# TUMFTM/DPFT

Hardware: AMD Instinct MI355X
Metric: training samples/sec (K-Radar C+R, bs4/GPU) (higher is better)
Workload: dtype f32

## Files before the change

dpft_amd/csrc/common.h:

```cpp
#pragma once
#include <hip/hip_runtime.h>
#include <stdint.h>
#include <stdio.h>
#include <string.h>

#include "../../include/dpft_hip.h"

typedef float f32x4 __attribute__((ext_vector_type(4)));
typedef float f32x16 __attribute__((ext_vector_type(16)));

namespace dpft {

void set_error(const char* fmt, ...);
struct BnReduceFuse {
    const float* y;
    const float* bnp;
    const unsigned char* mask8;
    int self_mask;
    float* sums;
    bool applied;
};
int conv_dgrad_residual(const dpft_conv_desc* d, const float* dy, const float* w_t, float* dx, const float* res_src,
                        const float* res_mask, void* workspace, dpft_stream_t stream, BnReduceFuse* fuse = nullptr,
                        const unsigned char* res_mask8 = nullptr);
// ... 19 lines not shown
__device__ __forceinline__ void bn_from_sums(const BnSumsRef& r, int c, float& mean, float& scale, float& beta, float& invstd) {
    const double m = bn_sums_get(r.sums, r.K, c, 0) * r.invn;
    const double var = fmax(bn_sums_get(r.sums, r.K, c, 1) * r.invn - m * m, 0.0);
    mean = (float)m;
    invstd = 1.0f / sqrtf((float)var + r.eps);
    scale = r.gamma[c] * invstd;
    beta = r.beta[c];
}
__device__ __forceinline__ void fill_pro_table(float* tab, const float* bnp, const BnSumsRef& r, int K, int tid, int nt) {
    if (r.sums) {
        for (int c = tid; c < K; c += nt) {
            float mean, scale, beta, invstd;
            bn_from_sums(r, c, mean, scale, beta, invstd);
            tab[c] = mean; tab[K + c] = scale; tab[2 * K + c] = beta;
        }
    } else {
        for (int i = tid; i < 3 * K; i += nt) tab[i] = bnp[i];
    }
}
int conv_fwd_sums(const dpft_conv_desc* d, const float* x, const float* w, const float* bias, const float* pro_bn,
                  int32_t pro_relu, float* y, float* stats, void* workspace, dpft_stream_t stream,
                  unsigned long long* sums = nullptr, bool* sums_used = nullptr,
                  const BnSumsRef* pro_sums = nullptr, bool* pro_sums_used = nullptr);
int conv_dgrad_fused(const dpft_conv_desc* d, const float* dy, const float* w_t, float* dx, int32_t accumulate,
                     void* workspace, dpft_stream_t stream, BnReduceFuse* fuse);
int bn_bwd_reduce_prezeroed(const float* y, const float* dout, const float* out, const float* mask_bnp, const float* bnp,
                            float* sums, int64_t M, int32_t K, bool act16, dpft_stream_t stream,
                            const unsigned char* mask8 = nullptr);
int bn_bwd_apply_zeroing(const float* y, const float* dout, const float* out, const float* mask_bnp, const float* bnp,
                         const float* gamma, const float* sums, float* dy, float* dgamma, float* dbeta, int64_t M,
                         int32_t K, float* zero_buf, int32_t zero_n, bool act16, dpft_stream_t stream,
                         const unsigned char* mask8 = nullptr, bool frozen = false);
int bn_act_any(const float* y, const float* bnp, const float* res, const float* res_bnp, int32_t relu, float* out,
               float* out32, int64_t M, int32_t K, bool act16, dpft_stream_t stream, unsigned char* mask8 = nullptr);
int bn_act_sums(const float* y, const float* bnp, const BnSumsRef& ys, const float* res, const float* res_bnp, const BnSumsRef& rs,
                int32_t relu, float* out, int64_t M, int32_t K, dpft_stream_t stream, unsigned char* mask8, bool* used);
struct BnSumsBatch {
    static constexpr int MAX = 48;
    const unsigned long long* sums[MAX];
    const float *gamma[MAX], *beta[MAX];
    float *rm[MAX], *rv[MAX], *out[MAX];
    double invn[MAX];
    long long M[MAX];
    int K[MAX];
    int n;
    float eps, momentum;
};
int bn_finalize_sums_batch(const BnSumsBatch& batch, dpft_stream_t stream);
int bn_relu_maxpool_any(const float* y, const float* bnp, float* out, int32_t B, int32_t H, int32_t W, int32_t K,
                        int32_t PH, int32_t PW, bool out16, dpft_stream_t stream);
int bn_relu_maxpool_bwd_any(const float* y, const float* bnp, const float* dout, float* dact, int32_t B, int32_t H,
                            int32_t W, int32_t K, int32_t PH, int32_t PW, bool dout16, dpft_stream_t stream);
int add_inplace_any(float* a, const float* b, int64_t n, bool a16, dpft_stream_t stream);
int cvt_f32_to_bf16(const float* src, float* dst_bf16, int64_t n, dpft_stream_t stream);
struct BnEvalBatch {
    const float *gamma[16], *beta[16], *rm[16], *rv[16];
    float* out[16];
    int K[16];
    int n;
    float eps;
};
int bn_eval_params_batch(const BnEvalBatch& batch, dpft_stream_t stream);
struct TransposeBatch {
    static constexpr int MAX = 80;
    const float* w[MAX];
    float* wt[MAX];
    int K[MAX], taps[MAX], C[MAX];
    int blk_start[MAX + 1];
    int n;
    int mode = 0;
    int tile = 0;
    static int tile_of(int k, int c) { return (k % 64 == 0 && c % 64 == 0) ? 64 : 32; }
    bool fits(int k, int c) const { return n == 0 || tile == tile_of(k, c); }
    void add(const float* src, float* dst, int k, int t, int c) {
        if (n == 0) tile = tile_of(k, c);
        w[n] = src; wt[n] = dst; K[n] = k; taps[n] = t; C[n] = c;
        if (n == 0) blk_start[0] = 0;
        blk_start[n + 1] = blk_start[n] + ((c + tile - 1) / tile) * ((k + tile - 1) / tile) * t;
        ++n;
    }
};
int weight_transpose_batch(const TransposeBatch& tb, dpft_stream_t stream);
int conv_mode_key();
bool profiling_active();
int zero_fill(void* ptr, size_t bytes, dpft_stream_t stream);
int bias_grad_ws(const float* dy, float* db, int64_t M, int32_t K, void* workspace, dpft_stream_t stream);

struct LdsGrant {
    size_t granted[16] = {};
};
inline bool lds_grant(LdsGrant& g, const void* fn, size_t lds) {
    int dev = 0;
    (void)hipGetDevice(&dev);
    size_t& have = g.granted[dev & 15];
    if (lds <= have) return true;
    if (hipFuncSetAttribute(fn, hipFuncAttributeMaxDynamicSharedMemorySize, (int)lds) != hipSuccess) return false;
    have = lds;
    return true;
}

inline int check_launch(const char* what) {
    hipError_t e = hipGetLastError();
    if (e != hipSuccess) {
        set_error("%s: launch failed: %s", what, hipGetErrorString(e));
        return DPFT_ERR_LAUNCH;
    }
    return DPFT_OK;
}

inline int cdiv(int64_t a, int64_t b) { return (int)((a + b - 1) / b); }

constexpr int kNumCU = 256;
constexpr int kNumXCD = 8;

__device__ __forceinline__ int xcd_remap(int bid, int nwg) {
    const int q = nwg / kNumXCD, r = nwg % kNumXCD;
    const int xcd = bid % kNumXCD, idx = bid / kNumXCD;
    const int base = (xcd < r) ? xcd * (q + 1) : r * (q + 1) + (xcd - r) * q;
    return base + idx;
}

}

#ifndef DPFT_PRIO_BN
#define DPFT_PRIO_BN 3
#endif
#ifndef DPFT_PRIO_IGEMM
#define DPFT_PRIO_IGEMM 1
#endif
#define DPFT_SETPRIO_BN() do { if (DPFT_PRIO_BN) __builtin_amdgcn_s_setprio(DPFT_PRIO_BN); } while (0)
#define DPFT_SETPRIO_IGEMM() do { if (DPFT_PRIO_IGEMM) __builtin_amdgcn_s_setprio(DPFT_PRIO_IGEMM); } while (0)

#define DPFT_REQUIRE(cond, ...)                 \
    do {                                        \
        if (!(cond)) {                          \
            dpft::set_error(__VA_ARGS__);       \
            return DPFT_ERR_ARG;                \
        }                                       \
    } while (0)
```

dpft_amd/csrc/conv.hip:

```cpp
#include "conv_core.h"

namespace dpft {


template <int BM, int BN, int WGM, int WGN, bool DGRAD, bool PRO, bool LIN = true, bool BF16 = false, int KS = 1>
__global__ __launch_bounds__(64 * WGM * WGN * KS) void igemm_vec_kernel(IgemmArgs a) {
    static_assert(KS == 1 || KS == 2, "K-split form: two wave sets");
    constexpr int NT = 64 * WGM * WGN * KS, ROWS = NT / 16;
    constexpr int RB = BM / WGM / 32, CB = BN / WGN / 32;
    constexpr int AP = BM / ROWS, BP = BN / ROWS;
    static_assert(WGM * WGN == 4 && RB >= 1 && CB >= 1, "bad tile");
    extern __shared__ __attribute__((aligned(16))) float smem[];
    float* As = smem;
    float* Bs = smem + BM * LDK;
    __bf16* Ah = reinterpret_cast<__bf16*>(smem);
    __bf16* Bh = Ah + BM * LDKH;

    const int tid = threadIdx.x, lane = tid & 63, wave = (tid >> 6) & 3;
    const int kh = KS == 1 ? 0 : tid >> 8;
    const int wm = wave / WGN, wn = wave % WGN;
    int mt, nt, split;
    decode_tile(a, mt, nt, split);
    const int m0 = mt * BM, n0 = nt * BN;

// ... 355 lines not shown
            bh = ok ? oh + a.pad : -(1 << 28);
            bw = ow + a.pad;
        }
        abase = a.x + (size_t)b * a.H * a.W * a.C;
    }
    const int brow = tid % BN, bkq = tid / BN;
    const bool bok = (n0 + brow) < a.N;
    const float* bbase = a.w + (size_t)(bok ? n0 + brow : 0) * a.Ktot;

    float ra[16], rbv[KPB];
    auto load_tile = [&](int kt) {
        int k = kt * BK + akh * 16;
        int tap = k / a.C;
        int c = k - tap * a.C;
        int r = tap / a.kw, s = tap - r * a.kw;
#pragma unroll
        for (int e = 0; e < 16; ++e) {
            int hi, wi;
            bool v = (k + e) < a.Ktot;
            if (!DGRAD) {
                hi = bh + r;
                wi = bw + s;
                v = v && (unsigned)hi < (unsigned)a.H && (unsigned)wi < (unsigned)a.W;
            } else {
                const int th = bh - r, tw = bw - s;
                v = v && th >= 0 && tw >= 0;
                hi = th / a.stride;
                wi = tw / a.stride;
                v = v && (hi * a.stride == th) && (wi * a.stride == tw) && hi < a.H && wi < a.W;
            }
            ra[e] = v ? abase[((size_t)hi * a.W + wi) * a.C + c] : 0.f;
            if (++c == a.C) {
                c = 0;
                if (++s == a.kw) {
                    s = 0;
                    ++r;
                }
            }
        }
        const int kb = kt * BK + bkq * KPB;
#pragma unroll
        for (int e = 0; e < KPB; ++e) rbv[e] = (bok && (kb + e) < a.Ktot) ? bbase[kb + e] : 0.f;
    };
    auto store_tile = [&]() {
#pragma unroll
        for (int e = 0; e < 16; ++e) As[arow * LDG + akh * 16 + e] = ra[e];
#pragma unroll
        for (int e = 0; e < KPB; ++e) Bs[brow * LDG + bkq * KPB + e] = rbv[e];
    };

    f32x16 acc[RB][CB];
#pragma unroll
    for (int j = 0; j < CB; ++j)
#pragma unroll
        for (int r = 0; r < 16; ++r) acc[0][j][r] = 0.f;

    const int kt_begin = split * a.ksteps_per_split;
    const int kt_end = min(a.ksteps, kt_begin + a.ksteps_per_split);
    const float* a_frag = As + (wm * 32 + (lane & 31)) * LDG + (lane >> 5);
    const float* b_frag = Bs + (lane & 31) * LDG + (lane >> 5);
    if (kt_begin < kt_end) {
        load_tile(kt_begin);
        store_tile();
    }
    __syncthreads();
    for (int kt = kt_begin; kt < kt_end; ++kt) {
        const bool more = kt + 1 < kt_end;
        if (more) load_tile(kt + 1);
#pragma unroll
        for (int kk = 0; kk < BK / 2; ++kk) {
            const float av = a_frag[kk * 2];
#pragma unroll
            for (int j = 0; j < CB; ++j)
                acc[0][j] = __builtin_amdgcn_mfma_f32_32x32x2f32(av, b_frag[j * 32 * LDG + kk * 2],
                                                                 acc[0][j], 0, 0, 0);
        }
        __syncthreads();
        if (more) store_tile();
        __syncthreads();
    }
    igemm_epilogue<BM, BN, WGM, WGN, RB, CB>(a, acc, m0, n0, mt, split, smem);
}

__global__ void splitk_reduce_kernel(const float* __restrict__ partial, const float* __restrict__ bias,
                                     float* __restrict__ y, int64_t MN, int N, int splits, int accumulate) {
    int64_t i = ((int64_t)blockIdx.x * blockDim.x + threadIdx.x) * 4;
    if (i >= MN) return;
    if (i + 3 < MN && (N % 4) == 0) {
        f32x4 s = *reinterpret_cast<const f32x4*>(partial + i);
        for (int k = 1; k < splits; ++k) {
            f32x4 t = *reinterpret_cast<const f32x4*>(partial + (size_t)k * MN + i);
            s += t;
        }
        if (bias) {
            const int c = (int)(i % N);
#pragma unroll
            for (int e = 0; e < 4; ++e) s[e] += bias[c + e];
        }
        if (accumulate) s += *reinterpret_cast<const f32x4*>(y + i);
        *reinterpret_cast<f32x4*>(y + i) = s;
    } else {
        for (int e = 0; e < 4 && i + e < MN; ++e) {
            float s = 0.f;
            for (int k = 0; k < splits; ++k) s += partial[(size_t)k * MN + i + e];
            if (bias) s += bias[(i + e) % N];
            if (accumulate) s += y[i + e];
            y[i + e] = s;
        }
    }
}

__global__ __launch_bounds__(256) void splitk_reduce_stats_kernel(const float* __restrict__ partial, float* __restrict__ y,
                                                                  float* __restrict__ stats, int64_t M, int N, int splits,
                                                                  int tile_rows) {
    __shared__ f32x4 red[16][16];
    __shared__ f32x4 smean[16];
    const int cl = threadIdx.x & 15, rg = threadIdx.x >> 4;
    const int tile = blockIdx.x, c = blockIdx.y * 64 + cl * 4;
    const int64_t r0 = (int64_t)tile * tile_rows, MN = M * N;
    const int cnt = (int)min((int64_t)tile_rows, M - r0);
    f32x4 v[8];
    f32x4 sum = {0.f, 0.f, 0.f, 0.f};
#pragma unroll
    for (int i = 0; i < 8; ++i) {
        const int r = rg + i * 16;
        v[i] = f32x4{0.f, 0.f, 0.f, 0.f};
        if (r < cnt) {
            const int64_t o = (r0 + r) * N + c;
            f32x4 a = *reinterpret_cast<const f32x4*>(partial + o);
            for (int k = 1; k < splits; ++k) a += *reinterpret_cast<const f32x4*>(partial + (size_t)k * MN + o);
            *reinterpret_cast<f32x4*>(y + o) = a;
            v[i] = a;
            sum += a;
        }
    }
    red[rg][cl] = sum;
    __syncthreads();
    if (rg == 0) {
        f32x4 t = red[0][cl];
        for (int i = 1; i < 16; ++i) t += red[i][cl];
        smean[cl] = t * (1.0f / (float)cnt);
    }
    __syncthreads();
    const f32x4 mean = smean[cl];
    f32x4 m2 = {0.f, 0.f, 0.f, 0.f};
#pragma unroll
    for (int i = 0; i < 8; ++i)
        if (rg + i * 16 < cnt) {
            const f32x4 dlt = v[i] - mean;
            m2 += dlt * dlt;
        }
    __syncthreads();
    red[rg][cl] = m2;
    __syncthreads();
    if (rg == 0) {
        f32x4 t = red[0][cl];
        for (int i = 1; i < 16; ++i) t += red[i][cl];
        *reinterpret_cast<f32x4*>(stats + ((size_t)tile * 2 + 0) * N + c) = mean;
        *reinterpret_cast<f32x4*>(stats + ((size_t)tile * 2 + 1) * N + c) = t;
    }
}

template <int PARTS>
__global__ __launch_bounds__(256) void splitk_reduce_wide_kernel(const float* __restrict__ partial, float* __restrict__ y,
                                                                 int64_t MN, int splits) {
    constexpr int CH = 256 / PARTS;
    __shared__ f32x4 red[256];
    const int ch = threadIdx.x % CH, part = threadIdx.x / CH;
    const int64_t i = ((int64_t)blockIdx.x * CH + ch) * 4;
    f32x4 s = {0.f, 0.f, 0.f, 0.f};
    if (i < MN)
        for (int k = part; k < splits; k += PARTS) s += *reinterpret_cast<const f32x4*>(partial + (size_t)k * MN + i);
    red[threadIdx.x] = s;
    __syncthreads();
    if (part == 0 && i < MN) {
#pragma unroll
        for (int q = 1; q < PARTS; ++q) s += red[q * CH + ch];
        *reinterpret_cast<f32x4*>(y + i) = s;
    }
}

__global__ void splitk_reduce_residual_kernel(const float* __restrict__ partial, const float* __restrict__ src,
                                              const float* __restrict__ mask, float* __restrict__ y, int64_t MN,
                                              int splits) {
    const int64_t i = (int64_t)blockIdx.x * blockDim.x + threadIdx.x;
    if (i >= MN) return;
    float s = 0.f;
    for (int k = 0; k < splits; ++k) s += partial[(size_t)k * MN + i];
    y[i] = s + (mask[i] > 0.f ? src[i] : 0.f);
}


template <int BMn, int BNc, int WGM, int WGN, bool PRO, bool BF16 = false>
__global__ __launch_bounds__(256) void wgrad_vec_kernel(WgradArgs a) {
    static_assert(!BF16 || (BMn == BNc && (BMn == 128 || BMn == 64)), "bf16 weight gradient: 128 x 128 and 64 x 64 tiles");
    constexpr int RB = BMn / WGM / 32, CB = BNc / WGN / 32;
    constexpr int YCH = BMn / 4, XCH = BNc / 4;
    constexpr int YRP = 256 / YCH, XRP = 256 / XCH;
    constexpr int YP = BKP / YRP, XP = BKP / XRP;
    static_assert(WGM * WGN == 4 && YP >= 1 && XP >= 1, "bad wgrad tile");
    constexpr int SMEM_FLOATS = BKP * (BMn + BNc);
    __shared__ __attribute__((aligned(16))) float smem[SMEM_FLOATS];
    float* Ys = smem;
    float* Xs = smem + BKP * BMn;
    const int tid = threadIdx.x, lane = tid & 63, wave = tid >> 6;
    const int wm = wave / WGN, wn = wave % WGN;

    const int nwg = a.ktiles * a.ctiles * a.taps * a.splits;
    int bid = xcd_remap(blockIdx.x, nwg);
    const int split = bid / (a.ktiles * a.ctiles * a.taps);
    bid -= split * (a.ktiles * a.ctiles * a.taps);
    const int tap = bid / (a.ktiles * a.ctiles);
    bid -= tap * (a.ktiles * a.ctiles);
    const int kt_ = bid / a.ctiles, ct_ = bid - kt_ * a.ctiles;
    const int n0 = kt_ * BMn, c0 = ct_ * BNc;
    const int r = tap / a.kw, s = tap - r * a.kw;

    const int ych = tid % YCH, yrow = tid / YCH;
    const int xch = tid % XCH, xrow = tid / XCH;
    const bool y_ok = (n0 + ych * 4) < a.K;
    const bool x_ok = (c0 + xch * 4) < a.C;
    f32x4 mu = {0.f, 0.f, 0.f, 0.f}, sc = {1.f, 1.f, 1.f, 1.f}, sh = {0.f, 0.f, 0.f, 0.f};
    if (PRO && x_ok) {
        mu = *reinterpret_cast<const f32x4*>(a.pro + c0 + xch * 4);
        sc = *reinterpret_cast<const f32x4*>(a.pro + a.C + c0 + xch * 4);
        sh = *reinterpret_cast<const f32x4*>(a.pro + 2 * a.C + c0 + xch * 4);
        if (BF16) sh -= mu * sc;
    }
    const int ohw = a.OH * a.OW;

    f32x4 ry[YP], rx[XP];
    unsigned x_valid = 0;
    constexpr unsigned OOB = 0x80000000u;
    const bool x16 = a.x16 != 0, dy16 = a.dy16 != 0;
    const __amdgpu_buffer_rsrc_t rsrc_y =
        __builtin_amdgcn_make_buffer_rsrc(const_cast<float*>(a.dy), 0, a.M * a.K * (dy16 ? 2 : 4), 0x00020000);
    const __amdgpu_buffer_rsrc_t rsrc_x =
        __builtin_amdgcn_make_buffer_rsrc(const_cast<float*>(a.x), 0, a.B * a.H * a.W * a.C * (x16 ? 2 : 4), 0x00020000);
    auto ypix = [&](int i) { return BF16 ? 2 * YRP * (i >> 1) + 2 * yrow + (i & 1) : yrow + i * YRP; };
    auto xpix = [&](int i) { return BF16 ? 2 * XRP * (i >> 1) + 2 * xrow + (i & 1) : xrow + i * XRP; };
    unsigned y_voff[YP];
#pragma unroll
    for (int i = 0; i < YP; ++i) y_voff[i] = y_ok ? (unsigned)(ypix(i) * a.K + n0 + ych * 4) * 4u : OOB;
    int xb[XP], xoh[XP], xow[XP];
    {
        const int p_first = (split * a.psteps_per_split) * BKP;
#pragma unroll
        for (int i = 0; i < XP; ++i) {
// ... 988 lines not shown
    (void)big16_tile(d, a, false, false, t);
    if (tile_rows) *tile_rows = t.bm;
    return cdiv(a.M, t.bm);
}

extern "C" int dpft_conv2d_nhwc_fwd_f32(const dpft_conv_desc* d, const float* x, const float* w,
                                        const float* bias, const float* pro_bn, int32_t pro_relu,
                                        float* y, float* stats, void* workspace, dpft_stream_t stream) {
    return dpft::conv_fwd_sums(d, x, w, bias, pro_bn, pro_relu, y, stats, workspace, stream);
}

int dpft::conv_fwd_sums(const dpft_conv_desc* d, const float* x, const float* w, const float* bias, const float* pro_bn,
                        int32_t pro_relu, float* y, float* stats, void* workspace, dpft_stream_t stream,
                        unsigned long long* sums, bool* sums_used, const BnSumsRef* pro_sums, bool* pro_sums_used) {
    if (sums_used) *sums_used = false;
    if (pro_sums_used) *pro_sums_used = false;
    if (pro_sums && !pro_sums->sums) pro_sums = nullptr;
    DPFT_REQUIRE(!pro_sums || (pro_bn && pro_sums_used), "conv fwd: a prologue from column sums needs the BN block's address and the answer slot");
    DPFT_REQUIRE(!sums || (stats && sums_used), "conv fwd: column sums need the statistics table and the answer slot");
    int rc = check_desc(d);
    if (rc) return rc;
    DPFT_REQUIRE(x && w && y, "conv fwd: null tensor");
    {
        static const char* skip = getenv("DPFT_SKIP");
        if (skip && ((strstr(skip, "fwd3x3") && d->kh == 3) || (strstr(skip, "fwd1x1") && d->kh == 1)) && (int64_t)d->B * d->OH * d->OW >= 4096) return DPFT_OK;
    }
    hipStream_t st = (hipStream_t)stream;
    ProfScope prof(0, d, st);
    if (conv16_matches(d) && !pro_bn && !stats) return conv16_forward(d, x, w, bias, y, st);
    static const bool thin_fwd = getenv("DPFT_THIN_FWD") == nullptr || atoi(getenv("DPFT_THIN_FWD")) != 0;
    if (thin_fwd && conv1x1_to16_matches(d) && !pro_bn && !stats) return conv1x1_to16_forward(d, x, w, bias, y, st);
    if (takes_stream1x1(d)) {
        const bool fits = !bias && (!pro_bn || pro_relu);
        DPFT_REQUIRE(fits || !stats, "conv fwd: statistics of a streaming 1x1 conv (%d -> %d) take no bias and only the BatchNorm + ReLU prologue", d->C, d->K);
        if (fits) {
            g_prof_family = kFamF32;
            unsigned long long* bns = sums && (int64_t)d->B * d->OH * d->OW < (1 << 22) ? sums : nullptr;
            if (bns) *sums_used = true;
            if (pro_sums) *pro_sums_used = true;
            return launch_stream1x1(d, x, w, pro_bn, y, stats, nullptr, nullptr, 0, st, bns, pro_sums);
        }
    }
    IgemmArgs a; fill_igemm(a, d, false);
    a.x = x; a.w = w; a.y = y; a.bias = bias; a.stats = stats;
    a.pro = pro_bn; a.pro_relu = pro_relu;
    a.x16 = a.y16 = d->act16 != 0;
    a.w16 = d->act16 == 2;
    if (d->a_planes && d->w_planes && !pro_bn && !d->act16) { a.x3 = d->a_planes; a.w3 = d->w_planes; }
    DPFT_REQUIRE(!(a.w16 && (bias || pro_bn)), "conv fwd: act16 = 2 (bf16 weights) takes no bias and no operand prologue");
    const bool pro = pro_bn != nullptr;
    TileChoice t = choose_tile(a.M, a.N, a.C, a.ksteps, (d->act16 || (pro && !pro_relu)) ? 1 : taps_of(d));
    const bool big16 = !pro && !bias && big16_tile(d, a, false, workspace != nullptr, t);
    if (d->act16 && !big16) t.splits = 1;
    if (big16 && t.splits > 1 && !sk_fixup_ok(a, t.splits, 1)) t.splits = 1;
    DPFT_REQUIRE(!(pro && !t.vec), "conv fwd: fused prologue needs C %% 64 == 0 (C=%d)", d->C);
    if (pro_sums) {
        static const int pipe_env = getenv("DPFT_PIPE") ? atoi(getenv("DPFT_PIPE")) : 3;
        if (!(t.vec && g_conv_bf16 != 1 && !d->act16 && pro_relu && (t.x3 || (pipe_env & 1)) && (int64_t)12 * d->C <= 16384)) return DPFT_OK;
        a.pro_s = *pro_sums;
        *pro_sums_used = true;
    }
    bool fixup = false;
    if (t.splits > 1) {
        DPFT_REQUIRE(workspace, "conv fwd: split-K selected but no workspace given");
        a.partial = ws_slabs(workspace);
        fixup = sk_fixup_ok(a, t.splits, 1);
        if (fixup) a.sk_ticket = reinterpret_cast<int*>(workspace);
        else a.stats = nullptr;
    }
    if (sums && !bias && t.vec && (a.N & 3) == 0 && (t.splits == 1 || fixup) && a.M < (1 << 22)) {
        a.bns = sums;
        a.stats = nullptr;
        *sums_used = true;
    }
    rc = launch_igemm<false>(a, t, pro, st);
    if (rc) return rc;
    if (t.splits > 1 && !fixup) {
        const int64_t MN = (int64_t)a.M * a.N;
        if (stats && !bias && (a.N % 64) == 0 && t.bm <= 128) {
            hipLaunchKernelGGL(splitk_reduce_stats_kernel, dim3(cdiv(a.M, t.bm), a.N / 64), dim3(256), 0, st, a.partial, y,
                               stats, (int64_t)a.M, a.N, t.splits, t.bm);
            return check_launch("conv fwd split-K reduce + stats");
        }
        hipLaunchKernelGGL(splitk_reduce_kernel, dim3(cdiv(MN, 1024)), dim3(256), 0, st, a.partial, bias, y, MN, a.N, t.splits, 0);
        rc = check_launch("conv fwd split-K reduce");
        if (rc) return rc;
        if (stats) {
            rc = dpft_bn_stats_f32(y, stats, a.M, a.N, t.bm, stream);
        }
    }
    return rc;
}

extern "C" int dpft_conv2d_nhwc_fwd_bnact_f32(const dpft_conv_desc* d, const float* x, const float* w, const float* out_bn,
                                              int32_t relu, const float* residual, float* y, void* workspace,
                                              dpft_stream_t stream) {
    int rc = check_desc(d);
    if (rc) return rc;
    DPFT_REQUIRE(x && w && y && out_bn, "conv fwd_bnact: null tensor");
    DPFT_REQUIRE(d->K % 4 == 0, "conv fwd_bnact: K %% 4 == 0 needed (K=%d)", d->K);
    hipStream_t st = (hipStream_t)stream;
    if (takes_stream1x1(d)) {
        ProfScope prof(0, d, st);
        g_prof_family = kFamF32;
        return launch_stream1x1(d, x, w, nullptr, y, nullptr, out_bn, residual, relu, st);
    }
    IgemmArgs a; fill_igemm(a, d, false);
    TileChoice t = choose_tile(a.M, a.N, a.C, a.ksteps, d->act16 ? 1 : taps_of(d));
    if (d->act16) t.splits = 1;
    const int64_t M = (int64_t)d->B * d->OH * d->OW;
    static const bool fix_all = getenv("DPFT_BNACT_FIXUP") == nullptr || atoi(getenv("DPFT_BNACT_FIXUP")) != 0;
    if ((t.x3 || (fix_all && t.vec && !conv16_matches(d))) && t.splits > 1 && workspace && sk_fixup_ok(a, t.splits, 1)) {
        ProfScope prof(0, d, st);
        a.x = x; a.w = w; a.y = y;
        a.partial = ws_slabs(workspace);
        a.sk_ticket = reinterpret_cast<int*>(workspace);
        a.obn = out_bn; a.oadd = residual; a.orelu = relu;
        return launch_igemm<false>(a, t, false, st);
    }
    if (!t.vec || t.splits > 1 || conv16_matches(d)) {
        rc = dpft_conv2d_nhwc_fwd_f32(d, x, w, nullptr, nullptr, 0, y, nullptr, workspace, stream);
        if (rc) return rc;
        return bn_act_any(y, out_bn, residual, nullptr, relu, y, nullptr, M, d->K, d->act16 != 0, stream);
    }
    ProfScope prof(0, d, st);
    a.x = x; a.w = w; a.y = y; a.bias = nullptr; a.stats = nullptr; a.pro = nullptr; a.pro_relu = 0;
    a.x16 = a.y16 = d->act16 != 0;
    if (d->a_planes && d->w_planes && !d->act16) { a.x3 = d->a_planes; a.w3 = d->w_planes; }
    a.obn = out_bn; a.oadd = residual; a.orelu = relu;
    static const int epf_on = getenv("DPFT_EPF") == nullptr ? 7 : atoi(getenv("DPFT_EPF"));
    if ((epf_on & 4) && residual && !d->act16 && !a.x3 && !t.x3 && (int64_t)a.M * a.N < (1ll << 29) && d->stride == 1 && g_conv_bf16 != 1) a.epf = 3;
    return launch_igemm<false>(a, t, false, st);
}

extern "C" int dpft_fpn_lateral_f32(const dpft_conv_desc* d, const float* x, const float* w, const float* bias, const float* top,
                                    int32_t TH, int32_t TW, float* lat, void* workspace, dpft_stream_t stream) {
    int rc = check_desc(d);
    if (rc) return rc;
    DPFT_REQUIRE(x && w && lat && d->kh == 1 && d->kw == 1 && d->stride == 1 && d->pad == 0, "fpn_lateral: a 1x1 conv (stride 1) with its tensors");
    DPFT_REQUIRE(!top || (TH >= 1 && TW >= 1 && TH <= d->H && TW <= d->W && d->K % 4 == 0), "fpn_lateral: bad top level (%d x %d)", TH, TW);
    static const bool fuse = getenv("DPFT_FPN_FUSE") == nullptr || atoi(getenv("DPFT_FPN_FUSE")) != 0;
    if (top && fuse && conv1x1_to16_top_matches(d)) {
        ProfScope prof(0, d, (hipStream_t)stream);
        g_prof_family = kFamVector;
        return conv1x1_to16_top_forward(d, x, w, bias, top, TH, TW, lat, (hipStream_t)stream);
    }
    rc = dpft_conv2d_nhwc_fwd_f32(d, x, w, bias, nullptr, 0, lat, nullptr, workspace, stream);
    if (rc || !top) return rc;
    return dpft_fpn_topdown_add_f32(lat, top, d->B, d->H, d->W, TH, TW, d->K, stream);
}

extern "C" int dpft_fpn_output_f32(const dpft_conv_desc* d, const float* lat, const float* w, const float* bias, const float* pos_x,
                                   const float* pos_y, float* out, void* workspace, dpft_stream_t stream) {
    int rc = check_desc(d);
    if (rc) return rc;
    DPFT_REQUIRE(lat && w && out && (pos_x == nullptr) == (pos_y == nullptr), "fpn_output: null tensor / one embedding table without the other");
    DPFT_REQUIRE(d->H == d->OH && d->W == d->OW, "fpn_output: a same-size conv");
    static const bool fuse = getenv("DPFT_FPN_FUSE") == nullptr || atoi(getenv("DPFT_FPN_FUSE")) != 0;
    if (pos_x && fuse && conv16_matches(d) && !d->act16) {
        ProfScope prof(0, d, (hipStream_t)stream);
        g_prof_family = kFamVector;
        return conv16_forward(d, lat, w, bias, out, (hipStream_t)stream, pos_x, pos_y);
    }
    rc = dpft_conv2d_nhwc_fwd_f32(d, lat, w, bias, nullptr, 0, out, nullptr, workspace, stream);
    if (rc || !pos_x) return rc;
    return dpft_add_pos_f32(out, pos_x, pos_y, d->B, d->H, d->W, d->K, stream);
}
// ... 19 lines not shown
        if (skip && ((strstr(skip, "dgrad3x3") && d->kh == 3) || (strstr(skip, "dgrad1x1") && d->kh == 1)) && (int64_t)d->B * d->H * d->W >= 4096) {
            if (fuse && fuse->sums) fuse->applied = true;
            return DPFT_OK;
        }
    }
    hipStream_t st = (hipStream_t)stream;
    ProfScope prof(1, d, st);
    if (conv16_matches(d)) return conv16_dgrad(d, dy, w_t, dx, accumulate, st);
    if (d->C <= 4 && d->K % 4 == 0 && (size_t)d->C * d->kh * d->kw * d->K * 4 <= 40960 && ((d->C * d->kh * d->kw * d->K) % 4) == 0) {
        const size_t lds = (size_t)d->C * d->kh * d->kw * d->K * 4;
        const dim3 grid(cdiv((int64_t)d->B * d->H * d->W, 256));
#define THIN_DGRAD(CI)                                                                                                  \
    hipLaunchKernelGGL(thin_dgrad_kernel<CI>, grid, dim3(256), lds, st, dy, w_t, dx, d->B, d->H, d->W, d->OH, d->OW, \
                       d->K, d->kh, d->kw, d->stride, d->pad, accumulate)
        switch (d->C) {
            case 1: THIN_DGRAD(1); break;
            case 2: THIN_DGRAD(2); break;
            case 3: THIN_DGRAD(3); break;
            default: THIN_DGRAD(4); break;
        }
#undef THIN_DGRAD
        return check_launch("conv dgrad (thin input)");
    }
    IgemmArgs a; fill_igemm(a, d, true);
    a.x = dy; a.w = w_t; a.y = dx; a.accumulate = accumulate;
    a.x16 = a.y16 = d->act16 != 0;
    a.w16 = d->act16 == 2;
    if (d->a_planes && d->w_planes && !d->act16) { a.x3 = d->a_planes; a.w3 = d->w_planes; }
    const bool fuse_ok = fuse && fuse->sums && (a.N & 3) == 0;
    const int64_t class_wgs = (int64_t)cdiv((int64_t)a.B * cdiv(a.OH, d->stride) * cdiv(a.OW, d->stride), 64) * cdiv(a.N, 64);
    if (d->stride > 1 && (a.C % BKV) == 0 && (class_wgs >= kNumCU / 2 || !workspace || d->act16)) {
        const int sp = d->stride, cpt = a.C / BKV;
        bool empty_class = false;
        for (int ph = 0; ph < sp; ++ph)
            for (int pw = 0; pw < sp; ++pw) {
                const int r0 = (ph + d->pad) % sp, s0 = (pw + d->pad) % sp;
                if (r0 >= d->kh || s0 >= d->kw) empty_class = true;
            }
        if (empty_class && !accumulate)
            DPFT_REQUIRE(zero_fill(dx, (d->act16 ? 2 : sizeof(float)) * (size_t)a.B * a.OH * a.OW * a.N, st) == DPFT_OK,
                         "conv dgrad: zero fill failed");
        for (int ph = 0; ph < sp; ++ph)
            for (int pw = 0; pw < sp; ++pw) {
                const int r0 = (ph + d->pad) % sp, s0 = (pw + d->pad) % sp;
                if (r0 >= d->kh || s0 >= d->kw || ph >= a.OH || pw >= a.OW) continue;
                IgemmArgs q = a;
                q.sub_step = sp; q.sub_ph = ph; q.sub_pw = pw;
                q.sub_oh = (a.OH - ph + sp - 1) / sp; q.sub_ow = (a.OW - pw + sp - 1) / sp;
                q.sub_r0 = r0; q.sub_s0 = s0;
                q.sub_nr = (d->kh - r0 + sp - 1) / sp; q.sub_ns = (d->kw - s0 + sp - 1) / sp;
                q.M = a.B * q.sub_oh * q.sub_ow;
                q.ksteps = q.sub_nr * q.sub_ns * cpt;
                TileChoice tq = choose_tile(q.M, q.N, q.C, q.ksteps);
                tq.splits = 1;
                if (fuse_ok && !empty_class) set_bnr(q, fuse);
                rc = launch_igemm<true>(q, tq, false, st);
                if (rc) return rc;
            }
        if (fuse_ok && !empty_class) fuse->applied = true;
        return DPFT_OK;
    }
    TileChoice t = choose_tile(a.M, a.N, a.C, a.ksteps, (d->act16 || d->stride > 1) ? 1 : taps_of(d));
    const bool big16 = big16_tile(d, a, true, workspace != nullptr, t);
    if (d->act16 && !big16) t.splits = 1;
    if (big16 && t.splits > 1 && !sk_fixup_ok(a, t.splits, 2)) t.splits = 1;
    bool fixup = false;
    if (t.splits > 1) {
        DPFT_REQUIRE(workspace, "conv dgrad: split-K selected but no workspace given");
        a.partial = ws_slabs(workspace);
        fixup = sk_fixup_ok(a, t.splits, 2);
        if (fixup) a.sk_ticket = reinterpret_cast<int*>(workspace);
    }
    if ((t.splits == 1 || fixup) && fuse_ok) {
        set_bnr(a, fuse);
        fuse->applied = true;
    }
    static const int epf_on = getenv("DPFT_EPF") == nullptr ? 3 : atoi(getenv("DPFT_EPF"));
    if ((epf_on & 2) && t.splits == 1 && a.bnr_sums && !accumulate && d->stride == 1 && t.vec && (int64_t)a.M * a.N < (1ll << 29))
        a.epf = 2;
    rc = launch_igemm<true>(a, t, false, st);
    if (rc) return rc;
    if (t.splits > 1 && !fixup) {
        const int64_t MN = (int64_t)a.M * a.N;
        hipLaunchKernelGGL(splitk_reduce_kernel, dim3(cdiv(MN, 1024)), dim3(256), 0, st, a.partial, (const float*)nullptr, dx, MN, a.N, t.splits, accumulate);
        rc = check_launch("conv dgrad split-K reduce");
    }
    return rc;
}

int dpft::conv_dgrad_residual(const dpft_conv_desc* d, const float* dy, const float* w_t, float* dx, const float* res_src,
                              const float* res_mask, void* workspace, dpft_stream_t stream, BnReduceFuse* fuse,
                              const unsigned char* res_mask8) {
    if (fuse) fuse->applied = false;
    int rc = check_desc(d);
    if (rc) return rc;
    DPFT_REQUIRE(dy && w_t && dx && res_src && res_mask, "conv dgrad residual: null tensor");
    {
        static const char* skip = getenv("DPFT_SKIP");
        if (skip && ((strstr(skip, "dgrad3x3") && d->kh == 3) || (strstr(skip, "dgrad1x1") && d->kh == 1)) && (int64_t)d->B * d->H * d->W >= 4096) {
            if (fuse && fuse->sums) fuse->applied = true;
            return DPFT_OK;
        }
    }

    DPFT_REQUIRE(d->stride == 1 && !conv16_matches(d), "conv dgrad residual: stride-1 bottleneck convs only");
    hipStream_t st = (hipStream_t)stream;
    ProfScope prof(1, d, st);
    IgemmArgs a; fill_igemm(a, d, true);
    a.x = dy; a.w = w_t; a.y = dx; a.res_src = res_src; a.res_mask = res_mask;
    a.x16 = a.y16 = d->act16 != 0;
    a.w16 = d->act16 == 2;
    if (d->a_planes && d->w_planes && !d->act16) { a.x3 = d->a_planes; a.w3 = d->w_planes; }
    if (res_mask8 && (a.N & 3) == 0) a.res_mask8 = res_mask8;
    TileChoice t = choose_tile(a.M, a.N, a.C, a.ksteps, d->act16 ? 1 : taps_of(d));
    const bool big16 = big16_tile(d, a, true, workspace != nullptr, t);
    if (d->act16 && !big16) t.splits = 1;
    if (big16 && t.splits > 1 && !sk_fixup_ok(a, t.splits, 4)) t.splits = 1;
    bool fixup = false;
    if (t.splits > 1) {
        DPFT_REQUIRE(workspace, "conv dgrad: split-K selected but no workspace given");
        a.partial = ws_slabs(workspace);
        fixup = sk_fixup_ok(a, t.splits, 4);
        if (fixup) a.sk_ticket = reinterpret_cast<int*>(workspace);
    }
    if ((t.splits == 1 || fixup) && fuse && fuse->sums && (a.N & 3) == 0) {
        set_bnr(a, fuse);
        fuse->applied = true;
    }
    static const int epf_on = getenv("DPFT_EPF") == nullptr ? 3 : atoi(getenv("DPFT_EPF"));
    if ((epf_on & 1) && t.splits == 1 && a.bnr_sums && a.bnr_mask8 && a.res_mask8 && t.vec && (int64_t)a.M * a.N < (1ll << 29) &&
        (int64_t)cdiv(a.M, 128) * cdiv(a.N, 64) >= kNumCU && getenv("DPFT_FORCE_TILE") == nullptr && !big16) {
        a.epf = 1;
        t.bm = 128; t.bn = 64;
    }
    rc = launch_igemm<true>(a, t, false, st);
    if (rc) return rc;
    if (t.splits > 1 && !fixup) {
        const int64_t MN = (int64_t)a.M * a.N;
        hipLaunchKernelGGL(splitk_reduce_residual_kernel, dim3(cdiv(MN, 256)), dim3(256), 0, st, a.partial, res_src,
                           res_mask, dx, MN, t.splits);
        rc = check_launch("conv dgrad split-K residual reduce");
    }
    return rc;
}

extern "C" int dpft_conv2d_nhwc_dgrad_bn_reduce_f32(const dpft_conv_desc* d, const float* dy, const float* w_t, float* dx,
                                                    int32_t accumulate, const float* res_src, const float* res_out,
                                                    const uint8_t* res_mask8, const float* bn_y, const float* bn_block,
                                                    const uint8_t* bn_mask8, int32_t bn_self_mask, float* sums,
                                                    int32_t* applied, void* workspace, dpft_stream_t stream) {
    DPFT_REQUIRE(bn_y && bn_block && sums && applied, "conv dgrad_bn_reduce: null BatchNorm argument");
    DPFT_REQUIRE((bn_mask8 != nullptr) != (bn_self_mask != 0), "conv dgrad_bn_reduce: exactly one of bn_mask8 / bn_self_mask");
    dpft::BnReduceFuse f{bn_y, bn_block, bn_mask8, bn_self_mask, sums, false};
    int rc;
    if (res_src) {
        DPFT_REQUIRE(!accumulate && res_out, "conv dgrad_bn_reduce: the residual form needs res_out and does not accumulate");
        rc = dpft::conv_dgrad_residual(d, dy, w_t, dx, res_src, res_out, workspace, stream, &f, res_mask8);
    } else {
        rc = dpft::conv_dgrad_fused(d, dy, w_t, dx, accumulate, workspace, stream, &f);
    }
    *applied = f.applied ? 1 : 0;
    return rc;
}

extern "C" int dpft_conv2d_nhwc_wgrad_f32(const dpft_conv_desc* d, const float* x, const float* dy,
                                          const float* pro_bn, int32_t pro_relu, float* dw,
                                          void* workspace, dpft_stream_t stream) {
    {
        static const char* skip = getenv("DPFT_SKIP");
        if (skip && strstr(skip, "wgrad")) return DPFT_OK;
    }
    int rc = check_desc(d);
    if (rc) return rc;
    DPFT_REQUIRE(x && dy && dw, "conv wgrad: null tensor");
    DPFT_REQUIRE(!pro_bn || ((d->C % 32 == 0) && (d->K % 4 == 0)),
                 "conv wgrad: fused prologue needs C %% 32 == 0 and K %% 4 == 0 (C=%d, K=%d)", d->C, d->K);
    hipStream_t st = (hipStream_t)stream;
    ProfScope prof(2, d, st);
    if (!pro_bn) {
        bool handled = false;
        rc = thin_wgrad(d, x, dy, dw, workspace, st, handled);
        if (rc || handled) return rc;
    }
    WgradArgs a; memset(&a, 0, sizeof(a));
    a.x = x; a.dy = dy; a.dw = dw; a.pro = pro_bn; a.pro_relu = pro_relu;
    a.x16 = a.dy16 = d->act16 != 0;
    a.B = d->B; a.H = d->H; a.W = d->W; a.C = d->C; a.OH = d->OH; a.OW = d->OW; a.K = d->K;
    a.kh = d->kh; a.kw = d->kw; a.stride = d->stride; a.pad = d->pad;
    a.M = d->B * d->OH * d->OW;
    a.taps = d->kh * d->kw;
    a.J = a.taps * a.C;
    const bool pro = pro_bn != nullptr;
    const bool vec = (d->C % 32 == 0) && (d->K % 4 == 0);
    a.psteps = cdiv(a.M, vec ? BKP : BK);
    DPFT_REQUIRE(!vec || ((int64_t)a.M * a.K < (1ll << 29) && (int64_t)a.B * a.H * a.W * a.C < (1ll << 29)),
                 "conv wgrad: operand larger than 2 GiB");
    int bmn, bnc;
    int64_t tiles;
    if (vec) {
        if (d->K <= 32) { bmn = 32; bnc = 128; }
        else if (d->K >= 128 && d->C >= 128 && (int64_t)cdiv(d->K, 128) * cdiv(d->C, 128) * a.taps >= 8) { bmn = 128; bnc = 128; }
        else { bmn = 64; bnc = 64; }
        a.ktiles = cdiv(d->K, bmn);
        a.ctiles = cdiv(d->C, bnc);
        tiles = (int64_t)a.ktiles * a.ctiles * a.taps;
    } else {
        bmn = 64; bnc = 64;
        a.ktiles = cdiv(d->K, 64);
        a.ctiles = cdiv(a.J, 64);
        tiles = (int64_t)a.ktiles * a.ctiles;
    }
    const int round_wgs = (vec && bmn == 128) ? kNumCU : kNumCU * 2;
    int splits = (int)std::max<int64_t>(1, round_wgs / tiles);
    {
        const int s2 = (int)std::max<int64_t>(1, 2 * round_wgs / tiles);
        const double f1 = (double)tiles * splits / round_wgs, f2 = (double)tiles * s2 / (2.0 * round_wgs);
        if (f1 < 0.8 && f2 > f1 + 0.1) splits = s2;
    }
    const int64_t wbytes = (int64_t)d->K * a.J * 4;
    const int max_splits = (int)std::max<int64_t>(1, std::min<int64_t>(512, (64ll << 20) / wbytes));
    if (splits > max_splits) splits = max_splits;
    if (splits > 1 && a.psteps / splits < 4) {
        if (vec && bmn == 128) {
            bmn = 64; bnc = 64;
            a.ktiles = cdiv(d->K, bmn); a.ctiles = cdiv(d->C, bnc);
            tiles = (int64_t)a.ktiles * a.ctiles * a.taps;
        }
        splits = (int)std::max<int64_t>(1, std::min<int64_t>(std::min<int64_t>(kNumCU / tiles, a.psteps), max_splits));
    }
    if (splits < 1) splits = 1;
    if (const char* f = getenv("DPFT_FORCE_WGRAD")) {
        int tb, sp;
        if (vec && sscanf(f, "%d,%d", &tb, &sp) == 2 && (tb == 128 || tb == 64)) {
            bmn = tb; bnc = tb;
            a.ktiles = cdiv(d->K, bmn); a.ctiles = cdiv(d->C, bnc);
            tiles = (int64_t)a.ktiles * a.ctiles * a.taps;
            splits = std::max(1, std::min(sp, max_splits));
        }
    }
    if (splits > 1 && !workspace) splits = 1;
    a.splits = splits;
    a.psteps_per_split = cdiv(a.psteps, splits);
    a.partial = splits > 1 ? ws_slabs(workspace) : nullptr;
    const int nwg = (int)(tiles * splits);
    dim3 grid(nwg), block(256);
    static const int wpipe_env = getenv("DPFT_PIPE") ? atoi(getenv("DPFT_PIPE")) : 3;
    static const int w16_env = getenv("DPFT_WGRAD16_PIPE") ? atoi(getenv("DPFT_WGRAD16_PIPE")) : 1;
    if (vec && d->act16 && !pro && w16_env && (bmn == 128 || bmn == 64) && (d->C % 8) == 0 && (d->K % 8) == 0) {
        const int pk = bmn == 128 ? 64 : 128;
        a.psteps = cdiv(a.M, pk);
        a.psteps_per_split = cdiv(a.psteps, splits);
        const size_t lds = (size_t)2 * pk * (bmn + bnc) * 2 + (size_t)a.psteps_per_split * pk * 4;
        g_prof_family = kFamBf16;
        if (bmn == 128) launch_lds(wgrad_pipe16_kernel<128, 128, 2, 2, 64>, grid, block, lds, st, a);
        else launch_lds(wgrad_pipe16_kernel<64, 64, 2, 2, 128>, grid, block, lds, st, a);
    } else if (vec && (wpipe_env & 2) && g_conv_bf16 != 1 && !d->act16 && (!pro || pro_relu) && (bmn == 128 || bmn == 64)) {
        const int pk = bmn == 128 ? 32 : 64;
        a.psteps = cdiv(a.M, pk);
        a.psteps_per_split = cdiv(a.psteps, splits);
        const size_t tbl = (size_t)a.psteps_per_split * pk * 4;
        g_prof_family = kFamF32;
        static const bool wx3 = getenv("DPFT_WGRAD_X3") == nullptr || atoi(getenv("DPFT_WGRAD_X3")) != 0;
        static const bool wx3_1x1 = getenv("DPFT_WGRAD_X3_1X1") == nullptr || atoi(getenv("DPFT_WGRAD_X3_1X1")) != 0;
        if (bmn == 128 && wx3 && split_on() && (a.taps > 1 || wx3_1x1) && 2.0 * a.M * (double)d->K * a.J >= 2e9) {
            g_prof_family = kFamX3;
            rc = launch_wgrad_x3(a, pro, grid, st);
            if (rc) return rc;
        } else if (bmn == 128) {
            const size_t lds = (size_t)2 * 32 * (128 + 128) * 4 + tbl;
            if (pro) launch_lds(wgrad_pipe_kernel<128, 128, 2, 2, 32, true>, grid, block, lds, st, a);
            else launch_lds(wgrad_pipe_kernel<128, 128, 2, 2, 32, false>, grid, block, lds, st, a);
        } else {
            const size_t lds = (size_t)2 * 64 * (64 + 64) * 4 + tbl;
            if (pro) launch_lds(wgrad_pipe_kernel<64, 64, 2, 2, 64, true>, grid, block, lds, st, a);
            else launch_lds(wgrad_pipe_kernel<64, 64, 2, 2, 64, false>, grid, block, lds, st, a);
        }
    } else if (vec) {
        g_prof_family = g_conv_bf16 == 1 && (bmn == 128 || bmn == 64) ? kFamBf16 : kFamF32;
#define LAUNCH_WG(BM_, BN_, WGM_, WGN_)                                                           \
    do {                                                                                          \
        if (pro) hipLaunchKernelGGL((wgrad_vec_kernel<BM_, BN_, WGM_, WGN_, true>), grid, block, 0, st, a);  \
        else hipLaunchKernelGGL((wgrad_vec_kernel<BM_, BN_, WGM_, WGN_, false>), grid, block, 0, st, a);     \
    } while (0)
        if (bmn == 128 && g_conv_bf16 == 1) {
            if (pro) hipLaunchKernelGGL((wgrad_vec_kernel<128, 128, 2, 2, true, true>), grid, block, 0, st, a);
            else hipLaunchKernelGGL((wgrad_vec_kernel<128, 128, 2, 2, false, true>), grid, block, 0, st, a);
        } else if (bmn == 64 && g_conv_bf16 == 1) {
            if (pro) hipLaunchKernelGGL((wgrad_vec_kernel<64, 64, 2, 2, true, true>), grid, block, 0, st, a);
            else hipLaunchKernelGGL((wgrad_vec_kernel<64, 64, 2, 2, false, true>), grid, block, 0, st, a);
        } else if (bmn == 128) LAUNCH_WG(128, 128, 2, 2);
        else if (bmn == 64) LAUNCH_WG(64, 64, 2, 2);
        else LAUNCH_WG(32, 128, 1, 4);
#undef LAUNCH_WG
    } else {
        hipLaunchKernelGGL(wgrad_gen_kernel, grid, block, 0, st, a);
    }
    rc = check_launch("conv wgrad");
    if (rc) return rc;
    {
        static const char* skip = getenv("DPFT_SKIP");
        if (skip && strstr(skip, "wreduce")) return rc;
    }
    if (splits > 1) {
        const int64_t n = (int64_t)d->K * a.J;
        if ((n & 3) == 0 && splits >= 16) {
            if (n / 4 <= (int64_t)kNumCU * 64) hipLaunchKernelGGL(splitk_reduce_wide_kernel<16>, dim3(cdiv(n / 4, 16)), dim3(256), 0, st, a.partial, dw, n, splits);
            else hipLaunchKernelGGL(splitk_reduce_wide_kernel<4>, dim3(cdiv(n / 4, 64)), dim3(256), 0, st, a.partial, dw, n, splits);
        } else {
            hipLaunchKernelGGL(splitk_reduce_kernel, dim3(cdiv(n, 1024)), dim3(256), 0, st, a.partial, (const float*)nullptr, dw, n, 4, splits, 0);
        }
        rc = check_launch("conv wgrad split-K reduce");
    }
    return rc;
}

extern "C" int dpft_weight_transpose_f32(const float* w, float* w_t, int32_t K, int32_t taps,
                                         int32_t C, dpft_stream_t stream) {
    DPFT_REQUIRE(w && w_t && K > 0 && taps > 0 && C > 0, "weight_transpose: bad arguments");
    dim3 grid(cdiv(C, 32), cdiv(K, 32), taps);
    hipLaunchKernelGGL(weight_transpose_kernel, grid, dim3(256), 0, (hipStream_t)stream, w, w_t, K, taps, C);
    return check_launch("weight_transpose");
}

extern "C" int dpft_weight_transpose_batch_f32(int32_t n, const float* const* w, float* const* w_t, const int32_t* K,
                                               const int32_t* taps, const int32_t* C, dpft_stream_t stream) {
    DPFT_REQUIRE(n >= 1 && n <= dpft::TransposeBatch::MAX && w && w_t && K && taps && C, "weight_transpose_batch: 1..80 tensors");
    dpft::TransposeBatch tb;
    tb.n = 0;
    tb.mode = 0;
    for (int i = 0; i < n; ++i) {
        DPFT_REQUIRE(w[i] && w_t[i] && K[i] > 0 && taps[i] > 0 && C[i] > 0, "weight_transpose_batch: bad entry %d", i);
        if (!tb.fits(K[i], C[i])) {
            int rc = dpft::weight_transpose_batch(tb, stream);
            if (rc) return rc;
            tb.n = 0;
        }
        tb.add(w[i], w_t[i], K[i], taps[i], C[i]);
    }
    return dpft::weight_transpose_batch(tb, stream);
}

int dpft::weight_transpose_batch(const TransposeBatch& tb, dpft_stream_t stream) {
    DPFT_REQUIRE(tb.n >= 1 && tb.n <= TransposeBatch::MAX, "weight_transpose_batch: 1..%d tensors", TransposeBatch::MAX);
    if (tb.tile == 64) hipLaunchKernelGGL(weight_transpose_batch64_kernel, dim3(tb.blk_start[tb.n]), dim3(256), 0, (hipStream_t)stream, tb);
    else hipLaunchKernelGGL(weight_transpose_batch_kernel, dim3(tb.blk_start[tb.n]), dim3(256), 0, (hipStream_t)stream, tb);
    return check_launch("weight_transpose_batch");
}

namespace dpft {
__global__ __launch_bounds__(256) void zero_fill_kernel(unsigned* __restrict__ p, size_t n4, size_t n) {
    const size_t stride = (size_t)gridDim.x * 256;
    for (size_t i = (size_t)blockIdx.x * 256 + threadIdx.x; i < n4; i += stride) reinterpret_cast<uint4*>(p)[i] = uint4{0u, 0u, 0u, 0u};
    if (blockIdx.x == 0)
        for (size_t i = n4 * 4 + threadIdx.x; i < n; i += 256) p[i] = 0u;
}
}

int dpft::zero_fill(void* ptr, size_t bytes, dpft_stream_t stream) {
    DPFT_REQUIRE(ptr && (bytes & 3) == 0 && ((uintptr_t)ptr & 15) == 0, "zero_fill: 16-byte aligned pointer, size a multiple of 4");
    const size_t n = bytes / 4, n4 = n / 4;
    const int blocks = (int)std::max<size_t>(1, std::min<size_t>(kNumCU * 8, (n4 + 255) / 256));
    hipLaunchKernelGGL(zero_fill_kernel, dim3(blocks), dim3(256), 0, (hipStream_t)stream, (unsigned*)ptr, n4, n);
    return check_launch("zero_fill");
}

extern "C" int dpft_bias_grad_f32(const float* dy, float* db, int64_t M, int32_t K,
                                  dpft_stream_t stream) {
    DPFT_REQUIRE(dy && db && M > 0 && K > 0 && K <= 256, "bias_grad: bad arguments (K=%d)", K);
    (void)hipMemsetAsync(db, 0, sizeof(float) * K, (hipStream_t)stream);
    const int rpi = 256 / K;
    int blocks = (int)std::min<int64_t>(1024, (M + rpi - 1) / rpi);
    hipLaunchKernelGGL(bias_grad_kernel, dim3(blocks), dim3(256), 0, (hipStream_t)stream, dy, db, M, K);
    return check_launch("bias_grad");
}

int dpft::bias_grad_ws(const float* dy, float* db, int64_t M, int32_t K, void* workspace, dpft_stream_t stream) {
    static const bool slab_on = getenv("DPFT_BIAS_SLAB") == nullptr || atoi(getenv("DPFT_BIAS_SLAB")) != 0;
    if (!workspace || !slab_on || K > 256 || K <= 0) return dpft_bias_grad_f32(dy, db, M, K, stream);
    const int rpi = 256 / K;
    const int blocks = (int)std::min<int64_t>(kBiasBlocks, (M + rpi - 1) / rpi);
    hipLaunchKernelGGL(bias_grad_slab_kernel, dim3(blocks), dim3(256), 0, (hipStream_t)stream, dy, db, M, (int)K, ws_slabs(workspace),
                       reinterpret_cast<int*>(workspace));
    return check_launch("bias_grad (slab)");
}

extern "C" int dpft_conv2d_nhwc_wgrad_bias_f32(const dpft_conv_desc* d, const float* x, const float* dy, float* dw, float* db,
                                               void* workspace, dpft_stream_t stream) {
    int rc = check_desc(d);
    if (rc) return rc;
    DPFT_REQUIRE(x && dy && dw && db, "conv wgrad_bias: null tensor");
    static const bool fuse = getenv("DPFT_BIAS_FUSE") == nullptr || atoi(getenv("DPFT_BIAS_FUSE")) != 0;
    const bool fusable = dpft::conv16_matches(d) ||
                         (d->kh == 1 && d->kw == 1 && d->stride == 1 && d->pad == 0 && d->K == 16 && (d->C == 3 || d->C == 6));
    if (fuse && fusable && workspace && !d->act16) {
        dpft::ProfScope prof(2, d, (hipStream_t)stream);
        bool handled = false, bias_done = false;
// ... 73 lines not shown
```

dpft_amd/csrc/conv_core.h:

```cpp
#pragma once
#include "common.h"

#include <math.h>
#include <stdlib.h>

#include <algorithm>
#include <type_traits>
#include <utility>
#include <vector>

namespace dpft {

constexpr int BK = 32;
constexpr int BKV = 64;
constexpr int LDK = BKV + 4;
constexpr int LDKH = BKV + 8;
typedef __bf16 bf16x4 __attribute__((ext_vector_type(4)));
typedef __bf16 bf16x8 __attribute__((ext_vector_type(8)));
constexpr int LDG = BK + 1;
constexpr int BKP = 64;

typedef unsigned u32x2 __attribute__((ext_vector_type(2)));
typedef unsigned u32x4 __attribute__((ext_vector_type(4)));
__device__ __forceinline__ f32x4 widen_bf16x4(u32x2 v) {
// ... 351 lines not shown
                    }
                    if (accum || resid || oadd) v += old[it];
                    if (obn && a.orelu) {
#pragma unroll
                        for (int e = 0; e < 4; ++e) v[e] = fmaxf(v[e], 0.f);
                    }
                    const size_t ooff = out_pixel(a, m0 + row) * a.N + n0 + c4 * 4;
                    store4_act(out, ooff, v, decltype(H16)::value);
                    if (bnr) {
                        const f32x4 yv = bnr_yv[it];
                        f32x4 d = v;
                        if (decltype(H16)::value) d = __builtin_convertvector(__builtin_convertvector(v, bf16x4s), f32x4);
                        if (PFM == 1 || a.bnr_mask8) {
                            const unsigned mk = bnr_mk[it];
#pragma unroll
                            for (int e = 0; e < 4; ++e) d[e] = ((mk >> e) & 1u) ? d[e] : 0.f;
                        } else if (a.bnr_self_mask) {
#pragma unroll
                            for (int e = 0; e < 4; ++e) d[e] = fmaf(yv[e] - bmu[e], bsc[e], bbe[e]) > 0.f ? d[e] : 0.f;
                        }
#pragma unroll
                        for (int e = 0; e < 4; ++e) {
                            bs0[e] += d[e];
                            bs1[e] += d[e] * ((yv[e] - bmu[e]) * bis[e]);
                        }
                    }
                }
            }
        };
        if (y16) store_all(std::true_type{});
        else store_all(std::false_type{});
        if (bnr) {
            __syncthreads();
            float* red = smem;
            *reinterpret_cast<f32x4*>(red + tid * 8) = bs0;
            *reinterpret_cast<f32x4*>(red + tid * 8 + 4) = bs1;
            __syncthreads();
            if (tid < BN && n0 + tid < a.N) {
                const int ch = tid >> 2, e = tid & 3;
                float t0 = 0.f, t1 = 0.f;
                for (int g = 0; g < NT / C4; ++g) {
                    t0 += red[(g * C4 + ch) * 8 + e];
                    t1 += red[(g * C4 + ch) * 8 + 4 + e];
                }
                atomicAdd(a.bnr_sums + n0 + tid, t0);
                atomicAdd(a.bnr_sums + a.N + n0 + tid, t1);
            }
        }
    } else {
        for (int idx = tid; idx < BM * BN; idx += NT) {
            const int row = idx / BN, c = idx - row * BN;
            if (m0 + row < a.M && n0 + c < a.N) {
                float v = Cs[row * LDC + c];
                if (add_bias) v += a.bias[n0 + c];
                const size_t off = out_pixel(a, m0 + row) * a.N + n0 + c;
                float* o = out + off;
                if (a.res_src != nullptr && !part) v += a.res_mask[off] > 0.f ? a.res_src[off] : 0.f;
                else if (accum) v += *o;
                *o = v;
            }
        }
    }
}

__device__ __forceinline__ void decode_tile(const IgemmArgs& a, int& mt, int& nt, int& split) {
    const int nwg = a.mtiles * a.ntiles * a.splits;
    int bid = xcd_remap(blockIdx.x, nwg);
    const int per = a.mtiles * a.ntiles;
    split = bid / per;
    bid -= split * per;
    mt = bid / a.ntiles;
    nt = bid - mt * a.ntiles;
}

template <typename Fn, int... I>
__device__ __forceinline__ void static_for_impl(Fn&& f, std::integer_sequence<int, I...>) {
    (f(std::integral_constant<int, I>{}), ...);
}
template <int N, typename Fn>
__device__ __forceinline__ void static_for(Fn&& f) {
    static_for_impl(f, std::make_integer_sequence<int, N>{});
}

struct WgradArgs {
    const float* x;
    const float* dy;
    float* dw;
    float* partial;
    const float* pro;
    int B, H, W, C;
    int OH, OW, K;
    int kh, kw, stride, pad;
    int M;
    int ktiles, ctiles, taps, splits, psteps, psteps_per_split;
    int pro_relu;
    int J;
    int x16, dy16;
};

int launch_igemm_x3(IgemmArgs& a, int bm, int bn, bool dgrad, bool pro, hipStream_t st);
int split_planes(const float* src, void* dst, int64_t n, hipStream_t st);
bool stream1x1_match(const dpft_conv_desc* d, int* tile_rows);
int launch_stream1x1(const dpft_conv_desc* d, const float* x, const float* w, const float* pro_bn, float* y, float* stats,
                     const float* out_bn, const float* residual, int relu, hipStream_t st, unsigned long long* bns = nullptr,
                     const BnSumsRef* pro_sums = nullptr);
int launch_igemm_b16w(IgemmArgs& a, int bm, int bn, bool dgrad, hipStream_t st);
int launch_wgrad_x3(const WgradArgs& a, bool pro, dim3 grid, hipStream_t st);

}
```

dpft_amd/csrc/conv_pipe.h:

```cpp
#pragma once

namespace dpft {


template <int BM, int BN, int WGM, int WGN, int PBK, bool DGRAD, bool PRO, bool B16 = false, int EPF = 0>
__global__ __launch_bounds__(256) void igemm_pipe_kernel(IgemmArgs a) {
    static_assert(EPF == 0 || (EPF == 3 ? (!DGRAD && !PRO) : (DGRAD && !PRO)), "epilogue prefetch: data gradients (1, 2) / inference forward (3)");
    static_assert(!(PRO && B16), "operand prologue: fp32 operands only");
    constexpr int EB = B16 ? 2 : 4;
    constexpr int EPC = 16 / EB;
    constexpr int RB = BM / WGM / 32, CB = BN / WGN / 32;
    constexpr int CH = PBK / EPC;
    constexpr int RW = 64 / CH;
    constexpr int RPP = 4 * RW;
    constexpr int AP = BM / RPP, BP = BN / RPP;
    constexpr int ROWB = PBK * EB;
    constexpr int A_BYTES = BM * ROWB, B_BYTES = BN * ROWB, STAGE = A_BYTES + B_BYTES;
    constexpr int NG = PBK / (2 * EPC);
    static_assert(CH == 8 || CH == 16, "rows of 128 or 256 bytes");
    static_assert(WGM * WGN == 4 && RB >= 1 && CB >= 1 && AP >= 1 && BP >= 1, "bad tile");
    static_assert(2 * STAGE <= 65536, "LDS offsets must fit the ds_read immediate");
    extern __shared__ __attribute__((aligned(16))) float smem[];
    typedef __attribute__((address_space(3))) char lds_char;
    lds_char* const lds0 = (lds_char*)smem;
// ... 202 lines not shown
    auto step = [&](auto STG, auto MORE) __attribute__((always_inline)) {
        constexpr int stg = decltype(STG)::value;
        constexpr bool more = decltype(MORE)::value;
        using OTHER = std::integral_constant<int, (stg ^ 1)>;
        if constexpr (more) prep();
        f32x4 af[2][RB], bf[2][CB];
        auto frags = [&](auto SET, auto KG) {
            constexpr int set = decltype(SET)::value, kg = decltype(KG)::value;
#pragma unroll
            for (int i = 0; i < RB; ++i) af[set][i] = *(lds_f32x4*)(size_t)(a_ad[kg] + (unsigned)(stg * STAGE + i * 32 * ROWB));
#pragma unroll
            for (int j = 0; j < CB; ++j) bf[set][j] = *(lds_f32x4*)(size_t)(b_ad[kg] + (unsigned)(stg * STAGE + j * 32 * ROWB));
        };
        frags(std::integral_constant<int, 0>{}, std::integral_constant<int, 0>{});
        __builtin_amdgcn_sched_barrier(0);
        static_for<SLOTS>([&](auto S) {
            constexpr int sl = decltype(S)::value;
            constexpr int g = sl / MPG, w = sl % MPG, e = w / (RB * CB), ij = w % (RB * CB), i = ij / CB, j = ij % CB;
            if constexpr (w == 0 && g + 1 < NG)
                frags(std::integral_constant<int, ((g + 1) & 1)>{}, std::integral_constant<int, (g + 1 < NG ? g + 1 : 0)>{});
            if constexpr (B16)
                acc[i][j] = __builtin_amdgcn_mfma_f32_32x32x16_bf16(__builtin_bit_cast(bf16x8, af[g & 1][i]),
                                                                    __builtin_bit_cast(bf16x8, bf[g & 1][j]), acc[i][j], 0, 0, 0);
            else
                acc[i][j] = __builtin_amdgcn_mfma_f32_32x32x2f32(af[g & 1][i][e], bf[g & 1][j][e], acc[i][j], 0, 0, 0);
            __builtin_amdgcn_sched_barrier(0);
            if constexpr (more && sl < NOPS) {
                vmem_op(OTHER{}, std::integral_constant<int, (sl < NOPS ? sl : 0)>{});
                __builtin_amdgcn_sched_barrier(0);
            }
            if constexpr (more && PRO) {
                constexpr int gq = g - (NG - LASTG);
                constexpr int sp = MPG / QPG;
                if constexpr (gq >= 0 && (w % sp) == sp - 1 && (w / sp) < QPG) {
                    consume(OTHER{}, std::integral_constant<int, (gq >= 0 ? gq * QPG + w / sp : 0)>{});
                    __builtin_amdgcn_sched_barrier(0);
                }
            }
        });
        if constexpr (more) advance();
    };
    auto fence = [&]() {
        asm volatile("s_waitcnt vmcnt(0) lgkmcnt(0)" ::: "memory");
        __builtin_amdgcn_s_barrier();
        __builtin_amdgcn_sched_barrier(0);
    };
    using S0 = std::integral_constant<int, 0>;
    using S1 = std::integral_constant<int, 1>;
    using T = std::true_type;
    using F = std::false_type;

    if (nsteps > 0) {
        prep();
        static_for<NOPS>([&](auto K) { vmem_op(S0{}, K); });
        if constexpr (PRO) static_for<AP>([&](auto I) { consume(S0{}, I); });
        advance();
    }
    if constexpr (EPF != 0) {
        static_for<EP_ITER * 4>([&](auto O) {
            constexpr int o = decltype(O)::value;
            pf_op(std::integral_constant<int, o / 4>{}, std::integral_constant<int, o % 4>{});
        });
    }
    fence();
    int s_ = 0;
    for (; s_ + 2 < nsteps; s_ += 2) {
        step(S0{}, T{});
        fence();
        step(S1{}, T{});
        fence();
    }
    if (nsteps - s_ == 2) {
        step(S0{}, T{});
        fence();
        step(S1{}, F{});
    } else if (nsteps - s_ == 1) {
        step(S0{}, F{});
    }
    if constexpr (EPF != 0) igemm_epilogue<BM, BN, WGM, WGN, RB, CB, 256, PFT>(a, acc, m0, n0, mt, split, smem, &pf);
    else igemm_epilogue<BM, BN, WGM, WGN, RB, CB, 256>(a, acc, m0, n0, mt, split, smem);
}

template <int BMn, int BNc, int WGM, int WGN, int PK, bool PRO>
__global__ __launch_bounds__(256) void wgrad_pipe_kernel(WgradArgs a) {
    constexpr int RB = BMn / WGM / 32, CB = BNc / WGN / 32;
    constexpr int YL = BMn / 4, XL = BNc / 4;
    constexpr int YRW = 64 / YL, XRW = 64 / XL;
    constexpr int YRPP = 4 * YRW, XRPP = 4 * XRW;
    constexpr int YP = PK / YRPP, XP = PK / XRPP;
    constexpr int Y_BYTES = PK * BMn * 4, X_BYTES = PK * BNc * 4, STAGE = Y_BYTES + X_BYTES;
    static_assert(WGM * WGN == 4 && RB >= 1 && CB >= 1 && YP >= 1 && XP >= 1 && YL <= 64 && XL <= 64, "bad wgrad tile");
    static_assert(2 * STAGE <= 65536, "LDS offsets must fit the ds_read immediate");
    extern __shared__ __attribute__((aligned(16))) float smem[];
    typedef __attribute__((address_space(3))) char lds_char;
    lds_char* const lds0 = (lds_char*)smem;
    const int tid = threadIdx.x, lane = tid & 63, wave = __builtin_amdgcn_readfirstlane(tid >> 6);
    const int wm = wave / WGN, wn = wave % WGN;

    const int nwg = a.ktiles * a.ctiles * a.taps * a.splits;
    int bid = xcd_remap(blockIdx.x, nwg);
    const int split = bid / (a.ktiles * a.ctiles * a.taps);
    bid -= split * (a.ktiles * a.ctiles * a.taps);
    const int tap = bid / (a.ktiles * a.ctiles);
    bid -= tap * (a.ktiles * a.ctiles);
    const int kt_ = bid / a.ctiles, ct_ = bid - kt_ * a.ctiles;
    const int n0 = kt_ * BMn, c0 = ct_ * BNc;
    const int r = tap / a.kw, s = tap - r * a.kw;

    const int yr = YRW * wave + lane / YL, ych = lane % YL;
    const int xr = XRW * wave + lane / XL, xch = lane % XL;
    const bool y_ok = (n0 + ych * 4) < a.K;
    const bool x_ok = (c0 + xch * 4) < a.C;
    f32x4 mu = {0.f, 0.f, 0.f, 0.f}, sc = {1.f, 1.f, 1.f, 1.f}, sh = {0.f, 0.f, 0.f, 0.f};
    if (PRO && x_ok) {
        mu = *reinterpret_cast<const f32x4*>(a.pro + c0 + xch * 4);
        sc = *reinterpret_cast<const f32x4*>(a.pro + a.C + c0 + xch * 4);
        sh = *reinterpret_cast<const f32x4*>(a.pro + 2 * a.C + c0 + xch * 4);
    }
    const int ohw = a.OH * a.OW;
    constexpr unsigned OOB = 0x80000000u;
    const __amdgpu_buffer_rsrc_t rsrc_y =
        __builtin_amdgcn_make_buffer_rsrc(const_cast<float*>(a.dy), 0, a.M * a.K * 4, 0x00020000);
    const __amdgpu_buffer_rsrc_t rsrc_x =
        __builtin_amdgcn_make_buffer_rsrc(const_cast<float*>(a.x), 0, a.B * a.H * a.W * a.C * 4, 0x00020000);
    unsigned y_voff[YP];
#pragma unroll
    for (int i = 0; i < YP; ++i) y_voff[i] = y_ok ? (unsigned)((YRPP * i + yr) * a.K + n0 + ych * 4) * 4u : OOB;
    const int ps_begin = split * a.psteps_per_split;
    const int ps_end = min(a.psteps, ps_begin + a.psteps_per_split);
    const int nsteps = max(ps_end - ps_begin, 0);
    unsigned* const tbl = reinterpret_cast<unsigned*>(reinterpret_cast<char*>(smem) + 2 * STAGE);
    {
        const int npix = nsteps * PK;
        for (int idx = tid; idx < npix; idx += 256) {
            const int p = ps_begin * PK + idx;
            const int b = p / ohw;
            const int rem = p - b * ohw;
            const int oh = rem / a.OW, ow = rem - oh * a.OW;
            const int hi = oh * a.stride - a.pad + r, wi = ow * a.stride - a.pad + s;
            const bool v = p < a.M && (unsigned)hi < (unsigned)a.H && (unsigned)wi < (unsigned)a.W;
            tbl[idx] = v ? ((((unsigned)b * a.H + hi) * a.W + wi) * a.C) * 4u : OOB;
        }
    }
    __syncthreads();
    typedef __attribute__((address_space(3))) const unsigned lds_u32;
    unsigned tbl_ad = (unsigned)(size_t)lds0 + 2 * STAGE + xr * 4;
    const unsigned x_lane = x_ok ? (unsigned)(c0 + xch * 4) * 4u : OOB;
    int next_ps = ps_begin;
    int so_y = 0;
    unsigned xoffs[XP];
    unsigned long long x_inv[PRO ? XP : 1] = {};
    auto prep = [&]() {
        so_y = __builtin_amdgcn_readfirstlane(next_ps * PK * a.K * 4);
#pragma unroll
        for (int i = 0; i < XP; ++i) {
            const unsigned t = *(lds_u32*)(size_t)(tbl_ad + (unsigned)(XRPP * i * 4));
            xoffs[i] = t + x_lane;
            if constexpr (PRO) x_inv[i] = __builtin_amdgcn_ballot_w64((int)xoffs[i] < 0);
        }
        tbl_ad += PK * 4;
        ++next_ps;
    };
    f32x4 rx[PRO ? XP : 1];
    unsigned rxo[PRO ? XP : 1] = {};
    unsigned long long rx_inv[PRO ? XP : 1] = {};
    constexpr int NOPS = YP + XP;
    auto vmem_op = [&](auto STG, auto K) {
        constexpr int stg = decltype(STG)::value, k = decltype(K)::value;
        if constexpr (k < YP) {
            __builtin_amdgcn_raw_ptr_buffer_load_lds(rsrc_y, lds0 + stg * STAGE + (YRPP * k + YRW * wave) * BMn * 4, 16,
                                                     (int)y_voff[k], so_y, 0, 0);
        } else {
            constexpr int i = k - YP;
            if constexpr (PRO) {
                rx[i] = __builtin_bit_cast(f32x4, __builtin_amdgcn_raw_buffer_load_b128(rsrc_x, (int)xoffs[i], 0, 0));
                rxo[i] = xoffs[i];
                rx_inv[i] = x_inv[i];
            } else {
                __builtin_amdgcn_raw_ptr_buffer_load_lds(rsrc_x, lds0 + stg * STAGE + Y_BYTES + (XRPP * i + XRW * wave) * BNc * 4, 16,
                                                         (int)xoffs[i], 0, 0, 0);
            }
        }
    };
// ... 373 lines not shown
```

dpft_amd/csrc/conv_x3.hip:

```cpp
#include "conv_core.h"

namespace dpft {

typedef __bf16 bf16x2_t __attribute__((ext_vector_type(2)));
typedef float f32x2_t __attribute__((ext_vector_type(2)));

__device__ __forceinline__ unsigned cvt_pk_bf16(float x, float y) {
    return __builtin_bit_cast(unsigned, __builtin_convertvector(f32x2_t{x, y}, bf16x2_t));
}
__device__ __forceinline__ void split3(const f32x4 v, u32x2& p1, u32x2& p2, u32x2& p3) {
#pragma unroll
    for (int h = 0; h < 2; ++h) {
        const float x = v[2 * h], y = v[2 * h + 1];
        const unsigned q1 = cvt_pk_bf16(x, y);
        const float rx = x - __uint_as_float(q1 << 16), ry = y - __uint_as_float(q1 & 0xffff0000u);
        const unsigned q2 = cvt_pk_bf16(rx, ry);
        const float sx = rx - __uint_as_float(q2 << 16), sy = ry - __uint_as_float(q2 & 0xffff0000u);
        p1[h] = q1;
        p2[h] = q2;
        p3[h] = cvt_pk_bf16(sx, sy);
    }
}

template <int BM, int BN, bool DGRAD, int PRO_, int EPF = 0>
// ... 597 lines not shown
    };
    using S0 = std::integral_constant<int, 0>;
    using S1 = std::integral_constant<int, 1>;
    using T = std::true_type;
    using F = std::false_type;
    if (nsteps > 0) {
        prep();
        static_for<NU>([&](auto U) { load_unit(S0{}, U); });
        advance();
        static_for<NU>([&](auto U) { store_unit(S0{}, U); });
        if (nsteps > 1) {
            prep();
            static_for<NU>([&](auto U) { load_unit(S1{}, U); });
            advance();
        }
        if (nsteps > 2) {
            prep();
            static_for<NU>([&](auto U) { load_unit(S0{}, U); });
            advance();
        }
    }
    if constexpr (EPF != 0) {
        static_for<EP_ITER * 4>([&](auto O) {
            constexpr int o = decltype(O)::value;
            pf_op(std::integral_constant<int, o / 4>{}, std::integral_constant<int, o % 4>{});
        });
    }
    fence();
    int rem = nsteps;
    for (; rem >= 5; rem -= 2) {
        step(S0{}, T{}, T{});
        fence();
        step(S1{}, T{}, T{});
        fence();
    }
    if (rem == 4) {
        step(S0{}, T{}, T{});
        fence();
        step(S1{}, T{}, F{});
        fence();
        step(S0{}, T{}, F{});
        fence();
        step(S1{}, F{}, F{});
    } else if (rem == 3) {
        step(S0{}, T{}, F{});
        fence();
        step(S1{}, T{}, F{});
        fence();
        step(S0{}, F{}, F{});
    } else if (rem == 2) {
        step(S0{}, T{}, F{});
        fence();
        step(S1{}, F{}, F{});
    } else if (rem == 1) {
        step(S0{}, F{}, F{});
    }
#pragma unroll
    for (int i = 0; i < RB; ++i)
#pragma unroll
        for (int j = 0; j < CB; ++j) acc[i][j] += acl[i][j];
    if constexpr (EPF != 0) igemm_epilogue<BM, BN, WGM, WGN, RB, CB, 256, PFT>(a, acc, m0, n0, mt, split, smem, &pf);
    else igemm_epilogue<BM, BN, WGM, WGN, RB, CB, 256>(a, acc, m0, n0, mt, split, smem);
}

__global__ __launch_bounds__(256) void split_planes_kernel(const float* __restrict__ src, __bf16* __restrict__ dst, int64_t n) {
    for (int64_t i = ((int64_t)blockIdx.x * 256 + threadIdx.x) * 4; i < n; i += (int64_t)gridDim.x * 1024) {
        const f32x4 v = *reinterpret_cast<const f32x4*>(src + i);
        u32x2 p1, p2, p3;
        split3(v, p1, p2, p3);
        *reinterpret_cast<u32x2*>(dst + i) = p1;
        *reinterpret_cast<u32x2*>(dst + n + i) = p2;
        *reinterpret_cast<u32x2*>(dst + 2 * n + i) = p3;
    }
}
int split_planes(const float* src, void* dst, int64_t n, hipStream_t st) {
    DPFT_REQUIRE(src && dst && n > 0 && n % 4 == 0, "split_planes: bad arguments (n %% 4 == 0)");
    const int nb = (int)std::min<int64_t>((n / 4 + 255) / 256, kNumCU * 16);
    hipLaunchKernelGGL(split_planes_kernel, dim3(nb), dim3(256), 0, st, src, (__bf16*)dst, n);
    return check_launch("split_planes");
}


template <int PRO_>
__global__ __launch_bounds__(256) void wgrad_x3_kernel(WgradArgs a) {
    constexpr bool PRO = PRO_ != 0, MASK = PRO_ == 2;
    constexpr int BMn = 128, BNc = 128, WGM = 2, WGN = 2, PK = 32;
    constexpr int RB = 2, CB = 2;
    constexpr int YL = BMn / 4, XL = BNc / 4;
    constexpr int YRW = 64 / YL, XRW = 64 / XL;
    constexpr int YRPP = 4 * YRW, XRPP = 4 * XRW;
    constexpr int YP = PK / YRPP, XP = PK / XRPP, NQ = YP + XP;
    constexpr int Y_ROWB = BMn * 2, X_ROWB = BNc * 2;
    constexpr int Y_PLANE = PK * Y_ROWB, X_PLANE = PK * X_ROWB;
    constexpr int Y_BYTES = 3 * Y_PLANE, X_BYTES = 3 * X_PLANE, STAGE = Y_BYTES + X_BYTES;
    constexpr int NG = PK / 16;
    extern __shared__ __attribute__((aligned(16))) float smem[];
    char* const lds = reinterpret_cast<char*>(smem);
    typedef __attribute__((address_space(3))) char lds_char;
    const unsigned lds_base = (unsigned)(size_t)(lds_char*)smem;
    const int tid = threadIdx.x, lane = tid & 63, wave = __builtin_amdgcn_readfirstlane(tid >> 6);
    const int wm = wave / WGN, wn = wave % WGN;

    const int nwg = a.ktiles * a.ctiles * a.taps * a.splits;
    int bid = xcd_remap(blockIdx.x, nwg);
    const int split = bid / (a.ktiles * a.ctiles * a.taps);
    bid -= split * (a.ktiles * a.ctiles * a.taps);
    const int tap = bid / (a.ktiles * a.ctiles);
    bid -= tap * (a.ktiles * a.ctiles);
    const int kt_ = bid / a.ctiles, ct_ = bid - kt_ * a.ctiles;
    const int n0 = kt_ * BMn, c0 = ct_ * BNc;
    const int r = tap / a.kw, s = tap - r * a.kw;

    const int yr = YRW * wave + lane / YL, ych = lane % YL;
    const int xr = XRW * wave + lane / XL, xch = lane % XL;
    const bool y_ok = (n0 + ych * 4) < a.K;
    const bool x_ok = (c0 + xch * 4) < a.C;
    f32x4 p_mu = {0.f, 0.f, 0.f, 0.f}, p_sc = {1.f, 1.f, 1.f, 1.f}, p_sh = {0.f, 0.f, 0.f, 0.f};
    if (PRO && x_ok) {
        p_mu = *reinterpret_cast<const f32x4*>(a.pro + c0 + xch * 4);
        p_sc = *reinterpret_cast<const f32x4*>(a.pro + a.C + c0 + xch * 4);
        p_sh = *reinterpret_cast<const f32x4*>(a.pro + 2 * a.C + c0 + xch * 4);
    }
    const int ohw = a.OH * a.OW;
    constexpr unsigned OOB = 0x80000000u;
    const __amdgpu_buffer_rsrc_t rsrc_y = __builtin_amdgcn_make_buffer_rsrc(const_cast<float*>(a.dy), 0, a.M * a.K * 4, 0x00020000);
    const __amdgpu_buffer_rsrc_t rsrc_x = __builtin_amdgcn_make_buffer_rsrc(const_cast<float*>(a.x), 0, a.B * a.H * a.W * a.C * 4, 0x00020000);
    unsigned y_voff[YP];
#pragma unroll
    for (int i = 0; i < YP; ++i) y_voff[i] = y_ok ? (unsigned)((YRPP * i + yr) * a.K + n0 + ych * 4) * 4u : OOB;
    const int ps_begin = split * a.psteps_per_split;
    const int ps_end = min(a.psteps, ps_begin + a.psteps_per_split);
    const int nsteps = max(ps_end - ps_begin, 0);
    unsigned* const tbl = reinterpret_cast<unsigned*>(lds + 2 * STAGE);
    {
        const int npix = nsteps * PK;
        for (int idx = tid; idx < npix; idx += 256) {
            const int p = ps_begin * PK + idx;
            const int b = p / ohw;
            const int rem = p - b * ohw;
            const int oh = rem / a.OW, ow = rem - oh * a.OW;
            const int hi = oh * a.stride - a.pad + r, wi = ow * a.stride - a.pad + s;
            const bool v = p < a.M && (unsigned)hi < (unsigned)a.H && (unsigned)wi < (unsigned)a.W;
            tbl[idx] = v ? ((((unsigned)b * a.H + hi) * a.W + wi) * a.C) * 4u : OOB;
        }
    }
    __syncthreads();
    typedef __attribute__((address_space(3))) const unsigned lds_u32;
    unsigned tbl_ad = lds_base + 2 * STAGE + xr * 4;
    const unsigned x_lane = x_ok ? (unsigned)(c0 + xch * 4) * 4u : OOB;
    int next_ps = ps_begin;
    int so_y = 0;
    unsigned xoffs[XP];
    auto prep = [&]() {
        so_y = __builtin_amdgcn_readfirstlane(next_ps * PK * a.K * 4);
#pragma unroll
        for (int i = 0; i < XP; ++i) xoffs[i] = *(lds_u32*)(size_t)(tbl_ad + (unsigned)(XRPP * i * 4)) + x_lane;
        tbl_ad += PK * 4;
        ++next_ps;
    };
    f32x4 rq[2][NQ];
    unsigned rx_bad[2] = {0, 0};
    auto load_quad = [&](auto SET, auto K) {
        constexpr int set = decltype(SET)::value, k = decltype(K)::value;
        if constexpr (k < YP) {
            rq[set][k] = __builtin_bit_cast(f32x4, __builtin_amdgcn_raw_buffer_load_b128(rsrc_y, (int)y_voff[k], so_y, 0));
        } else {
            constexpr int i = k - YP;
            rq[set][k] = __builtin_bit_cast(f32x4, __builtin_amdgcn_raw_buffer_load_b128(rsrc_x, (int)xoffs[i], 0, 0));
            if constexpr (MASK) rx_bad[set] = (rx_bad[set] & ~(1u << i)) | ((xoffs[i] >> 31) << i);
        }
    };
    const int yw_off = yr * Y_ROWB + ((((ych >> 1) ^ ((yr & 3) << 2)) << 4) | ((ych & 1) << 3));
    const int xw_off = xr * X_ROWB + ((((xch >> 1) ^ ((xr & 3) << 2)) << 4) | ((xch & 1) << 3));
    f32x4 cv;
    u32x2 c1, c2, c3;
    float rr0 = 0.f, rr1 = 0.f;
    auto piece = [&](auto STG, auto K, auto ID) __attribute__((always_inline)) {
        constexpr int stg = decltype(STG)::value, k = decltype(K)::value, id = decltype(ID)::value;
        constexpr bool bn = PRO && k >= YP;
        if constexpr (id == 0 || id == 1) {
            if constexpr (id == 0) cv = rq[stg][k];
#pragma unroll
            for (int e = 2 * id; e < 2 * id + 2; ++e) cv[e] = fmaxf(fmaf(cv[e] - p_mu[e], p_sc[e], p_sh[e]), 0.f);
        } else if constexpr (id == 2) {
            const unsigned keep = ~(unsigned)__builtin_amdgcn_sbfe(rx_bad[stg], k - YP, 1);
#pragma unroll
            for (int e = 0; e < 4; ++e) cv[e] = __uint_as_float(__float_as_uint(cv[e]) & keep);
// ... 300 lines not shown
```

dpft_amd/csrc/resnet_plan.hip:

```cpp
#include <algorithm>
#include <vector>

#include "common.h"

namespace dpft {

struct ConvRef {
    dpft_conv_desc d{};
    int w;
    size_t wt = 0;
    size_t w16 = 0;
};

struct BlockPlan {
    ConvRef c1, c2, c3, cd;
    bool has_ds;
    int bn1, bn2, bn3, bnd;
    int layer;
    size_t x, y1, y2, y3, yd, out, mask;
    size_t a1 = 0, a2 = 0;
    size_t p1, p2, p3, pd;
    size_t s1, s2, s3, sd;
    int t1, t2, t3, td, r1, r2, r3, rd;
};

struct ResnetPlan {
    dpft_resnet_desc desc;
    std::vector<BlockPlan> blocks;
    ConvRef adj, c0;
    int bn0;
    size_t xa, y0, p0, s0, pool;
    int t0, r0;
    int PH, PW;
    int n_conv, n_bn;
    size_t out_off[4];
    size_t out32_off[4];
    int out_shape[4][4];
    size_t fwd_floats;
    size_t bwd_floats;
    size_t ws_bytes;
    size_t arena_bytes;
    size_t g_off[2];
    size_t gmax;
    size_t o_dy, o_da, o_dd, o_wt, o_sums;
    std::vector<size_t> bnacc;
    size_t o_bnacc = 0, bnacc_floats = 0;
    struct PendingBn { int bn, K; long long M; size_t bnp; };
    std::vector<char> bn_pending;
    std::vector<PendingBn> pend_list;
    size_t o_dy2;
    int g_cur;
    bool g_valid;
    bool frozen = false;
    int mode_key = 0;
    hipStream_t side = nullptr;
    bool side_owned = true, side_set = false;
    bool ev_valid[3] = {false, false, false};
    bool use_graph = false;
    struct GraphEntry {
        int kind;
        const void *x, *arena, *dout, *st;
        uint64_t tables_hash;
        int warm;
        hipGraphExec_t exec;
        bool failed;
    };
    std::vector<GraphEntry> graphs;
    hipEvent_t ev_ready = nullptr, ev_done[3] = {nullptr, nullptr, nullptr}, ev_join = nullptr, ev_wt = nullptr;
    int dyi = 0;
    ~ResnetPlan() {
        if (side_set && side_owned) (void)hipStreamDestroy(side);
        for (auto& g : graphs)
            if (g.exec) (void)hipGraphExecDestroy(g.exec);
        if (ev_ready) (void)hipEventDestroy(ev_ready);
        if (ev_join) (void)hipEventDestroy(ev_join);
        if (ev_wt) (void)hipEventDestroy(ev_wt);
        for (auto& e : ev_done)
            if (e) (void)hipEventDestroy(e);
    }
};

static size_t align64(size_t f) { return (f + 63) & ~(size_t)63; }

static dpft_conv_desc mk(int B, int H, int W, int C, int K, int k, int s, int p) {
    dpft_conv_desc d{};
    d.B = B; d.H = H; d.W = W; d.C = C; d.K = K; d.kh = k; d.kw = k; d.stride = s; d.pad = p;
    d.OH = (H + 2 * p - k) / s + 1;
    d.OW = (W + 2 * p - k) / s + 1;
    return d;
}

static size_t nelem_out(const dpft_conv_desc& d) { return (size_t)d.B * d.OH * d.OW * d.K; }
static size_t nelem_in(const dpft_conv_desc& d) { return (size_t)d.B * d.H * d.W * d.C; }
static size_t nelem_w(const dpft_conv_desc& d) { return (size_t)d.K * d.kh * d.kw * d.C; }

}

using namespace dpft;

extern "C" int64_t dpft_resnet_plan_create(const dpft_resnet_desc* desc) {
    if (!desc || desc->B <= 0 || desc->H <= 0 || desc->W <= 0 || desc->n_layers < 1 || desc->n_layers > 4 ||
        desc->act16 < 0 || desc->act16 > 2) {
        set_error("resnet_plan_create: bad descriptor");
        return 0;
    }
    ResnetPlan* p = new ResnetPlan();
    p->desc = *desc;
    p->mode_key = conv_mode_key();
    size_t off = 0;
    auto take = [&](size_t floats) { size_t o = off; off += align64(floats); return o; };
    int nconv = 0, nbn = 0;
    const int B = desc->B;
    size_t wsb = 0;
    auto track_ws = [&](const dpft_conv_desc& d) {
        int64_t w = dpft_conv2d_workspace_bytes(&d);
        if (w > 0 && (size_t)w > wsb) wsb = (size_t)w;
    };
    size_t gmax = 0;
    auto track_g = [&](size_t n) { if (n > gmax) gmax = n; };
    auto stats_of = [&](const dpft_conv_desc& d, int& tiles, int& rows) {
        int32_t r = 0;
        tiles = dpft_conv2d_stats_tiles(&d, &r);
        rows = r;
        return (size_t)tiles * 2 * d.K;
    };
    int H = desc->H, W = desc->W;
    if (desc->in_channels != 3) {
        p->adj.d = mk(B, H, W, desc->in_channels, 3, 1, 1, 0);
        p->adj.w = nconv++;
        p->xa = take(nelem_out(p->adj.d));
        track_ws(p->adj.d);
    } else {
        p->adj.w = -1;
        p->xa = (size_t)-1;
    }
    p->c0.d = mk(B, H, W, 3, 64, 7, 2, 3);
    p->c0.w = nconv++;
    p->bn0 = nbn++;
    track_ws(p->c0.d);
    p->y0 = take(nelem_out(p->c0.d));
    p->p0 = take(4 * 64);
    p->s0 = take(stats_of(p->c0.d, p->t0, p->r0));
    track_g(nelem_out(p->c0.d));
    p->PH = (p->c0.d.OH + 2 - 3) / 2 + 1;
    p->PW = (p->c0.d.OW + 2 - 3) / 2 + 1;
    p->pool = take((size_t)B * p->PH * p->PW * 64);
    track_g((size_t)B * p->PH * p->PW * 64);
    int curH = p->PH, curW = p->PW, inC = 64;
    size_t cur = p->pool;
    const int planes_of[4] = {64, 128, 256, 512};
    for (int li = 0; li < desc->n_layers; ++li) {
        const int planes = planes_of[li];
        for (int b = 0; b < desc->depths[li]; ++b) {
            BlockPlan bp;
            const int stride = (li > 0 && b == 0) ? 2 : 1;
            bp.layer = li;
            bp.has_ds = (b == 0);
            bp.x = cur;
            bp.c1.d = mk(B, curH, curW, inC, planes, 1, 1, 0);   bp.c1.w = nconv++;  bp.bn1 = nbn++;
            bp.c2.d = mk(B, curH, curW, planes, planes, 3, stride, 1);  bp.c2.w = nconv++;  bp.bn2 = nbn++;
            const int oh = bp.c2.d.OH, ow = bp.c2.d.OW;
            bp.c3.d = mk(B, oh, ow, planes, planes * 4, 1, 1, 0);  bp.c3.w = nconv++;  bp.bn3 = nbn++;
            if (bp.has_ds) {
                bp.cd.d = mk(B, curH, curW, inC, planes * 4, 1, stride, 0);  bp.cd.w = nconv++;  bp.bnd = nbn++;
            } else {
                bp.cd.w = -1; bp.bnd = -1;
            }
            bp.c1.d.act16 = bp.c2.d.act16 = bp.c3.d.act16 = desc->act16;
            if (bp.has_ds) bp.cd.d.act16 = desc->act16;
            if (desc->act16 == 2) {
                bp.a1 = take(nelem_out(bp.c1.d) / 2);
                bp.a2 = take(nelem_out(bp.c2.d) / 2);
                bp.c1.w16 = take((nelem_w(bp.c1.d) + 1) / 2);
                bp.c2.w16 = take((nelem_w(bp.c2.d) + 1) / 2);
                bp.c3.w16 = take((nelem_w(bp.c3.d) + 1) / 2);
                if (bp.has_ds) bp.cd.w16 = take((nelem_w(bp.cd.d) + 1) / 2);
            }
            bp.y1 = take(nelem_out(bp.c1.d));  bp.p1 = take(4 * planes);  bp.s1 = take(stats_of(bp.c1.d, bp.t1, bp.r1));
            bp.y2 = take(nelem_out(bp.c2.d));  bp.p2 = take(4 * planes);  bp.s2 = take(stats_of(bp.c2.d, bp.t2, bp.r2));
            bp.y3 = take(nelem_out(bp.c3.d));  bp.p3 = take(4 * planes * 4);  bp.s3 = take(stats_of(bp.c3.d, bp.t3, bp.r3));
            if (bp.has_ds) {
                bp.yd = take(nelem_out(bp.cd.d));  bp.pd = take(4 * planes * 4);  bp.sd = take(stats_of(bp.cd.d, bp.td, bp.rd));
                track_ws(bp.cd.d);
            } else {
                bp.yd = bp.pd = bp.sd = (size_t)-1; bp.td = bp.rd = 0;
            }
            bp.out = take(nelem_out(bp.c3.d));
            bp.mask = take((nelem_out(bp.c3.d) / 4 + 3) / 4);
            track_ws(bp.c1.d); track_ws(bp.c2.d); track_ws(bp.c3.d);
            track_g(nelem_in(bp.c1.d)); track_g(nelem_out(bp.c1.d)); track_g(nelem_out(bp.c2.d)); track_g(nelem_out(bp.c3.d));
            p->blocks.push_back(bp);
            cur = bp.out;
            curH = oh; curW = ow; inC = planes * 4;
        }
        p->out_off[li] = cur;
        p->out32_off[li] = desc->act16 ? take(nelem_out(p->blocks.back().c3.d)) : cur;
        p->out_shape[li][0] = B; p->out_shape[li][1] = curH; p->out_shape[li][2] = curW; p->out_shape[li][3] = inC;
    }
    p->n_conv = nconv;
    p->n_bn = nbn;
    {
        p->bnacc.assign(nbn, 0);
        size_t acc = 0;
        auto add = [&](int bn, int K) { p->bnacc[bn] = acc; acc += align64((size_t)8 * K); };
        add(p->bn0, 64);
        for (const BlockPlan& b : p->blocks) {
            add(b.bn1, b.c1.d.K); add(b.bn2, b.c2.d.K); add(b.bn3, b.c3.d.K);
            if (b.has_ds) add(b.bnd, b.cd.d.K);
        }
        p->bnacc_floats = acc;
        p->bn_pending.assign(nbn, 0);
        p->o_bnacc = take(acc);
    }
    p->fwd_floats = off;
    p->gmax = gmax;
    p->g_off[0] = take(gmax);
    p->g_off[1] = take(gmax);
    size_t wmax = nelem_w(p->c0.d);
    for (int li = 0; li < p->desc.n_layers; ++li) {
        size_t acc = 0;
        for (auto& b : p->blocks) {
            if (b.layer != li) continue;
            b.c1.wt = acc; acc += align64(nelem_w(b.c1.d));
            b.c2.wt = acc; acc += align64(nelem_w(b.c2.d));
            b.c3.wt = acc; acc += align64(nelem_w(b.c3.d));
            if (b.has_ds) { b.cd.wt = acc; acc += align64(nelem_w(b.cd.d)); }
        }
        wmax = std::max(wmax, acc);
    }
    p->bwd_floats = off;
    p->o_dy = take(gmax);
    p->o_dy2 = take(gmax);
    p->o_da = take(gmax);
    p->o_dd = take(gmax);
    p->o_wt = take(wmax);
    p->o_sums = take(2 * 2 * 2048);
    p->ws_bytes = wsb;
    p->arena_bytes = off * sizeof(float) + 2 * wsb + 384;
    p->g_valid = false;
    p->g_cur = 0;
    return (int64_t)(intptr_t)p;
}

extern "C" void dpft_resnet_plan_destroy(int64_t h) { delete (ResnetPlan*)(intptr_t)h; }

extern "C" int64_t dpft_resnet_plan_query(int64_t h, int32_t what, int32_t idx) {
    ResnetPlan* p = (ResnetPlan*)(intptr_t)h;
    if (!p) return -1;
    switch (what) {
        case 0: return (int64_t)p->arena_bytes;
        case 1: return p->n_conv;
        case 2: return p->n_bn;
        case 3: return (int64_t)p->out32_off[idx];
        case 4: return p->out_shape[idx / 4][idx % 4];
        case 5: return (int64_t)p->fwd_floats;
        default: return -1;
    }
}

extern "C" int dpft_resnet_plan_set_side_stream(int64_t h, dpft_stream_t side) {
    ResnetPlan* p = (ResnetPlan*)(intptr_t)h;
    DPFT_REQUIRE(p, "resnet_plan_set_side_stream: null plan");
    if (p->side_set && p->side_owned && p->side != (hipStream_t)side) (void)hipStreamDestroy(p->side);
    p->side = (hipStream_t)side;
    p->side_owned = false;
    p->side_set = true;
    return DPFT_OK;
}

namespace dpft {

struct Tables {
    const dpft_resnet_tables* t;
    const float* w(int i) const { return (const float*)t->conv_w[i]; }
    float* dw(int i) const { return (float*)t->conv_dw[i]; }
    const float* gamma(int i) const { return (const float*)t->bn_gamma[i]; }
    const float* beta(int i) const { return (const float*)t->bn_beta[i]; }
    float* rm(int i) const { return (float*)t->bn_rm[i]; }
    float* rv(int i) const { return (float*)t->bn_rv[i]; }
    float* dgamma(int i) const { return (float*)t->bn_dgamma[i]; }
    float* dbeta(int i) const { return (float*)t->bn_dbeta[i]; }
};

#define RC(call)              \
    do {                      \
        int rc_ = (call);     \
        if (rc_) return rc_;  \
    } while (0)


static float* stage_out32(const ResnetPlan* p, const BlockPlan& b, float* A) {
    if (!p->desc.act16 || b.out != p->out_off[b.layer]) return nullptr;
    return A + p->out32_off[b.layer];
}

static int bn_params(const ResnetPlan* p, const Tables& T, int bn, const float* stats, int tiles, int rows, int64_t M,
                     int K, float* bnp, bool train, dpft_stream_t st) {
    if (train)
        return dpft_bn_finalize_f32(stats, tiles, rows, M, K, T.gamma(bn), T.beta(bn), p->desc.eps, p->desc.momentum,
                                    T.rm(bn), T.rv(bn), bnp, st);
    return DPFT_OK;
}

static bool bn_sums_on(const ResnetPlan* p) {
    static const int on = getenv("DPFT_BN_SUMS") ? atoi(getenv("DPFT_BN_SUMS")) : 1;
    return on != 0 && p->desc.act16 == 0 && !p->frozen;
}
static BnSumsRef bn_sums_ref(const ResnetPlan* p, const Tables& T, float* A, int bn, int K, int64_t M) {
    return BnSumsRef{(const unsigned long long*)(A + p->o_bnacc + p->bnacc[bn]), T.gamma(bn), T.beta(bn), 1.0 / (double)M, p->desc.eps, K};
}
static int bn_finalize_pending(ResnetPlan* p, const Tables& T, float* A, size_t from, dpft_stream_t st) {
    BnSumsBatch batch;
    memset(&batch, 0, sizeof(batch));
    batch.eps = p->desc.eps; batch.momentum = p->desc.momentum;
    for (size_t i = from; i < p->pend_list.size(); ++i) {
        const ResnetPlan::PendingBn& e = p->pend_list[i];
        if (!p->bn_pending[e.bn]) continue;
        const int j = batch.n++;
        batch.sums[j] = (const unsigned long long*)(A + p->o_bnacc + p->bnacc[e.bn]);
        batch.gamma[j] = T.gamma(e.bn); batch.beta[j] = T.beta(e.bn); batch.rm[j] = T.rm(e.bn); batch.rv[j] = T.rv(e.bn);
        batch.out[j] = A + e.bnp; batch.invn[j] = 1.0 / (double)e.M; batch.M[j] = e.M; batch.K[j] = e.K;
        p->bn_pending[e.bn] = 0;
        if (batch.n == BnSumsBatch::MAX) {
            RC(bn_finalize_sums_batch(batch, st));
            batch.n = 0;
        }
    }
    if (batch.n > 0) RC(bn_finalize_sums_batch(batch, st));
    return DPFT_OK;
}
static int bn_finalize_one(ResnetPlan* p, const Tables& T, float* A, int bn, dpft_stream_t st) {
    for (size_t i = 0; i < p->pend_list.size(); ++i)
        if (p->pend_list[i].bn == bn) {
            BnSumsBatch batch;
            memset(&batch, 0, sizeof(batch));
            const ResnetPlan::PendingBn& e = p->pend_list[i];
            batch.eps = p->desc.eps; batch.momentum = p->desc.momentum; batch.n = 1;
            batch.sums[0] = (const unsigned long long*)(A + p->o_bnacc + p->bnacc[bn]);
// ... 136 lines not shown
                }
                tb.add(T.w(c->w), A + c->w16, c->d.K, c->d.kh * c->d.kw, c->d.C);
                if (tb.n == TransposeBatch::MAX) {
                    RC(weight_transpose_batch(tb, st));
                    tb.n = 0;
                }
            }
        }
        if (tb.n > 0) RC(weight_transpose_batch(tb, st));
    }
    for (const BlockPlan& b : p->blocks) {
        const int64_t M1 = (int64_t)b.c1.d.B * b.c1.d.OH * b.c1.d.OW, M2 = (int64_t)b.c2.d.B * b.c2.d.OH * b.c2.d.OW;
        if (w16) {
            RC(conv_bn_train(p, T, b.c1, b.bn1, A + b.x, nullptr, A, A + b.y1, A + b.s1, b.t1, b.r1, M1, A + b.p1, ws, st, A + b.c1.w16));
            RC(train_act_pass(p, T, A, A + b.y1, b.bn1, b.c1.d.K, M1, A + b.p1, nullptr, -1, nullptr, A + b.a1, nullptr, true, st, nullptr));
            RC(conv_bn_train(p, T, b.c2, b.bn2, A + b.a1, nullptr, A, A + b.y2, A + b.s2, b.t2, b.r2, M2, A + b.p2, ws, st, A + b.c2.w16));
            RC(train_act_pass(p, T, A, A + b.y2, b.bn2, b.c2.d.K, M2, A + b.p2, nullptr, -1, nullptr, A + b.a2, nullptr, true, st, nullptr));
            RC(conv_bn_train(p, T, b.c3, b.bn3, A + b.a2, nullptr, A, A + b.y3, A + b.s3, b.t3, b.r3, M2, A + b.p3, ws, st, A + b.c3.w16));
        } else {
        RC(conv_bn_train(p, T, b.c1, b.bn1, A + b.x, nullptr, A, A + b.y1, A + b.s1, b.t1, b.r1, M1, A + b.p1, ws, st));
        RC(conv_bn_train(p, T, b.c2, b.bn2, A + b.y1, A + b.p1, A, A + b.y2, A + b.s2, b.t2, b.r2, M2, A + b.p2, ws, st, nullptr, b.bn1, b.c1.d.K, M1));
        RC(conv_bn_train(p, T, b.c3, b.bn3, A + b.y2, A + b.p2, A, A + b.y3, A + b.s3, b.t3, b.r3, M2, A + b.p3, ws, st, nullptr, b.bn2, b.c2.d.K, M2));
        }
        if (b.has_ds)
            RC(conv_bn_train(p, T, b.cd, b.bnd, A + b.x, nullptr, A, A + b.yd, A + b.sd, b.td, b.rd, M2, A + b.pd, ws, st,
                             w16 ? A + b.cd.w16 : nullptr));
        RC(train_act_pass(p, T, A, A + b.y3, b.bn3, b.c3.d.K, M2, A + b.p3, b.has_ds ? A + b.yd : A + b.x, b.has_ds ? b.bnd : -1,
                          b.has_ds ? A + b.pd : nullptr, A + b.out, stage_out32(p, b, A), a16, st, tr ? (unsigned char*)(A + b.mask) : nullptr));
    }
    RC(bn_finalize_pending(p, T, A, 0, st));
    p->g_valid = false;
    return DPFT_OK;
}

namespace dpft {

struct BnSums {
    float* buf[2];
    int cur;
    bool frozen;
};
static int bn_backward(const float* y, const float* dout, const float* out, const float* mask_bnp, const float* bnp,
                       const float* gamma, BnSums& bs, float* dy, float* dgamma, float* dbeta, int64_t M, int K,
                       dpft_stream_t st, bool act16 = false, const unsigned char* mask8 = nullptr, bool reduced = false) {
    float* sums = bs.buf[bs.cur];
    float* other = bs.buf[bs.cur ^ 1];
    bs.cur ^= 1;
    if (!reduced) RC(bn_bwd_reduce_prezeroed(y, dout, out, mask_bnp, bnp, sums, M, K, act16, st, mask8));
    return bn_bwd_apply_zeroing(y, dout, out, mask_bnp, bnp, gamma, sums, dy, dgamma, dbeta, M, K, other, 2 * 2048, act16, st,
                                mask8, bs.frozen);
}

static hipStream_t shared_side_stream() {
    static hipStream_t s = nullptr;
    static int mode = -1;
    if (mode < 0) {
        const char* e = getenv("DPFT_SHARED_WGRAD_STREAM");
        mode = (e && e[0] == '1') ? 1 : 0;
    }
    if (mode == 1 && !s && hipStreamCreateWithFlags(&s, hipStreamNonBlocking) != hipSuccess) s = nullptr;
    return mode == 1 ? s : nullptr;
}

struct SideCtx {
    ResnetPlan* p;
    hipStream_t main;
    void* ws2;
    int init() {
        if (!p->side_set) {
            if (hipStream_t sh = shared_side_stream()) {
                p->side = sh;
                p->side_owned = false;
            } else {
                DPFT_REQUIRE(hipStreamCreateWithFlags(&p->side, hipStreamNonBlocking) == hipSuccess, "resnet_backward: side stream");
            }
            p->side_set = true;
        }
        if (!p->ev_ready) {
            DPFT_REQUIRE(hipEventCreateWithFlags(&p->ev_ready, hipEventDisableTiming) == hipSuccess, "resnet_backward: event");
            DPFT_REQUIRE(hipEventCreateWithFlags(&p->ev_join, hipEventDisableTiming) == hipSuccess, "resnet_backward: event");
            DPFT_REQUIRE(hipEventCreateWithFlags(&p->ev_wt, hipEventDisableTiming) == hipSuccess, "resnet_backward: event");
            for (auto& e : p->ev_done)
                DPFT_REQUIRE(hipEventCreateWithFlags(&e, hipEventDisableTiming) == hipSuccess, "resnet_backward: event");
        }
        return DPFT_OK;
    }
    int acquire(int slot) {
        if (!p->ev_valid[slot]) return DPFT_OK;
        DPFT_REQUIRE(hipStreamWaitEvent(main, p->ev_done[slot], 0) == hipSuccess, "resnet_backward: wait event");
        return DPFT_OK;
    }
    int wgrad(int slot, const dpft_conv_desc* d, const float* x, const float* dy, const float* pro, int relu, float* dw) {
        if (profiling_active())
            return dpft_conv2d_nhwc_wgrad_f32(d, x, dy, pro, relu, dw, ws2, (dpft_stream_t)main);
        DPFT_REQUIRE(hipEventRecord(p->ev_ready, main) == hipSuccess, "resnet_backward: record event");
        DPFT_REQUIRE(hipStreamWaitEvent(p->side, p->ev_ready, 0) == hipSuccess, "resnet_backward: wait event");
        RC(dpft_conv2d_nhwc_wgrad_f32(d, x, dy, pro, relu, dw, ws2, (dpft_stream_t)p->side));
        DPFT_REQUIRE(hipEventRecord(p->ev_done[slot], p->side) == hipSuccess, "resnet_backward: record event");
        p->ev_valid[slot] = true;
        return DPFT_OK;
    }
    int transposes(const Tables& T, float* wt_base, int stage) {
        hipStream_t ts = profiling_active() ? main : p->side;
        if (ts != main) {
            DPFT_REQUIRE(hipEventRecord(p->ev_ready, main) == hipSuccess, "resnet_backward: record event");
            DPFT_REQUIRE(hipStreamWaitEvent(ts, p->ev_ready, 0) == hipSuccess, "resnet_backward: wait event");
        }
        TransposeBatch tb;
        tb.n = 0;
        tb.mode = p->desc.act16 == 2 ? 1 : 0;
        for (auto& b : p->blocks) {
            if (b.layer != stage) continue;
            const ConvRef* cs[4] = {&b.c3, &b.c2, &b.c1, b.has_ds ? &b.cd : nullptr};
            for (const ConvRef* c : cs) {
                if (!c) continue;
                if (!tb.fits(c->d.K, c->d.C)) {
                    RC(weight_transpose_batch(tb, (dpft_stream_t)ts));
                    tb.n = 0;
                }
                tb.add(T.w(c->w), wt_base + c->wt, c->d.K, c->d.kh * c->d.kw, c->d.C);
                if (tb.n == TransposeBatch::MAX) {
                    RC(weight_transpose_batch(tb, (dpft_stream_t)ts));
                    tb.n = 0;
                }
            }
        }
        if (tb.n > 0) RC(weight_transpose_batch(tb, (dpft_stream_t)ts));
        if (ts != main) {
            DPFT_REQUIRE(hipEventRecord(p->ev_wt, ts) == hipSuccess, "resnet_backward: record event");
            DPFT_REQUIRE(hipStreamWaitEvent(main, p->ev_wt, 0) == hipSuccess, "resnet_backward: wait event");
        }
        return DPFT_OK;
    }
    int join() {
        DPFT_REQUIRE(hipEventRecord(p->ev_join, p->side) == hipSuccess, "resnet_backward: record event");
        DPFT_REQUIRE(hipStreamWaitEvent(main, p->ev_join, 0) == hipSuccess, "resnet_backward: wait event");
        return DPFT_OK;
    }
};

static int block_backward(ResnetPlan* p, const BlockPlan& b, const Tables& T, float* A, void* ws, SideCtx& sc,
                          BnSums& sums, const float* gp, float* dx, dpft_stream_t st, bool bn3_reduced,
                          const BlockPlan* nextb, bool* next_reduced) {
    float* dyv[2] = {A + p->o_dy, A + p->o_dy2};
    float* dab = A + p->o_da;
    float* dyd = A + p->o_dd;
    float* wt = A + p->o_wt;
    const int planes = b.c1.d.K, K3 = b.c3.d.K;
    const bool a16 = p->desc.act16 != 0;
    static const bool fuse_on = getenv("DPFT_BN_FUSE") == nullptr || atoi(getenv("DPFT_BN_FUSE")) != 0;
    const int64_t M1 = (int64_t)b.c1.d.B * b.c1.d.OH * b.c1.d.OW, M2 = (int64_t)b.c2.d.B * b.c2.d.OH * b.c2.d.OW;
    int& cur = p->dyi;
    RC(sc.acquire(cur));
    const unsigned char* m8 = (const unsigned char*)(A + b.mask);
    RC(bn_backward(A + b.y3, gp, nullptr, nullptr, A + b.p3, T.gamma(b.bn3), sums, dyv[cur], T.dgamma(b.bn3), T.dbeta(b.bn3), M2, K3, st, a16, m8, bn3_reduced));
    const bool w16 = p->desc.act16 == 2;
    if (w16) RC(sc.wgrad(cur, &b.c3.d, A + b.a2, dyv[cur], nullptr, 0, T.dw(b.c3.w)));
    else RC(sc.wgrad(cur, &b.c3.d, A + b.y2, dyv[cur], A + b.p2, 1, T.dw(b.c3.w)));
    BnReduceFuse f2{A + b.y2, A + b.p2, nullptr, 1, fuse_on ? sums.buf[sums.cur] : nullptr, false};
    RC(conv_dgrad_fused(&b.c3.d, dyv[cur], wt + b.c3.wt, dab, 0, ws, st, &f2));
    cur ^= 1;
    RC(sc.acquire(cur));
    RC(bn_backward(A + b.y2, dab, nullptr, A + b.p2, A + b.p2, T.gamma(b.bn2), sums, dyv[cur], T.dgamma(b.bn2), T.dbeta(b.bn2), M2, planes, st, a16, nullptr, f2.applied));
    if (w16) RC(sc.wgrad(cur, &b.c2.d, A + b.a1, dyv[cur], nullptr, 0, T.dw(b.c2.w)));
    else RC(sc.wgrad(cur, &b.c2.d, A + b.y1, dyv[cur], A + b.p1, 1, T.dw(b.c2.w)));
    BnReduceFuse f1{A + b.y1, A + b.p1, nullptr, 1, fuse_on ? sums.buf[sums.cur] : nullptr, false};
    RC(conv_dgrad_fused(&b.c2.d, dyv[cur], wt + b.c2.wt, dab, 0, ws, st, &f1));
    cur ^= 1;
    RC(sc.acquire(cur));
    RC(bn_backward(A + b.y1, dab, nullptr, A + b.p1, A + b.p1, T.gamma(b.bn1), sums, dyv[cur], T.dgamma(b.bn1), T.dbeta(b.bn1), M1, planes, st, a16, nullptr, f1.applied));
    RC(sc.wgrad(cur, &b.c1.d, A + b.x, dyv[cur], nullptr, 0, T.dw(b.c1.w)));
    BnReduceFuse fn{nullptr, nullptr, nullptr, 0, nullptr, false};
    if (b.has_ds) {
        RC(sc.acquire(2));
        RC(bn_backward(A + b.yd, gp, nullptr, nullptr, A + b.pd, T.gamma(b.bnd), sums, dyd, T.dgamma(b.bnd), T.dbeta(b.bnd), M2, K3, st, a16, m8));
        RC(sc.wgrad(2, &b.cd.d, A + b.x, dyd, nullptr, 0, T.dw(b.cd.w)));
        RC(dpft_conv2d_nhwc_dgrad_f32(&b.cd.d, dyd, wt + b.cd.wt, dx, 0, ws, st));
        if (nextb && fuse_on)
            fn = BnReduceFuse{A + nextb->y3, A + nextb->p3, (const unsigned char*)(A + nextb->mask), 0, sums.buf[sums.cur], false};
        RC(conv_dgrad_fused(&b.c1.d, dyv[cur], wt + b.c1.wt, dx, 1, ws, st, nextb ? &fn : nullptr));
    } else {
        if (nextb && fuse_on)
            fn = BnReduceFuse{A + nextb->y3, A + nextb->p3, (const unsigned char*)(A + nextb->mask), 0, sums.buf[sums.cur], false};
        static const bool m8_a16 = getenv("DPFT_RES_MASK8_A16") == nullptr || atoi(getenv("DPFT_RES_MASK8_A16")) != 0;
        RC(conv_dgrad_residual(&b.c1.d, dyv[cur], wt + b.c1.wt, dx, gp, A + b.out, ws, st, nextb ? &fn : nullptr, (a16 && !m8_a16) ? nullptr : m8));
    }
    if (next_reduced) *next_reduced = fn.applied;
    cur ^= 1;
    return DPFT_OK;
}

}

static int backward_stage_impl(ResnetPlan* p, int32_t stage, const float* x, const dpft_resnet_tables* tables,
                               void* arena, const float* dout, dpft_stream_t st) {
    Tables T{tables};
    float* A = (float*)arena;
    void* ws = (char*)arena + (p->arena_bytes - 2 * p->ws_bytes - 256);
    SideCtx sc{p, (hipStream_t)st, (char*)arena + (p->arena_bytes - p->ws_bytes - 128)};
    RC(sc.init());
    {
        int done = 0;
        for (const BlockPlan& b : p->blocks) done += b.layer > stage ? 1 : 0;
        p->g_cur = done & 1;
        p->dyi = done & 1;
        p->g_valid = stage != p->desc.n_layers - 1;
        p->ev_valid[0] = p->ev_valid[1] = p->ev_valid[2] = false;
    }
    const size_t out_n = (size_t)p->out_shape[stage][0] * p->out_shape[stage][1] * p->out_shape[stage][2] * p->out_shape[stage][3];
    const float* gp;
    if (!p->g_valid) {
        DPFT_REQUIRE(stage == p->desc.n_layers - 1, "resnet_backward: stages must start at the last one");
        if (dout && p->desc.act16) {
            RC(cvt_f32_to_bf16(dout, A + p->g_off[p->g_cur], (int64_t)out_n, st));
            gp = A + p->g_off[p->g_cur];
        } else if (dout) {
            gp = dout;
        } else {
            RC(zero_fill(A + p->g_off[p->g_cur], out_n * sizeof(float), st));
            gp = A + p->g_off[p->g_cur];
        }
    } else {
        if (dout) RC(add_inplace_any(A + p->g_off[p->g_cur], dout, (int64_t)out_n, p->desc.act16 != 0, st));
        gp = A + p->g_off[p->g_cur];
    }
    BnSums sums{{A + p->o_sums, A + p->o_sums + 2 * 2048}, 0, p->frozen};
    RC(zero_fill(sums.buf[0], 2 * 2 * 2048 * sizeof(float), st));
    RC(sc.transposes(T, A + p->o_wt, stage));
    bool reduced = false;
    for (int i = (int)p->blocks.size() - 1; i >= 0; --i) {
        const BlockPlan& b = p->blocks[i];
        if (b.layer != stage) continue;
        float* dx = A + p->g_off[p->g_cur ^ 1];
        const BlockPlan* nextb = (i > 0 && p->blocks[i - 1].layer == stage) ? &p->blocks[i - 1] : nullptr;
        bool next_reduced = false;
        RC(block_backward(p, b, T, A, ws, sc, sums, gp, dx, st, reduced, nextb, &next_reduced));
        reduced = next_reduced;
        p->g_cur ^= 1;
        gp = dx;
    }
    p->g_valid = true;
    if (stage == 0) {
        float* dab = A + p->o_da;
        float* wt = A + p->o_wt;
        const dpft_conv_desc& d0 = p->c0.d;
        const int64_t M0 = (int64_t)d0.B * d0.OH * d0.OW;
        const int slot = p->dyi;
        float* dyb = A + (slot ? p->o_dy2 : p->o_dy);
        RC(bn_relu_maxpool_bwd_any(A + p->y0, A + p->p0, gp, dab, d0.B, d0.OH, d0.OW, 64, p->PH, p->PW, p->desc.act16 != 0, st));
        RC(sc.acquire(slot));
        RC(bn_backward(A + p->y0, dab, nullptr, nullptr, A + p->p0, T.gamma(p->bn0), sums, dyb, T.dgamma(p->bn0), T.dbeta(p->bn0), M0, 64, st));
        const float* xa = p->adj.w >= 0 ? A + p->xa : x;
        RC(sc.wgrad(slot, &d0, xa, dyb, nullptr, 0, T.dw(p->c0.w)));
        p->dyi ^= 1;
        if (p->adj.w >= 0) {
            RC(dpft_weight_transpose_f32(T.w(p->c0.w), wt, 64, 49, 3, st));
            RC(dpft_conv2d_nhwc_dgrad_f32(&d0, dyb, wt, dab, 0, ws, st));
            RC(dpft_conv2d_nhwc_wgrad_f32(&p->adj.d, x, dab, nullptr, 0, T.dw(p->adj.w), ws, st));
        }
        p->g_valid = false;
    }
    return sc.join();
}

namespace dpft {

static uint64_t tables_hash(const ResnetPlan* p, const dpft_resnet_tables* t) {
    uint64_t h = 1469598103934665603ull;
    auto mix = [&](const void* q) { h = (h ^ (uint64_t)(uintptr_t)q) * 1099511628211ull; };
    for (int i = 0; i < p->n_conv; ++i) { mix(t->conv_w[i]); mix(t->conv_dw ? t->conv_dw[i] : nullptr); }
    for (int i = 0; i < p->n_bn; ++i) {
        mix(t->bn_gamma[i]); mix(t->bn_beta[i]); mix(t->bn_rm[i]); mix(t->bn_rv[i]);
        mix(t->bn_dgamma ? t->bn_dgamma[i] : nullptr); mix(t->bn_dbeta ? t->bn_dbeta[i] : nullptr);
    }
    return h;
}

template <typename Fn>
static int run_graphed(ResnetPlan* p, int kind, const void* x, const void* arena, const void* dout,
                       const dpft_resnet_tables* tables, dpft_stream_t st, Fn&& fn) {
    const bool single_stream = kind < 0 || (p->side_set && p->side == (hipStream_t)st);
    static const char* kinds = getenv("DPFT_PLAN_GRAPH_KINDS");
    if (kinds && ((kind < 0 && !strchr(kinds, 'f')) || (kind >= 0 && !strchr(kinds, 'b')))) return fn();
    if (!p->use_graph || profiling_active() || !single_stream) return fn();
    const uint64_t th = tables_hash(p, tables);
    ResnetPlan::GraphEntry* e = nullptr;
    for (auto& g : p->graphs)
        if (g.kind == kind && g.x == x && g.arena == arena && g.dout == dout && g.st == st && g.tables_hash == th) e = &g;
    if (!e) {
        if (p->graphs.size() > 64) return fn();
        p->graphs.push_back(ResnetPlan::GraphEntry{kind, x, arena, dout, st, th, 0, nullptr, false});
        e = &p->graphs.back();
    }
    if (e->exec) {
        static const int dbg_sync = getenv("DPFT_PLAN_GRAPH_SYNC") ? atoi(getenv("DPFT_PLAN_GRAPH_SYNC")) : 0;
        if (dbg_sync & 1) (void)hipDeviceSynchronize();
        DPFT_REQUIRE(hipGraphLaunch(e->exec, (hipStream_t)st) == hipSuccess, "resnet plan: graph launch failed");
        if (dbg_sync & 2) (void)hipDeviceSynchronize();
        return DPFT_OK;
    }
    if (e->failed || e->warm < 2) {
        ++e->warm;
        return fn();
    }
    hipStream_t hs = (hipStream_t)st;
    if (hipStreamBeginCapture(hs, hipStreamCaptureModeRelaxed) != hipSuccess) {
        (void)hipGetLastError();
        e->failed = true;
        return fn();
    }
    const int rc = fn();
    hipGraph_t graph = nullptr;
    const hipError_t ec = hipStreamEndCapture(hs, &graph);
    if (rc != DPFT_OK || ec != hipSuccess || !graph) {
        (void)hipGetLastError();
        if (graph) (void)hipGraphDestroy(graph);
        e->failed = true;
        return rc != DPFT_OK ? rc : fn();
    }
    hipGraphExec_t exec = nullptr;
    const hipError_t ei = hipGraphInstantiate(&exec, graph, nullptr, nullptr, 0);
    (void)hipGraphDestroy(graph);
// ... 40 lines not shown
```

dpft_amd/hip/lib.py:

```python
from __future__ import annotations

import ctypes as C
import os
from typing import Optional, Sequence

import torch

LIB_PATH = os.path.join(os.path.dirname(os.path.dirname(os.path.abspath(__file__))), "libdpft_hip.so")
MAX_LEVELS = 8


class HipLibraryError(RuntimeError):
    pass


class ConvDesc(C.Structure):
    _fields_ = [(n, C.c_int32) for n in ("B", "H", "W", "C", "K", "kh", "kw", "stride", "pad", "OH", "OW", "act16")] + \
               [("a_planes", C.c_void_p), ("w_planes", C.c_void_p)]


class Pyramid(C.Structure):
    _fields_ = [("level", C.c_void_p * MAX_LEVELS), ("grad", C.c_void_p * MAX_LEVELS),
                ("H", C.c_int32 * MAX_LEVELS), ("W", C.c_int32 * MAX_LEVELS), ("L", C.c_int32),
                ("grad_replicas", C.c_int32 * MAX_LEVELS)]


class ResnetDesc(C.Structure):
    _fields_ = [("B", C.c_int32), ("H", C.c_int32), ("W", C.c_int32), ("in_channels", C.c_int32),
                ("depths", C.c_int32 * 4), ("n_layers", C.c_int32), ("eps", C.c_float), ("momentum", C.c_float),
                ("act16", C.c_int32)]


class ResnetTables(C.Structure):
    _fields_ = [(n, C.POINTER(C.c_void_p)) for n in
                ("conv_w", "conv_dw", "bn_gamma", "bn_beta", "bn_rm", "bn_rv", "bn_dgamma", "bn_dbeta")]


class DecoderView(C.Structure):
    _fields_ = [(n, C.c_void_p) for n in (
        "in_proj_w", "in_proj_b", "out_proj_w", "out_proj_b", "norm1_w", "norm1_b",
        "off_w", "off_b", "att_w", "att_b", "val_w", "val_b", "outp_w", "outp_b", "norm2_w", "norm2_b",
        "ffn1_w", "ffn1_b", "ffn2_w", "ffn2_b", "norm3_w", "norm3_b")]


class SaParams(C.Structure):
    _fields_ = [(n, C.c_void_p) for n in ("in_w", "in_b", "out_w", "out_b", "n1_w", "n1_b")]


class HeadTrain(C.Structure):
    _fields_ = [("y3", C.c_void_p), ("packed", C.c_void_p), ("red_w", C.c_void_p), ("head_w", (C.c_void_p * 3) * 4),
                ("prev_center", C.c_void_p), ("T", C.c_void_p * 4), ("P", C.c_void_p * 4), ("shape", C.c_void_p * 4),
                ("p_rows", C.c_int32 * 4), ("has_t", C.c_int32 * 4), ("num_classes", C.c_int32),
                ("x", C.c_void_p), ("center", C.c_void_p), ("size", C.c_void_p), ("angle", C.c_void_p),
                ("cls", C.c_void_p), ("refs", C.c_void_p),
                ("dx", C.c_void_p), ("dcenter", C.c_void_p), ("dsize", C.c_void_p), ("dangle", C.c_void_p),
                ("dcls", C.c_void_p), ("drefs", C.c_void_p),
                ("dy3", C.c_void_p), ("dcenter_prev", C.c_void_p), ("rows", C.c_void_p), ("shape_stride", C.c_int32)]


class DecoderFwd(C.Structure):
    _fields_ = [("B", C.c_int32), ("Q", C.c_int32), ("V", C.c_int32), ("iters", C.c_int32), ("num_classes", C.c_int32),
                ("n_points", C.c_int32 * 4), ("packed_views", C.c_void_p), ("packed_heads", C.c_void_p),
                ("pyr", C.c_void_p), ("query0", C.c_void_p), ("pos", C.c_void_p), ("center0", C.c_void_p),
                ("T", C.c_void_p * 4), ("P", C.c_void_p * 4), ("shape", C.c_void_p * 4),
                ("p_rows", C.c_int32 * 4), ("has_t", C.c_int32 * 4), ("work", C.c_void_p),
                ("center", C.c_void_p), ("size", C.c_void_p), ("angle", C.c_void_p), ("cls", C.c_void_p),
                ("attn0", C.c_void_p), ("shape_stride", C.c_int32)]


class MemOp(C.Structure):
    _fields_ = [("dst", C.c_void_p), ("src", C.c_void_p), ("bytes", C.c_uint64)]


class SumSrc(C.Structure):
    _fields_ = [("src", C.c_void_p), ("n_lead", C.c_int32)]


class OuterSpec(C.Structure):
    _fields_ = [("col_a", C.c_int32), ("n_a", C.c_int32), ("col_b", C.c_int32), ("n_b", C.c_int32), ("out_off", C.c_int64)]


_P, _I, _L, _F = C.c_void_p, C.c_int32, C.c_int64, C.c_float
_DESC = C.POINTER(ConvDesc)
_PYR = C.POINTER(Pyramid)

SIGNATURES = {
    "dpft_version": (_I, []),
    "dpft_last_error": (C.c_char_p, []),
    "dpft_conv2d_workspace_bytes": (_L, [_DESC]),
    "dpft_conv2d_workspace_header_bytes": (_L, []),
    "dpft_conv2d_workspace_init": (_I, [_P, _P]),
    "dpft_split_planes_f32": (_I, [_P, _P, _L, _P]),
    "dpft_conv2d_stats_tiles": (_I, [_DESC, C.POINTER(_I)]),
    "dpft_conv_set_compute": (_I, [_I]),
    "dpft_conv_get_compute": (_I, []),
    "dpft_conv_set_split": (_I, [_I]),
    "dpft_conv_get_split": (_I, []),
    "dpft_conv2d_nhwc_fwd_f32": (_I, [_DESC, _P, _P, _P, _P, _I, _P, _P, _P, _P]),
    "dpft_conv2d_nhwc_fwd_bnact_f32": (_I, [_DESC, _P, _P, _P, _I, _P, _P, _P, _P]),
    "dpft_conv2d_nhwc_dgrad_f32": (_I, [_DESC, _P, _P, _P, _I, _P, _P]),
    "dpft_conv2d_nhwc_dgrad_bn_reduce_f32": (_I, [_DESC, _P, _P, _P, _I, _P, _P, _P, _P, _P, _P, _I, _P, _P, _P, _P]),
    "dpft_conv2d_nhwc_wgrad_f32": (_I, [_DESC, _P, _P, _P, _I, _P, _P, _P]),
    "dpft_conv2d_nhwc_wgrad_bias_f32": (_I, [_P, _P, _P, _P, _P, _P, _P]),
    "dpft_weight_transpose_f32": (_I, [_P, _P, _I, _I, _I, _P]),
    "dpft_weight_transpose_batch_f32": (_I, [_I, _P, _P, _P, _P, _P, _P]),
    "dpft_bias_grad_f32": (_I, [_P, _P, _L, _I, _P]),
    "dpft_bn_stats_f32": (_I, [_P, _P, _L, _I, _I, _P]),
    "dpft_bn_finalize_f32": (_I, [_P, _I, _I, _L, _I, _P, _P, _F, _F, _P, _P, _P, _P]),
    "dpft_bn_eval_params_f32": (_I, [_P, _P, _P, _P, _F, _I, _P, _P]),
    "dpft_bn_act_f32": (_I, [_P, _P, _P, _P, _I, _P, _L, _I, _P]),
    "dpft_bn_relu_maxpool_f32": (_I, [_P, _P, _P, _I, _I, _I, _I, _I, _I, _P]),
    "dpft_bn_relu_maxpool_bwd_f32": (_I, [_P, _P, _P, _P, _I, _I, _I, _I, _I, _I, _P]),
    "dpft_bn_bwd_reduce_f32": (_I, [_P, _P, _P, _P, _P, _P, _L, _I, _P]),
    "dpft_bn_bwd_apply_f32": (_I, [_P, _P, _P, _P, _P, _P, _P, _P, _P, _P, _L, _I, _P]),
    "dpft_relu_bwd_f32": (_I, [_P, _P, _P, _L, _P]),
    "dpft_add_inplace_f32": (_I, [_P, _P, _L, _P]),
    "dpft_bn_act_any_f32": (_I, [_P, _P, _P, _P, _I, _P, _P, _P, _L, _I, _I, _P]),
    "dpft_bn_act_sums_f32": (_I, [_P] * 10 + [_F, _I, _P, _P, _L, _I, C.POINTER(_I), _P]),
    "dpft_bn_bwd_reduce_any_f32": (_I, [_P] * 7 + [_L, _I, _I, _P]),
    "dpft_bn_bwd_apply_any_f32": (_I, [_P] * 12 + [_I, _L, _I, _I, _I, _P]),
    "dpft_bn_relu_maxpool_any_f32": (_I, [_P, _P, _P, _I, _I, _I, _I, _I, _I, _I, _P]),
    "dpft_bn_relu_maxpool_bwd_any_f32": (_I, [_P, _P, _P, _P, _I, _I, _I, _I, _I, _I, _I, _P]),
    "dpft_add_inplace_any_f32": (_I, [_P, _P, _L, _I, _P]),
    "dpft_cvt_f32_bf16": (_I, [_P, _P, _L, _P]),
    "dpft_bn_last_form": (_I, [C.POINTER(_I)]),
    "dpft_fpn_topdown_add_f32": (_I, [_P, _P, _I, _I, _I, _I, _I, _I, _P]),
    "dpft_fpn_topdown_add_bwd_f32": (_I, [_P, _P, _I, _I, _I, _I, _I, _I, _P]),
    "dpft_add_pos_f32": (_I, [_P, _P, _P, _I, _I, _I, _I, _P]),
    "dpft_fpn_lateral_f32": (_I, [_DESC, _P, _P, _P, _P, _I, _I, _P, _P, _P]),
    "dpft_fpn_output_f32": (_I, [_DESC, _P, _P, _P, _P, _P, _P, _P, _P]),
    "dpft_msda_fwd_f32": (_I, [_P, _P, _P, _P, _P, _P, _I, _I, _I, _I, _I, _I, _I, _P]),
    "dpft_msda_bwd_f32": (_I, [_P, _P, _P, _P, _P, _P, _P, _P, _P, _I, _I, _I, _I, _I, _I, _I, _P]),
    "dpft_xattn_fwd_f32": (_I, [_PYR, _P, _P, _P, _P, _P, _P, _P, _P, _I, _I, _I, _I, _I, _P]),
    "dpft_xattn_bwd_f32": (_I, [_PYR, _P, _P, _P, _P, _P, _P, _P, _P, _P, _I, _I, _I, _I, _I, _P]),
    "dpft_giou3d_yaw_f32": (_I, [_P, _P, _P, _I, _I, _I, _P]),
    "dpft_decoder_packed_view_floats": (_L, []),
    "dpft_decoder_packed_head_floats": (_L, []),
    "dpft_decoder_packed_infer_floats": (_L, [_I]),
    "dpft_decoder_pack_infer_f32": (_I, [C.POINTER(DecoderView), _I, _I, _P, _P, _I, _I, _P, _P, _I, _P, _P]),
    "dpft_decoder_pack_view_f32": (_I, [C.POINTER(DecoderView), _I, _I, _P, _P]),
    "dpft_decoder_pack_views_f32": (_I, [_P, _I, _P, _P, _P, _P]),
    "dpft_decoder_pack_head_f32": (_I, [_P, C.POINTER(C.c_void_p * 12), _I, _I, _P, _P]),
    "dpft_decoder_work_floats": (_L, [_I, _I, _I]),
    "dpft_debug_decoder_stamps": (_I, [_P]),
    "dpft_selfattn_train_fwd_f32": (_I, [_P, _I, _P, _L, _P, _F, _P, _I, _P, _P, _P, _P, _P, _I, _I, _P]),
    "dpft_selfattn_train_bwd_f32": (_I, [_P, _I, _P, _L, _P, _F, _P, _I, _P, _P, _P, _P, _P, _P, _P, _P, _P, _I, _I, _P]),
    "dpft_selfattn_train_scratch_floats": (_L, [_I, _I, _I]),
    "dpft_xattn_ffn_train_row_floats": (_L, []),
    "dpft_head_train_row_floats": (_L, []),
    "dpft_head_train_fwd_f32": (_I, [C.POINTER(HeadTrain), _I, _I, _I, _P]),
    "dpft_head_train_bwd_f32": (_I, [C.POINTER(HeadTrain), _I, _I, _I, _P]),
    "dpft_xattn_ffn_train_saved_floats": (_L, []),
    "dpft_xattn_ffn_train_scratch_floats": (_L, []),
    "dpft_xattn_ffn_train_fwd_f32": (_I, [_P, _P, _P, _I, _P, _P, _P, _P, _F, _P, _I, _P, _P, _I, _I, _P]),
    "dpft_xattn_ffn_train_bwd_f32": (_I, [_P, _P, _P, _I, _P, _P, _P, _P, _F, _P, _I, _P, _P, _P, _P, _P, _P, _P, _I, _I, _P]),
    "dpft_decoder_forward_f32": (_I, [C.POINTER(DecoderFwd), _P]),
    "dpft_decoder_attn0_f32": (_I, [_P, _P, _I, _I, _P, _P]),
    "dpft_pack_targets_f32": (_I, [_P, _P, _P, _P, _P, _I, _I, _I, _P, _P, _P, _P, _P]),
    "dpft_match_cost_f32": (_I, [_P, _P, _P, _P, _P, _P, _P, C.POINTER(_F * 5), _P, _I, _I, _I, _I, _P]),
    "dpft_set_loss_fwd_f32": (_I, [_P, _P, _P, _P, _P, _P, _P, _P, C.POINTER(_F * 5), _F, _P, _I, _I, _I, _I, _P]),
    "dpft_set_loss_scratch_floats": (_L, [_I, _I]),
    "dpft_set_loss_fwd_total_f32": (_I, [_P, _P, _P, _P, _P, _P, _P, _P, C.POINTER(_F * 5), _F, _P, _P, _P, _P, _I, _I, _I, _I, _P]),
    "dpft_set_loss_bwd_f32": (_I, [_P, _P, _P, _P, _P, _P, _P, _P, C.POINTER(_F * 5), _F, _P, _P, _P, _P, _P, _I, _I, _I, _I, _P]),
    "dpft_resize_bilinear_nhwc_f32": (_I, [_P, _P, _I, _I, _I, _I, _I, _I, _P]),
    "dpft_resize_bilinear_nhwc_u8": (_I, [_P, _P, _I, _I, _I, _I, _I, _I, _P]),
    "dpft_scale_clip_f32": (_I, [_P, _P, _L, _F, _F, _F, _F, _P]),
    "dpft_detection_metrics_f32": (_I, [_P, _P, _P, _P, _P, _P, _P, _F, _I, _P, _P, _I, _I, _I, _I, _P]),
    "dpft_radar_projection_scratch_floats": (_L, [_I, _I, _I, _I]),
    "dpft_export_select_f32": (_I, [_P, _P, _P, _P, _P, _I, _P, _P, _P, _I, _I, _I, _P]),
    "dpft_radar_projection_f32": (_I, [_P, _P, _P, _P, _P, _I, _I, _I, _I, _I, _I, _P]),
    "dpft_profile_start": (_I, []),
    "dpft_profile_stop": (_I, []),
    "dpft_profile_serialize": (_I, [_I]),
    "dpft_profile_overhead_ms": (_F, []),
    "dpft_profile_get": (_I, [_I, C.POINTER(_I), C.POINTER(C.c_double), C.POINTER(_F), C.POINTER(_I * 7)]),
    "dpft_profile_get_family": (_I, [_I, C.POINTER(_I)]),
    "dpft_rows_outer_f32": (_I, [_P, _I, _I, _I, _P, _I, _P, _L, _P]),
    "dpft_memops": (_I, [_I, _P, _P]),
    "dpft_lsap_batch_f32": (_I, [_P, _I, _I, _I, _P, _P, _P]),
    "dpft_assign_loss_f32": (_I, [_P] * 11 + [_F] + [_P] * 8 + [_I] * 4 + [_P]),
    "dpft_lsap_batch_dev_f32": (_I, [_P] * 5 + [_I] * 3 + [_P]),
    "dpft_assign_loss_dev_f32": (_I, [_P] * 11 + [_F] + [_P] * 8 + [_I] * 4 + [_P]),
    "dpft_add_many_f32": (_I, [_I, _P, _P]),
    "dpft_i64_add_many": (_I, [_I, _P, _L, _P]),
    "dpft_seed_advance": (_I, [_P, _P, _L, _P]),
# ... 107 lines not shown
```

dpft_amd/hip/ops.py:

```python
from __future__ import annotations

import ctypes as C
from typing import Optional, Sequence, Tuple

import torch

from dpft_amd.hip.lib import ConvDesc, HipLibraryError, lib, make_desc, make_pyramid, ptr, stream

_ws_cache = {}

def conv_set_compute(mode: str) -> None:
    lib.call("dpft_conv_set_compute", {"fp32": 0, "bf16": 1, "bf16x3": 2}[mode])
    _conv_cache.clear()


def conv_get_compute() -> str:
    return ("fp32", "bf16", "bf16x3")[int(lib.dpft_conv_get_compute())]


def conv_set_split(on: bool) -> None:
    lib.call("dpft_conv_set_split", int(bool(on)))
    _conv_cache.clear()


# ... 136 lines not shown
    def __init__(self, cv, planes):
        self.cv, self.planes = cv, planes

    def __enter__(self):
        if self.planes is not None:
            self.cv.desc.a_planes, self.cv.desc.w_planes = ptr(self.planes[0]), ptr(self.planes[1])

    def __exit__(self, *exc):
        self.cv.desc.a_planes = self.cv.desc.w_planes = None


def conv_fwd(cv: Conv, x, w, bias=None, pro=None, want_stats=False, out=None, planes=None):
    y = out if out is not None else torch.empty((cv.B, cv.OH, cv.OW, cv.K), dtype=torch.float32, device=x.device)
    if out is not None and (tuple(out.shape) != (cv.B, cv.OH, cv.OW, cv.K) or not out.is_contiguous() or out.dtype != torch.float32):
        raise ValueError("conv_fwd: the output buffer does not match the problem")
    ws = workspace(cv.ws_bytes, x.device)
    pb, prelu = (pro[0], int(pro[1])) if pro is not None else (None, 0)
    with _with_planes(cv, planes):
        stats = torch.empty((cv.tiles, 2, cv.K), dtype=torch.float32, device=x.device) if want_stats else None
        lib.call("dpft_conv2d_nhwc_fwd_f32", C.byref(cv.desc), ptr(x), ptr(w), ptr(bias), ptr(pb), prelu,
                 ptr(y), ptr(stats), ptr(ws), stream())
    return y, stats


def fpn_lateral(cv: Conv, x, w, bias, top=None, out=None):
    y = out if out is not None else torch.empty((cv.B, cv.OH, cv.OW, cv.K), dtype=torch.float32, device=x.device)
    ws = workspace(cv.ws_bytes, x.device)
    TH, TW = (top.shape[1], top.shape[2]) if top is not None else (0, 0)
    lib.call("dpft_fpn_lateral_f32", C.byref(cv.desc), ptr(x), ptr(w), ptr(bias), ptr(top), TH, TW, ptr(y), ptr(ws), stream())
    return y


def fpn_output(cv: Conv, lat, w, bias, pos=None, out=None):
    y = out if out is not None else torch.empty((cv.B, cv.OH, cv.OW, cv.K), dtype=torch.float32, device=lat.device)
    if out is not None and (tuple(out.shape) != (cv.B, cv.OH, cv.OW, cv.K) or not out.is_contiguous() or out.dtype != torch.float32):
        raise ValueError("fpn_output: the output buffer does not match the problem")
    ws = workspace(cv.ws_bytes, lat.device)
    px, py = pos if pos is not None else (None, None)
    lib.call("dpft_fpn_output_f32", C.byref(cv.desc), ptr(lat), ptr(w), ptr(bias), ptr(px), ptr(py), ptr(y), ptr(ws), stream())
    return y


def conv_fwd_bnact(cv: Conv, x, w, out_bn, relu=True, residual=None):
    y = torch.empty((cv.B, cv.OH, cv.OW, cv.K), dtype=torch.float32, device=x.device)
    ws = workspace(cv.ws_bytes, x.device)
    lib.call("dpft_conv2d_nhwc_fwd_bnact_f32", C.byref(cv.desc), ptr(x), ptr(w), ptr(out_bn), int(relu), ptr(residual),
             ptr(y), ptr(ws), stream())
    return y


def conv_dgrad(cv: Conv, dy, w_t, out=None, accumulate=False, planes=None):
    if out is None:
        out = torch.empty((cv.B, cv.H, cv.W, cv.C), dtype=torch.float32, device=dy.device)
        accumulate = False
    ws = workspace(cv.ws_bytes, dy.device)
    with _with_planes(cv, planes):
        lib.call("dpft_conv2d_nhwc_dgrad_f32", C.byref(cv.desc), ptr(dy), ptr(w_t), ptr(out), int(accumulate), ptr(ws),
                 stream())
    return out


def conv_dgrad_bn_reduce(cv: Conv, dy, w_t, bn_y, bn_block, sums, bn_mask8=None, residual=None, out=None, accumulate=False,
                         planes=None):
    if out is None:
        out = torch.empty((cv.B, cv.H, cv.W, cv.C), dtype=torch.float32, device=dy.device)
        accumulate = False
    ws = workspace(cv.ws_bytes, dy.device)
    applied = C.c_int32(0)
    rs, ro, rm = residual if residual is not None else (None, None, None)
    with _with_planes(cv, planes):
        lib.call("dpft_conv2d_nhwc_dgrad_bn_reduce_f32", C.byref(cv.desc), ptr(dy), ptr(w_t), ptr(out), int(accumulate),
                 ptr(rs), ptr(ro), ptr(rm), ptr(bn_y), ptr(bn_block), ptr(bn_mask8), int(bn_mask8 is None), ptr(sums),
                 C.addressof(applied), ptr(ws), stream())
    return out, bool(applied.value)


def conv_wgrad(cv: Conv, x, dy, pro=None, out=None):
    dw = out if out is not None else torch.empty((cv.K, cv.kh, cv.kw, cv.C), dtype=torch.float32, device=x.device)
    ws = workspace(cv.ws_bytes, x.device)
    pb, prelu = (pro[0], int(pro[1])) if pro is not None else (None, 0)
    lib.call("dpft_conv2d_nhwc_wgrad_f32", C.byref(cv.desc), ptr(x), ptr(dy), ptr(pb), prelu, ptr(dw),
             ptr(ws), stream())
    return dw


def conv_wgrad_bias(cv: Conv, x, dy, out=None, bias_out=None):
    dw = out if out is not None else torch.empty((cv.K, cv.kh, cv.kw, cv.C), dtype=torch.float32, device=x.device)
    db = bias_out if bias_out is not None else torch.empty(cv.K, dtype=torch.float32, device=x.device)
    ws = workspace(cv.ws_bytes, x.device)
    lib.call("dpft_conv2d_nhwc_wgrad_bias_f32", C.byref(cv.desc), ptr(x), ptr(dy), ptr(dw), ptr(db), ptr(ws), stream())
    return dw, db


def weight_transpose(w_khwc: torch.Tensor) -> torch.Tensor:
    K, kh, kw, Cin = w_khwc.shape
    wt = torch.empty((Cin, kh, kw, K), dtype=torch.float32, device=w_khwc.device)
    lib.call("dpft_weight_transpose_f32", ptr(w_khwc), ptr(wt), K, kh * kw, Cin, stream())
    return wt


def weight_transpose_many(ws) -> list:
    ws = list(ws)
    n = len(ws)
    sizes = [w.numel() for w in ws]
    flat = torch.empty(sum(sizes), dtype=torch.float32, device=ws[0].device)
    outs, off = [], 0
    for w, sz in zip(ws, sizes):
        K, kh, kw, Cin = w.shape
        outs.append(flat[off:off + sz].view(Cin, kh, kw, K))
        off += sz
    src = (C.c_void_p * n)(*[w.data_ptr() for w in ws])
    dst = (C.c_void_p * n)(*[o.data_ptr() for o in outs])
    Ks = (C.c_int32 * n)(*[w.shape[0] for w in ws])
    taps = (C.c_int32 * n)(*[w.shape[1] * w.shape[2] for w in ws])
    Cs = (C.c_int32 * n)(*[w.shape[3] for w in ws])
    lib.call("dpft_weight_transpose_batch_f32", n, C.cast(src, C.c_void_p), C.cast(dst, C.c_void_p), C.cast(Ks, C.c_void_p),
             C.cast(taps, C.c_void_p), C.cast(Cs, C.c_void_p), stream())
    return outs


def bias_grad(dy: torch.Tensor, out=None) -> torch.Tensor:
    K = dy.shape[-1]
    db = out if out is not None else torch.empty((K,), dtype=torch.float32, device=dy.device)
    lib.call("dpft_bias_grad_f32", ptr(dy), ptr(db), dy.numel() // K, K, stream())
    return db


def bn_stats(y: torch.Tensor, tile_rows: int = 128) -> torch.Tensor:
    K = y.shape[-1]
    M = y.numel() // K
    tiles = (M + tile_rows - 1) // tile_rows
    stats = torch.empty((tiles, 2, K), dtype=torch.float32, device=y.device)
    lib.call("dpft_bn_stats_f32", ptr(y), ptr(stats), M, K, tile_rows, stream())
    return stats


def bn_finalize(stats, tile_rows, M, gamma, beta, eps, momentum, running_mean=None, running_var=None):
    K = gamma.numel()
    bnp = torch.empty((4, K), dtype=torch.float32, device=gamma.device)
    lib.call("dpft_bn_finalize_f32", ptr(stats), stats.shape[0], tile_rows, M, K, ptr(gamma), ptr(beta),
             float(eps), float(momentum), ptr(running_mean), ptr(running_var), ptr(bnp), stream())
    return bnp


def bn_eval_params(gamma, beta, running_mean, running_var, eps):
    K = gamma.numel()
    bnp = torch.empty((4, K), dtype=torch.float32, device=gamma.device)
    lib.call("dpft_bn_eval_params_f32", ptr(gamma), ptr(beta), ptr(running_mean), ptr(running_var), float(eps),
             K, ptr(bnp), stream())
    return bnp


def bn_act(y, bnp, res=None, res_bnp=None, relu=True):
    out = torch.empty_like(y)
    K = y.shape[-1]
    lib.call("dpft_bn_act_f32", ptr(y), ptr(bnp), ptr(res), ptr(res_bnp), int(relu), ptr(out), y.numel() // K, K,
             stream())
    return out


def bn_relu_maxpool(y, bnp):
    B, H, W, K = y.shape
    PH, PW = (H + 2 - 3) // 2 + 1, (W + 2 - 3) // 2 + 1
    out = torch.empty((B, PH, PW, K), dtype=torch.float32, device=y.device)
    lib.call("dpft_bn_relu_maxpool_f32", ptr(y), ptr(bnp), ptr(out), B, H, W, K, PH, PW, stream())
    return out
# ... 185 lines not shown
```

include/dpft_hip.h:

```cpp
#ifndef DPFT_HIP_H
#define DPFT_HIP_H

#include <stdint.h>

#ifdef __cplusplus
extern "C" {
#endif

#define DPFT_OK 0
#define DPFT_ERR_ARG (-1)
#define DPFT_ERR_LAUNCH (-2)
#define DPFT_ERR_UNSUPPORTED (-3)

typedef void* dpft_stream_t;

int dpft_version(void);
const char* dpft_last_error(void);

typedef struct dpft_conv_desc {
    int32_t B, H, W, C;
    int32_t K;
    int32_t kh, kw, stride, pad;
    int32_t OH, OW;
    int32_t act16;
    const void* a_planes;
    const void* w_planes;
} dpft_conv_desc;

int64_t dpft_conv2d_workspace_bytes(const dpft_conv_desc* d);
int64_t dpft_conv2d_workspace_header_bytes(void);
int dpft_conv2d_workspace_init(void* workspace, dpft_stream_t stream);
int dpft_split_planes_f32(const float* src, void* planes, int64_t n, dpft_stream_t stream);
int32_t dpft_conv2d_stats_tiles(const dpft_conv_desc* d, int32_t* tile_rows);

int dpft_conv_set_compute(int32_t mode);
int32_t dpft_conv_get_compute(void);
int dpft_conv_set_split(int32_t on);
int32_t dpft_conv_get_split(void);


int dpft_conv2d_nhwc_fwd_f32(const dpft_conv_desc* d, const float* x, const float* w,
                             const float* bias, const float* pro_bn, int32_t pro_relu, float* y,
                             float* stats, void* workspace, dpft_stream_t stream);
int dpft_conv2d_nhwc_fwd_bnact_f32(const dpft_conv_desc* desc, const float* x, const float* w, const float* out_bn,
                                   int32_t relu, const float* residual, float* y, void* workspace, dpft_stream_t stream);

int dpft_conv2d_nhwc_dgrad_f32(const dpft_conv_desc* d, const float* dy, const float* w_t,
                               float* dx, int32_t accumulate, void* workspace,
                               dpft_stream_t stream);

int dpft_conv2d_nhwc_dgrad_bn_reduce_f32(const dpft_conv_desc* d, const float* dy, const float* w_t, float* dx,
                                         int32_t accumulate, const float* res_src, const float* res_out,
                                         const uint8_t* res_mask8, const float* bn_y, const float* bn_block,
                                         const uint8_t* bn_mask8, int32_t bn_self_mask, float* sums,
                                         int32_t* applied, void* workspace, dpft_stream_t stream);
int dpft_conv2d_nhwc_wgrad_f32(const dpft_conv_desc* d, const float* x, const float* dy,
                               const float* pro_bn, int32_t pro_relu, float* dw, void* workspace,
                               dpft_stream_t stream);
int dpft_weight_transpose_f32(const float* w, float* w_t, int32_t K, int32_t taps, int32_t C,
                              dpft_stream_t stream);
int dpft_weight_transpose_batch_f32(int32_t n, const float* const* w, float* const* w_t, const int32_t* K,
                                    const int32_t* taps, const int32_t* C, dpft_stream_t stream);
int dpft_conv2d_nhwc_wgrad_bias_f32(const dpft_conv_desc* d, const float* x, const float* dy, float* dw, float* db,
                                    void* workspace, dpft_stream_t stream);
int dpft_bias_grad_f32(const float* dy, float* db, int64_t M, int32_t K, dpft_stream_t stream);

int dpft_bn_stats_f32(const float* y, float* stats, int64_t M, int32_t K, int32_t tile_rows,
                      dpft_stream_t stream);
int dpft_bn_finalize_f32(const float* stats, int32_t tiles, int32_t tile_rows, int64_t M, int32_t K,
                         const float* gamma, const float* beta, float eps, float momentum,
                         float* running_mean, float* running_var, float* bnp, dpft_stream_t stream);
int dpft_bn_eval_params_f32(const float* gamma, const float* beta, const float* running_mean,
                            const float* running_var, float eps, int32_t K, float* bnp,
                            dpft_stream_t stream);
int dpft_bn_act_f32(const float* y, const float* bnp, const float* res, const float* res_bnp,
                    int32_t relu, float* out, int64_t M, int32_t K, dpft_stream_t stream);
int dpft_bn_relu_maxpool_f32(const float* y, const float* bnp, float* out, int32_t B, int32_t H,
                             int32_t W, int32_t K, int32_t PH, int32_t PW, dpft_stream_t stream);
int dpft_bn_relu_maxpool_bwd_f32(const float* y, const float* bnp, const float* dout, float* dz,
                                 int32_t B, int32_t H, int32_t W, int32_t K, int32_t PH, int32_t PW,
                                 dpft_stream_t stream);
int dpft_bn_bwd_reduce_f32(const float* y, const float* dout, const float* out,
                           const float* mask_bnp, const float* bnp, float* sums, int64_t M,
                           int32_t K, dpft_stream_t stream);
int dpft_bn_bwd_apply_f32(const float* y, const float* dout, const float* out,
                          const float* mask_bnp, const float* bnp, const float* gamma,
                          const float* sums, float* dy, float* dgamma, float* dbeta, int64_t M,
                          int32_t K, dpft_stream_t stream);
int dpft_relu_bwd_f32(const float* dout, const float* out, float* dz, int64_t n,
                      dpft_stream_t stream);
int dpft_add_inplace_f32(float* a, const float* b, int64_t n, dpft_stream_t stream);

int dpft_bn_act_any_f32(const void* y, const float* bnp, const void* res, const float* res_bnp, int32_t relu, void* out,
                        float* out32, uint8_t* mask8, int64_t M, int32_t K, int32_t storage, dpft_stream_t stream);
int dpft_bn_act_sums_f32(const float* y, const float* bnp, const uint64_t* y_sums, const float* y_gamma, const float* y_beta,
                         const float* res, const float* res_bnp, const uint64_t* res_sums, const float* res_gamma,
                         const float* res_beta, float eps, int32_t relu, float* out, uint8_t* mask8, int64_t M,
                         int32_t K, int32_t* used, dpft_stream_t stream);
int dpft_bn_bwd_reduce_any_f32(const void* y, const void* dout, const void* out, const float* mask_bnp, const uint8_t* mask8,
                               const float* bnp, float* sums, int64_t M, int32_t K, int32_t storage, dpft_stream_t stream);
int dpft_bn_bwd_apply_any_f32(const void* y, const void* dout, const void* out, const float* mask_bnp, const uint8_t* mask8,
                              const float* bnp, const float* gamma, const float* sums, void* dy, float* dgamma, float* dbeta,
                              float* zero_buf, int32_t zero_n, int64_t M, int32_t K, int32_t storage, int32_t frozen,
                              dpft_stream_t stream);
int dpft_bn_relu_maxpool_any_f32(const float* y, const float* bnp, void* out, int32_t B, int32_t H, int32_t W, int32_t K,
                                 int32_t PH, int32_t PW, int32_t storage, dpft_stream_t stream);
int dpft_bn_relu_maxpool_bwd_any_f32(const float* y, const float* bnp, const void* dout, float* dz, int32_t B, int32_t H,
                                     int32_t W, int32_t K, int32_t PH, int32_t PW, int32_t storage, dpft_stream_t stream);
int dpft_add_inplace_any_f32(void* a, const float* b, int64_t n, int32_t storage, dpft_stream_t stream);
int dpft_cvt_f32_bf16(const float* src, void* dst, int64_t n, dpft_stream_t stream);
#define DPFT_BN_FORM_NONE 0
#define DPFT_BN_FORM_GENERIC 1
#define DPFT_BN_FORM_FIXC1 2
#define DPFT_BN_FORM_FIXC2 3
#define DPFT_BN_FORM_FIXC3 4
#define DPFT_BN_FORM_WIDE16 5
#define DPFT_BN_FORM_WIDE16_FIXC 6
#define DPFT_BN_FORM_POOL_TILED 7
#define DPFT_BN_FORM_SUMS_TAKEN 8
#define DPFT_BN_FORM_SUMS_DECLINED 9
int dpft_bn_last_form(int32_t* form);

typedef struct dpft_resnet_desc {
    int32_t B, H, W, in_channels;
    int32_t depths[4];
    int32_t n_layers;
    float eps, momentum;
    int32_t act16;
} dpft_resnet_desc;

typedef struct dpft_resnet_tables {
    void* const* conv_w;
    void* const* conv_dw;
    void* const* bn_gamma;
    void* const* bn_beta;
    void* const* bn_rm;
    void* const* bn_rv;
    void* const* bn_dgamma;
    void* const* bn_dbeta;
} dpft_resnet_tables;

// ... 254 lines not shown
```

Measured before the change: 165.1.

## Batch same-shape wgrad problems across bottleneck blocks into grouped launches

Adds a grouped weight-gradient entry point that runs up to eight same-shape wgrad problems in one kernel launch and one grouped split-K reduce, indexing per-problem pointers by block. In the ResNet backward pass, wgrads of identical-shape blocks without downsampling are deferred into a ring of gradient slots on the side stream and flushed together at stage boundaries. The aim is to fill the GPU better for small wgrads and cut launch count. In exchange it uses extra ring buffers, holds activations-gradient slots longer, and adds event synchronization complexity.

```diff
diff --git a/dpft_amd/csrc/common.h b/dpft_amd/csrc/common.h
--- a/dpft_amd/csrc/common.h
+++ b/dpft_amd/csrc/common.h
@@ -125,6 +125,7 @@
 };
 int weight_transpose_batch(const TransposeBatch& tb, dpft_stream_t stream);
 int conv_mode_key();
+int conv_wgrad_group_limit(const dpft_conv_desc* d, bool pro, int pro_relu, bool unsplit_too);
 bool profiling_active();
 int zero_fill(void* ptr, size_t bytes, dpft_stream_t stream);
 int bias_grad_ws(const float* dy, float* db, int64_t M, int32_t K, void* workspace, dpft_stream_t stream);
diff --git a/dpft_amd/csrc/conv.hip b/dpft_amd/csrc/conv.hip
--- a/dpft_amd/csrc/conv.hip
+++ b/dpft_amd/csrc/conv.hip
@@ -461,8 +461,16 @@
     igemm_epilogue<BM, BN, WGM, WGN, RB, CB>(a, acc, m0, n0, mt, split, smem);
 }
 
+struct ReduceGroup {
+    float* y[kWgradGroupMax];
+};
+
 __global__ void splitk_reduce_kernel(const float* __restrict__ partial, const float* __restrict__ bias,
-                                     float* __restrict__ y, int64_t MN, int N, int splits, int accumulate) {
+                                     float* __restrict__ y, int64_t MN, int N, int splits, int accumulate, const ReduceGroup grp) {
+    if (gridDim.y > 1) {
+        y = grp.y[blockIdx.y];
+        partial += (size_t)blockIdx.y * splits * MN;
+    }
     int64_t i = ((int64_t)blockIdx.x * blockDim.x + threadIdx.x) * 4;
     if (i >= MN) return;
     if (i + 3 < MN && (N % 4) == 0) {
@@ -542,7 +550,11 @@
 
 template <int PARTS>
 __global__ __launch_bounds__(256) void splitk_reduce_wide_kernel(const float* __restrict__ partial, float* __restrict__ y,
-                                                                 int64_t MN, int splits) {
+                                                                 int64_t MN, int splits, const ReduceGroup grp) {
+    if (gridDim.y > 1) {
+        y = grp.y[blockIdx.y];
+        partial += (size_t)blockIdx.y * splits * MN;
+    }
     constexpr int CH = 256 / PARTS;
     __shared__ f32x4 red[256];
     const int ch = threadIdx.x % CH, part = threadIdx.x / CH;
@@ -1697,7 +1709,7 @@
                                stats, (int64_t)a.M, a.N, t.splits, t.bm);
             return check_launch("conv fwd split-K reduce + stats");
         }
-        hipLaunchKernelGGL(splitk_reduce_kernel, dim3(cdiv(MN, 1024)), dim3(256), 0, st, a.partial, bias, y, MN, a.N, t.splits, 0);
+        hipLaunchKernelGGL(splitk_reduce_kernel, dim3(cdiv(MN, 1024)), dim3(256), 0, st, a.partial, bias, y, MN, a.N, t.splits, 0, ReduceGroup{});
         rc = check_launch("conv fwd split-K reduce");
         if (rc) return rc;
         if (stats) {
@@ -1883,7 +1895,7 @@
     if (rc) return rc;
     if (t.splits > 1 && !fixup) {
         const int64_t MN = (int64_t)a.M * a.N;
-        hipLaunchKernelGGL(splitk_reduce_kernel, dim3(cdiv(MN, 1024)), dim3(256), 0, st, a.partial, (const float*)nullptr, dx, MN, a.N, t.splits, accumulate);
+        hipLaunchKernelGGL(splitk_reduce_kernel, dim3(cdiv(MN, 1024)), dim3(256), 0, st, a.partial, (const float*)nullptr, dx, MN, a.N, t.splits, accumulate, ReduceGroup{});
         rc = check_launch("conv dgrad split-K reduce");
     }
     return rc;
@@ -1964,25 +1976,76 @@
     return rc;
 }
 
-extern "C" int dpft_conv2d_nhwc_wgrad_f32(const dpft_conv_desc* d, const float* x, const float* dy,
-                                          const float* pro_bn, int32_t pro_relu, float* dw,
-                                          void* workspace, dpft_stream_t stream) {
+namespace dpft {
+
+struct WgradChoice {
+    int bmn, bnc, ktiles, ctiles, splits;
+    int64_t tiles;
+};
+static WgradChoice choose_wgrad(const dpft_conv_desc* d, bool vec, int psteps, int n, bool have_ws) {
+    WgradChoice c;
+    const int taps = d->kh * d->kw, J = taps * d->C;
+    auto set_tile = [&](int t) {
+        c.bmn = t; c.bnc = t;
+        c.ktiles = cdiv(d->K, t); c.ctiles = cdiv(d->C, t);
+        c.tiles = (int64_t)c.ktiles * c.ctiles * taps;
+    };
+    if (vec) {
+        if (d->K <= 32) {
+            c.bmn = 32; c.bnc = 128;
+            c.ktiles = cdiv(d->K, 32); c.ctiles = cdiv(d->C, 128);
+            c.tiles = (int64_t)c.ktiles * c.ctiles * taps;
+        } else if (d->K >= 128 && d->C >= 128 && (int64_t)cdiv(d->K, 128) * cdiv(d->C, 128) * taps >= 8) set_tile(128);
+        else set_tile(64);
+    } else {
+        c.bmn = 64; c.bnc = 64;
+        c.ktiles = cdiv(d->K, 64);
+        c.ctiles = cdiv(J, 64);
+        c.tiles = (int64_t)c.ktiles * c.ctiles;
+    }
+    const int round_wgs = (vec && c.bmn == 128) ? kNumCU : kNumCU * 2;
+    int splits = (int)std::max<int64_t>(1, round_wgs / (c.tiles * n));
     {
-        static const char* skip = getenv("DPFT_SKIP");
-        if (skip && strstr(skip, "wgrad")) return DPFT_OK;
-    }
-    int rc = check_desc(d);
-    if (rc) return rc;
-    DPFT_REQUIRE(x && dy && dw, "conv wgrad: null tensor");
-    DPFT_REQUIRE(!pro_bn || ((d->C % 32 == 0) && (d->K % 4 == 0)),
-                 "conv wgrad: fused prologue needs C %% 32 == 0 and K %% 4 == 0 (C=%d, K=%d)", d->C, d->K);
-    hipStream_t st = (hipStream_t)stream;
-    ProfScope prof(2, d, st);
-    if (!pro_bn) {
-        bool handled = false;
-        rc = thin_wgrad(d, x, dy, dw, workspace, st, handled);
-        if (rc || handled) return rc;
-    }
+        const int s2 = (int)std::max<int64_t>(1, 2 * round_wgs / (c.tiles * n));
+        const double f1 = (double)c.tiles * n * splits / round_wgs, f2 = (double)c.tiles * n * s2 / (2.0 * round_wgs);
+        if (f1 < 0.8 && f2 > f1 + 0.1) splits = s2;
+    }
+    const int64_t wbytes = (int64_t)d->K * J * 4;
+    const int max_splits = (int)std::max<int64_t>(1, std::min<int64_t>(512, (64ll << 20) / wbytes) / n);
+    if (splits > max_splits) splits = max_splits;
+    if (splits > 1 && psteps / splits < 4) {
+        if (vec && c.bmn == 128) set_tile(64);
+        splits = (int)std::max<int64_t>(1, std::min<int64_t>(std::min<int64_t>(kNumCU / (c.tiles * n), psteps), max_splits));
+    }
+    if (splits < 1) splits = 1;
+    if (const char* f = getenv("DPFT_FORCE_WGRAD")) {
+        int tb, sp;
+        if (vec && sscanf(f, "%d,%d", &tb, &sp) == 2 && (tb == 128 || tb == 64)) {
+            set_tile(tb);
+            splits = std::max(1, std::min(sp, max_splits));
+        }
+    }
+    if (splits > 1 && !have_ws) splits = 1;
+    c.splits = splits;
+    return c;
+}
+
+static bool wgrad_pipe_form(const dpft_conv_desc* d, bool vec, bool pro, int pro_relu, int bmn) {
+    static const int wpipe_env = getenv("DPFT_PIPE") ? atoi(getenv("DPFT_PIPE")) : 3;
+    return vec && (wpipe_env & 2) && g_conv_bf16 != 1 && !d->act16 && (!pro || pro_relu) && (bmn == 128 || bmn == 64);
+}
+
+static bool wgrad_takes_group(const dpft_conv_desc* d, int n, bool pro, int pro_relu, bool have_ws) {
+    const bool vec = (d->C % 32 == 0) && (d->K % 4 == 0);
+    const int M = d->B * d->OH * d->OW;
+    return wgrad_pipe_form(d, vec, pro, pro_relu, choose_wgrad(d, vec, cdiv(M, vec ? BKP : BK), n, have_ws).bmn);
+}
+
+static int wgrad_launch(const dpft_conv_desc* d, int n, const float* const* xs, const float* const* dys, const float* const* pros,
+                        int32_t pro_relu, float* const* dws, void* workspace, hipStream_t st) {
+    int rc = DPFT_OK;
+    const float *x = xs[0], *dy = dys[0], *pro_bn = pros ? pros[0] : nullptr;
+    float* dw = dws[0];
     WgradArgs a; memset(&a, 0, sizeof(a));
     a.x = x; a.dy = dy; a.dw = dw; a.pro = pro_bn; a.pro_relu = pro_relu;
     a.x16 = a.dy16 = d->act16 != 0;
@@ -1991,61 +2054,28 @@
     a.M = d->B * d->OH * d->OW;
     a.taps = d->kh * d->kw;
     a.J = a.taps * a.C;
+    a.nprob = 1;
     const bool pro = pro_bn != nullptr;
     const bool vec = (d->C % 32 == 0) && (d->K % 4 == 0);
     a.psteps = cdiv(a.M, vec ? BKP : BK);
     DPFT_REQUIRE(!vec || ((int64_t)a.M * a.K < (1ll << 29) && (int64_t)a.B * a.H * a.W * a.C < (1ll << 29)),
                  "conv wgrad: operand larger than 2 GiB");
-    int bmn, bnc;
-    int64_t tiles;
-    if (vec) {
-        if (d->K <= 32) { bmn = 32; bnc = 128; }
-        else if (d->K >= 128 && d->C >= 128 && (int64_t)cdiv(d->K, 128) * cdiv(d->C, 128) * a.taps >= 8) { bmn = 128; bnc = 128; }
-        else { bmn = 64; bnc = 64; }
-        a.ktiles = cdiv(d->K, bmn);
-        a.ctiles = cdiv(d->C, bnc);
-        tiles = (int64_t)a.ktiles * a.ctiles * a.taps;
-    } else {
-        bmn = 64; bnc = 64;
-        a.ktiles = cdiv(d->K, 64);
-        a.ctiles = cdiv(a.J, 64);
-        tiles = (int64_t)a.ktiles * a.ctiles;
-    }
-    const int round_wgs = (vec && bmn == 128) ? kNumCU : kNumCU * 2;
-    int splits = (int)std::max<int64_t>(1, round_wgs / tiles);
-    {
-        const int s2 = (int)std::max<int64_t>(1, 2 * round_wgs / tiles);
-        const double f1 = (double)tiles * splits / round_wgs, f2 = (double)tiles * s2 / (2.0 * round_wgs);
-        if (f1 < 0.8 && f2 > f1 + 0.1) splits = s2;
-    }
-    const int64_t wbytes = (int64_t)d->K * a.J * 4;
-    const int max_splits = (int)std::max<int64_t>(1, std::min<int64_t>(512, (64ll << 20) / wbytes));
-    if (splits > max_splits) splits = max_splits;
-    if (splits > 1 && a.psteps / splits < 4) {
-        if (vec && bmn == 128) {
-            bmn = 64; bnc = 64;
-            a.ktiles = cdiv(d->K, bmn); a.ctiles = cdiv(d->C, bnc);
-            tiles = (int64_t)a.ktiles * a.ctiles * a.taps;
-        }
-        splits = (int)std::max<int64_t>(1, std::min<int64_t>(std::min<int64_t>(kNumCU / tiles, a.psteps), max_splits));
-    }
-    if (splits < 1) splits = 1;
-    if (const char* f = getenv("DPFT_FORCE_WGRAD")) {
-        int tb, sp;
-        if (vec && sscanf(f, "%d,%d", &tb, &sp) == 2 && (tb == 128 || tb == 64)) {
-            bmn = tb; bnc = tb;
-            a.ktiles = cdiv(d->K, bmn); a.ctiles = cdiv(d->C, bnc);
-            tiles = (int64_t)a.ktiles * a.ctiles * a.taps;
-            splits = std::max(1, std::min(sp, max_splits));
-        }
-    }
-    if (splits > 1 && !workspace) splits = 1;
+    const WgradChoice ch = choose_wgrad(d, vec, a.psteps, n, workspace != nullptr);
+    const int bmn = ch.bmn, bnc = ch.bnc, splits = ch.splits;
+    const int64_t tiles = ch.tiles;
+    a.ktiles = ch.ktiles; a.ctiles = ch.ctiles;
+    DPFT_REQUIRE(n == 1 || wgrad_pipe_form(d, vec, pro, pro_relu, bmn), "conv wgrad group: this form takes single launches only");
     a.splits = splits;
     a.psteps_per_split = cdiv(a.psteps, splits);
     a.partial = splits > 1 ? ws_slabs(workspace) : nullptr;
+    const int64_t wn = (int64_t)d->K * a.J;
+    if (n > 1) {
+        a.nprob = n;
+        for (int i = 0; i < n; ++i)
+            a.grp[i] = WgradPtrs{xs[i], dys[i], pros ? pros[i] : nullptr, dws[i], a.partial ? a.partial + (int64_t)i * splits * wn : nullptr};
+    }
     const int nwg = (int)(tiles * splits);
-    dim3 grid(nwg), block(256);
-    static const int wpipe_env = getenv("DPFT_PIPE") ? atoi(getenv("DPFT_PIPE")) : 3;
+    dim3 grid(nwg * n), block(256);
     static const int w16_env = getenv("DPFT_WGRAD16_PIPE") ? atoi(getenv("DPFT_WGRAD16_PIPE")) : 1;
     if (vec && d->act16 && !pro && w16_env && (bmn == 128 || bmn == 64) && (d->C % 8) == 0 && (d->K % 8) == 0) {
         const int pk = bmn == 128 ? 64 : 128;
@@ -2055,7 +2085,7 @@
         g_prof_family = kFamBf16;
         if (bmn == 128) launch_lds(wgrad_pipe16_kernel<128, 128, 2, 2, 64>, grid, block, lds, st, a);
         else launch_lds(wgrad_pipe16_kernel<64, 64, 2, 2, 128>, grid, block, lds, st, a);
-    } else if (vec && (wpipe_env & 2) && g_conv_bf16 != 1 && !d->act16 && (!pro || pro_relu) && (bmn == 128 || bmn == 64)) {
+    } else if (wgrad_pipe_form(d, vec, pro, pro_relu, bmn)) {
         const int pk = bmn == 128 ? 32 : 64;
         a.psteps = cdiv(a.M, pk);
         a.psteps_per_split = cdiv(a.psteps, splits);
@@ -2103,16 +2133,87 @@
         if (skip && strstr(skip, "wreduce")) return rc;
     }
     if (splits > 1) {
-        const int64_t n = (int64_t)d->K * a.J;
-        if ((n & 3) == 0 && splits >= 16) {
-            if (n / 4 <= (int64_t)kNumCU * 64) hipLaunchKernelGGL(splitk_reduce_wide_kernel<16>, dim3(cdiv(n / 4, 16)), dim3(256), 0, st, a.partial, dw, n, splits);
-            else hipLaunchKernelGGL(splitk_reduce_wide_kernel<4>, dim3(cdiv(n / 4, 64)), dim3(256), 0, st, a.partial, dw, n, splits);
+        ReduceGroup rg; memset(&rg, 0, sizeof(rg));
+        for (int i = 0; i < n; ++i) rg.y[i] = dws[i];
+        if ((wn & 3) == 0 && splits >= 16) {
+            if (wn / 4 <= (int64_t)kNumCU * 64) hipLaunchKernelGGL(splitk_reduce_wide_kernel<16>, dim3(cdiv(wn / 4, 16), n), dim3(256), 0, st, a.partial, dw, wn, splits, rg);
+            else hipLaunchKernelGGL(splitk_reduce_wide_kernel<4>, dim3(cdiv(wn / 4, 64), n), dim3(256), 0, st, a.partial, dw, wn, splits, rg);
         } else {
-            hipLaunchKernelGGL(splitk_reduce_kernel, dim3(cdiv(n, 1024)), dim3(256), 0, st, a.partial, (const float*)nullptr, dw, n, 4, splits, 0);
+            hipLaunchKernelGGL(splitk_reduce_kernel, dim3(cdiv(wn, 1024), n), dim3(256), 0, st, a.partial, (const float*)nullptr, dw, wn, 4, splits, 0, rg);
         }
         rc = check_launch("conv wgrad split-K reduce");
     }
     return rc;
+}
+
+int conv_wgrad_group_limit(const dpft_conv_desc* d, bool pro, int pro_relu, bool unsplit_too) {
+    const bool vec = (d->C % 32 == 0) && (d->K % 4 == 0);
+    const int M = d->B * d->OH * d->OW;
+    const WgradChoice ch = choose_wgrad(d, vec, cdiv(M, vec ? BKP : BK), 1, true);
+    if (!wgrad_pipe_form(d, vec, pro, pro_relu, ch.bmn)) return 1;
+    return unsplit_too ? kWgradGroupMax : std::min(ch.splits, kWgradGroupMax);
+}
+
+}
+
+extern "C" int dpft_conv2d_nhwc_wgrad_f32(const dpft_conv_desc* d, const float* x, const float* dy,
+                                          const float* pro_bn, int32_t pro_relu, float* dw,
+                                          void* workspace, dpft_stream_t stream) {
+    {
+        static const char* skip = getenv("DPFT_SKIP");
+        if (skip && strstr(skip, "wgrad")) return DPFT_OK;
+    }
+    int rc = check_desc(d);
+    if (rc) return rc;
+    DPFT_REQUIRE(x && dy && dw, "conv wgrad: null tensor");
+    DPFT_REQUIRE(!pro_bn || ((d->C % 32 == 0) && (d->K % 4 == 0)),
+                 "conv wgrad: fused prologue needs C %% 32 == 0 and K %% 4 == 0 (C=%d, K=%d)", d->C, d->K);
+    hipStream_t st = (hipStream_t)stream;
+    ProfScope prof(2, d, st);
+    if (!pro_bn) {
+        bool handled = false;
+        rc = thin_wgrad(d, x, dy, dw, workspace, st, handled);
+        if (rc || handled) return rc;
+    }
+    return wgrad_launch(d, 1, &x, &dy, &pro_bn, pro_relu, &dw, workspace, st);
+}
+
+extern "C" int dpft_conv2d_nhwc_wgrad_group_f32(const dpft_conv_desc* d, int32_t n, const float* const* x, const float* const* dy,
+                                                const float* const* pro_bn, int32_t pro_relu, float* const* dw,
+                                                void* workspace, dpft_stream_t stream) {
+    int rc = check_desc(d);
+    if (rc) return rc;
+    DPFT_REQUIRE(n >= 1 && n <= kWgradGroupMax, "conv wgrad group: n = %d is outside 1 .. %d", n, kWgradGroupMax);
+    DPFT_REQUIRE(x && dy && dw, "conv wgrad group: null table");
+    int npro = 0;
+    for (int i = 0; i < n; ++i) {
+        DPFT_REQUIRE(x[i] && dy[i] && dw[i], "conv wgrad group: null tensor (problem %d)", i);
+        npro += (pro_bn && pro_bn[i]) ? 1 : 0;
+    }
+    DPFT_REQUIRE(npro == 0 || npro == n, "conv wgrad group: the prologue is given for %d of %d problems", npro, n);
+    DPFT_REQUIRE(npro == 0 || ((d->C % 32 == 0) && (d->K % 4 == 0)),
+                 "conv wgrad: fused prologue needs C %% 32 == 0 and K %% 4 == 0 (C=%d, K=%d)", d->C, d->K);
+    const float* const* pros = npro ? pro_bn : nullptr;
+    if (n > 1 && wgrad_takes_group(d, n, npro != 0, pro_relu, workspace != nullptr)) {
+        static const char* skip = getenv("DPFT_SKIP");
+        if (skip && strstr(skip, "wgrad")) return DPFT_OK;
+        hipStream_t st = (hipStream_t)stream;
+        {
+            ProfScope prof(2, d, st);
+            rc = wgrad_launch(d, n, x, dy, pros, pro_relu, dw, workspace, st);
+        }
+        const int fam = g_prof_family;
+        for (int i = 1; i < n && !rc; ++i) {
+            ProfScope prof(2, d, st);
+            g_prof_family = fam;
+        }
+        return rc;
+    }
+    for (int i = 0; i < n; ++i) {
+        rc = dpft_conv2d_nhwc_wgrad_f32(d, x[i], dy[i], pros ? pros[i] : nullptr, pro_relu, dw[i], workspace, stream);
+        if (rc) return rc;
+    }
+    return DPFT_OK;
 }
 
 extern "C" int dpft_weight_transpose_f32(const float* w, float* w_t, int32_t K, int32_t taps,
diff --git a/dpft_amd/csrc/conv_core.h b/dpft_amd/csrc/conv_core.h
--- a/dpft_amd/csrc/conv_core.h
+++ b/dpft_amd/csrc/conv_core.h
@@ -457,7 +457,16 @@
     static_for_impl(f, std::make_integer_sequence<int, N>{});
 }
 
-struct WgradArgs {
+constexpr int kWgradGroupMax = 8;
+struct WgradPtrs {
+    const float* x;
+    const float* dy;
+    const float* pro;
+    float* dw;
+    float* partial;
+};
+
+struct WgradHead {
     const float* x;
     const float* dy;
     float* dw;
@@ -472,6 +481,18 @@
     int J;
     int x16, dy16;
 };
+struct WgradArgs : WgradHead {
+    int nprob;
+    WgradPtrs grp[kWgradGroupMax];
+};
+
+__device__ __forceinline__ int wgrad_pick_problem(const WgradArgs& k, WgradHead& a, int nwg) {
+    if (k.nprob <= 1) return xcd_remap(blockIdx.x, nwg);
+    const int flat = xcd_remap(blockIdx.x, nwg * k.nprob);
+    const int prob = flat / nwg;
+    a.x = k.grp[prob].x; a.dy = k.grp[prob].dy; a.pro = k.grp[prob].pro; a.dw = k.grp[prob].dw; a.partial = k.grp[prob].partial;
+    return flat - prob * nwg;
+}
 
 int launch_igemm_x3(IgemmArgs& a, int bm, int bn, bool dgrad, bool pro, hipStream_t st);
 int split_planes(const float* src, void* dst, int64_t n, hipStream_t st);
diff --git a/dpft_amd/csrc/conv_pipe.h b/dpft_amd/csrc/conv_pipe.h
--- a/dpft_amd/csrc/conv_pipe.h
+++ b/dpft_amd/csrc/conv_pipe.h
@@ -308,7 +308,7 @@
 }
 
 template <int BMn, int BNc, int WGM, int WGN, int PK, bool PRO>
-__global__ __launch_bounds__(256) void wgrad_pipe_kernel(WgradArgs a) {
+__global__ __launch_bounds__(256) void wgrad_pipe_kernel(WgradArgs a_) {
     constexpr int RB = BMn / WGM / 32, CB = BNc / WGN / 32;
     constexpr int YL = BMn / 4, XL = BNc / 4;
     constexpr int YRW = 64 / YL, XRW = 64 / XL;
@@ -323,8 +323,9 @@
     const int tid = threadIdx.x, lane = tid & 63, wave = __builtin_amdgcn_readfirstlane(tid >> 6);
     const int wm = wave / WGN, wn = wave % WGN;
 
+    WgradHead a = a_;
     const int nwg = a.ktiles * a.ctiles * a.taps * a.splits;
-    int bid = xcd_remap(blockIdx.x, nwg);
+    int bid = wgrad_pick_problem(a_, a, nwg);
     const int split = bid / (a.ktiles * a.ctiles * a.taps);
     bid -= split * (a.ktiles * a.ctiles * a.taps);
     const int tap = bid / (a.ktiles * a.ctiles);
diff --git a/dpft_amd/csrc/conv_x3.hip b/dpft_amd/csrc/conv_x3.hip
--- a/dpft_amd/csrc/conv_x3.hip
+++ b/dpft_amd/csrc/conv_x3.hip
@@ -703,7 +703,7 @@
 
 
 template <int PRO_>
-__global__ __launch_bounds__(256) void wgrad_x3_kernel(WgradArgs a) {
+__global__ __launch_bounds__(256) void wgrad_x3_kernel(WgradArgs a_) {
     constexpr bool PRO = PRO_ != 0, MASK = PRO_ == 2;
     constexpr int BMn = 128, BNc = 128, WGM = 2, WGN = 2, PK = 32;
     constexpr int RB = 2, CB = 2;
@@ -722,8 +722,9 @@
     const int tid = threadIdx.x, lane = tid & 63, wave = __builtin_amdgcn_readfirstlane(tid >> 6);
     const int wm = wave / WGN, wn = wave % WGN;
 
+    WgradHead a = a_;
     const int nwg = a.ktiles * a.ctiles * a.taps * a.splits;
-    int bid = xcd_remap(blockIdx.x, nwg);
+    int bid = wgrad_pick_problem(a_, a, nwg);
     const int split = bid / (a.ktiles * a.ctiles * a.taps);
     bid -= split * (a.ktiles * a.ctiles * a.taps);
     const int tap = bid / (a.ktiles * a.ctiles);
diff --git a/dpft_amd/csrc/resnet_plan.hip b/dpft_amd/csrc/resnet_plan.hip
--- a/dpft_amd/csrc/resnet_plan.hip
+++ b/dpft_amd/csrc/resnet_plan.hip
@@ -49,6 +49,9 @@
     std::vector<char> bn_pending;
     std::vector<PendingBn> pend_list;
     size_t o_dy2;
+    int group[4][3] = {{1, 1, 1}, {1, 1, 1}, {1, 1, 1}, {1, 1, 1}};
+    size_t ring[3] = {0, 0, 0}, ring_slot[3] = {0, 0, 0};
+    size_t ring_bytes = 0;
     int g_cur;
     bool g_valid;
     bool frozen = false;
@@ -56,6 +59,8 @@
     hipStream_t side = nullptr;
     bool side_owned = true, side_set = false;
     bool ev_valid[3] = {false, false, false};
+    hipEvent_t ev_ring[3] = {nullptr, nullptr, nullptr};
+    bool ring_valid[3] = {false, false, false};
     bool use_graph = false;
     struct GraphEntry {
         int kind;
@@ -77,8 +82,15 @@
         if (ev_wt) (void)hipEventDestroy(ev_wt);
         for (auto& e : ev_done)
             if (e) (void)hipEventDestroy(e);
+        for (auto& e : ev_ring)
+            if (e) (void)hipEventDestroy(e);
     }
 };
+
+static int wgrad_group_mode() {
+    static const int mode = getenv("DPFT_WGRAD_GROUP") == nullptr ? 0 : atoi(getenv("DPFT_WGRAD_GROUP"));
+    return mode;
+}
 
 static size_t align64(size_t f) { return (f + 63) & ~(size_t)63; }
 
@@ -235,6 +247,47 @@
     p->o_dd = take(gmax);
     p->o_wt = take(wmax);
     p->o_sums = take(2 * 2 * 2048);
+    if (wgrad_group_mode() != 0 && desc->act16 == 0) {
+        constexpr size_t kRingCap = (size_t)1 << 30;
+        size_t slot[4][3] = {};
+        for (int li = 0; li < desc->n_layers; ++li) {
+            const BlockPlan* rb = nullptr;
+            int run = 0;
+            for (const BlockPlan& b : p->blocks)
+                if (b.layer == li && !b.has_ds) { rb = &b; ++run; }
+            if (run < 2) continue;
+            const ConvRef* cs[3] = {&rb->c3, &rb->c2, &rb->c1};
+            for (int pos = 0; pos < 3; ++pos) {
+                const bool pro = pos < 2;
+                p->group[li][pos] = std::max(1, std::min(run, conv_wgrad_group_limit(&cs[pos]->d, pro, 1, wgrad_group_mode() >= 2)));
+                slot[li][pos] = align64(nelem_out(cs[pos]->d));
+            }
+        }
+        auto ring_floats = [&](int pos) {
+            size_t f = 0;
+            for (int li = 0; li < desc->n_layers; ++li)
+                if (p->group[li][pos] > 1) f = std::max(f, p->group[li][pos] * slot[li][pos]);
+            return f;
+        };
+        for (;;) {
+            if ((ring_floats(0) + ring_floats(1) + ring_floats(2)) * sizeof(float) <= kRingCap) break;
+            int bl = -1, bp = -1;
+            size_t big = 0;
+            for (int li = 0; li < desc->n_layers; ++li)
+                for (int pos = 0; pos < 3; ++pos)
+                    if (p->group[li][pos] > 1 && p->group[li][pos] * slot[li][pos] > big) { big = p->group[li][pos] * slot[li][pos]; bl = li; bp = pos; }
+            --p->group[bl][bp];
+        }
+        for (int pos = 0; pos < 3; ++pos) {
+            size_t s = 0;
+            for (int li = 0; li < desc->n_layers; ++li)
+                if (p->group[li][pos] > 1) s = std::max(s, slot[li][pos]);
+            p->ring_slot[pos] = s;
+            const size_t f = ring_floats(pos);
+            if (f) p->ring[pos] = take(f);
+            p->ring_bytes += f * sizeof(float);
+        }
+    }
     p->ws_bytes = wsb;
     p->arena_bytes = off * sizeof(float) + 2 * wsb + 384;
     p->g_valid = false;
@@ -254,6 +307,8 @@
         case 3: return (int64_t)p->out32_off[idx];
         case 4: return p->out_shape[idx / 4][idx % 4];
         case 5: return (int64_t)p->fwd_floats;
+        case 6: return (int64_t)p->ring_bytes;
+        case 7: return p->group[idx / 3][idx % 3];
         default: return -1;
     }
 }
@@ -556,7 +611,47 @@
             DPFT_REQUIRE(hipEventCreateWithFlags(&p->ev_wt, hipEventDisableTiming) == hipSuccess, "resnet_backward: event");
             for (auto& e : p->ev_done)
                 DPFT_REQUIRE(hipEventCreateWithFlags(&e, hipEventDisableTiming) == hipSuccess, "resnet_backward: event");
-        }
+            for (auto& e : p->ev_ring)
+                DPFT_REQUIRE(hipEventCreateWithFlags(&e, hipEventDisableTiming) == hipSuccess, "resnet_backward: event");
+        }
+        return DPFT_OK;
+    }
+    struct Pending {
+        const dpft_conv_desc* d = nullptr;
+        int n = 0, relu = 0;
+        const float *x[8], *dy[8], *pro[8];
+        float* dw[8];
+    } pend[3];
+    int ring_acquire(int pos) {
+        if (pend[pos].n != 0 || !p->ring_valid[pos]) return DPFT_OK;
+        DPFT_REQUIRE(hipStreamWaitEvent(main, p->ev_ring[pos], 0) == hipSuccess, "resnet_backward: wait event");
+        return DPFT_OK;
+    }
+    float* ring_slot(float* A, int pos) { return A + p->ring[pos] + (size_t)pend[pos].n * p->ring_slot[pos]; }
+    int wgrad_defer(int pos, int group, const dpft_conv_desc* d, const float* x, const float* dy, const float* pro, int relu, float* dw) {
+        Pending& q = pend[pos];
+        q.d = d; q.relu = relu;
+        q.x[q.n] = x; q.dy[q.n] = dy; q.pro[q.n] = pro; q.dw[q.n] = dw;
+        ++q.n;
+        return q.n >= group ? flush(pos) : DPFT_OK;
+    }
+    int flush(int pos) {
+        Pending& q = pend[pos];
+        if (q.n == 0) return DPFT_OK;
+        const int n = q.n;
+        q.n = 0;
+        const float* const* pros = q.pro[0] ? q.pro : nullptr;
+        if (profiling_active())
+            return dpft_conv2d_nhwc_wgrad_group_f32(q.d, n, q.x, q.dy, pros, q.relu, q.dw, ws2, (dpft_stream_t)main);
+        DPFT_REQUIRE(hipEventRecord(p->ev_ready, main) == hipSuccess, "resnet_backward: record event");
+        DPFT_REQUIRE(hipStreamWaitEvent(p->side, p->ev_ready, 0) == hipSuccess, "resnet_backward: wait event");
+        RC(dpft_conv2d_nhwc_wgrad_group_f32(q.d, n, q.x, q.dy, pros, q.relu, q.dw, ws2, (dpft_stream_t)p->side));
+        DPFT_REQUIRE(hipEventRecord(p->ev_ring[pos], p->side) == hipSuccess, "resnet_backward: record event");
+        p->ring_valid[pos] = true;
+        return DPFT_OK;
+    }
+    int flush_all() {
+        for (int pos = 0; pos < 3; ++pos) RC(flush(pos));
         return DPFT_OK;
     }
     int acquire(int slot) {
@@ -625,25 +720,33 @@
     static const bool fuse_on = getenv("DPFT_BN_FUSE") == nullptr || atoi(getenv("DPFT_BN_FUSE")) != 0;
     const int64_t M1 = (int64_t)b.c1.d.B * b.c1.d.OH * b.c1.d.OW, M2 = (int64_t)b.c2.d.B * b.c2.d.OH * b.c2.d.OW;
     int& cur = p->dyi;
-    RC(sc.acquire(cur));
+    const int* grp = p->group[b.layer];
+    const bool g3 = !b.has_ds && grp[0] > 1, g2 = !b.has_ds && grp[1] > 1, g1 = !b.has_ds && grp[2] > 1;
+    RC(g3 ? sc.ring_acquire(0) : sc.acquire(cur));
+    float* const dz3 = g3 ? sc.ring_slot(A, 0) : dyv[cur];
     const unsigned char* m8 = (const unsigned char*)(A + b.mask);
-    RC(bn_backward(A + b.y3, gp, nullptr, nullptr, A + b.p3, T.gamma(b.bn3), sums, dyv[cur], T.dgamma(b.bn3), T.dbeta(b.bn3), M2, K3, st, a16, m8, bn3_reduced));
+    RC(bn_backward(A + b.y3, gp, nullptr, nullptr, A + b.p3, T.gamma(b.bn3), sums, dz3, T.dgamma(b.bn3), T.dbeta(b.bn3), M2, K3, st, a16, m8, bn3_reduced));
     const bool w16 = p->desc.act16 == 2;
-    if (w16) RC(sc.wgrad(cur, &b.c3.d, A + b.a2, dyv[cur], nullptr, 0, T.dw(b.c3.w)));
-    else RC(sc.wgrad(cur, &b.c3.d, A + b.y2, dyv[cur], A + b.p2, 1, T.dw(b.c3.w)));
+    if (g3) RC(sc.wgrad_defer(0, grp[0], &b.c3.d, A + b.y2, dz3, A + b.p2, 1, T.dw(b.c3.w)));
+    else if (w16) RC(sc.wgrad(cur, &b.c3.d, A + b.a2, dz3, nullptr, 0, T.dw(b.c3.w)));
+    else RC(sc.wgrad(cur, &b.c3.d, A + b.y2, dz3, A + b.p2, 1, T.dw(b.c3.w)));
     BnReduceFuse f2{A + b.y2, A + b.p2, nullptr, 1, fuse_on ? sums.buf[sums.cur] : nullptr, false};
-    RC(conv_dgrad_fused(&b.c3.d, dyv[cur], wt + b.c3.wt, dab, 0, ws, st, &f2));
+    RC(conv_dgrad_fused(&b.c3.d, dz3, wt + b.c3.wt, dab, 0, ws, st, &f2));
     cur ^= 1;
-    RC(sc.acquire(cur));
-    RC(bn_backward(A + b.y2, dab, nullptr, A + b.p2, A + b.p2, T.gamma(b.bn2), sums, dyv[cur], T.dgamma(b.bn2), T.dbeta(b.bn2), M2, planes, st, a16, nullptr, f2.applied));
-    if (w16) RC(sc.wgrad(cur, &b.c2.d, A + b.a1, dyv[cur], nullptr, 0, T.dw(b.c2.w)));
-    else RC(sc.wgrad(cur, &b.c2.d, A + b.y1, dyv[cur], A + b.p1, 1, T.dw(b.c2.w)));
+    RC(g2 ? sc.ring_acquire(1) : sc.acquire(cur));
+    float* const dz2 = g2 ? sc.ring_slot(A, 1) : dyv[cur];
+    RC(bn_backward(A + b.y2, dab, nullptr, A + b.p2, A + b.p2, T.gamma(b.bn2), sums, dz2, T.dgamma(b.bn2), T.dbeta(b.bn2), M2, planes, st, a16, nullptr, f2.applied));
+    if (g2) RC(sc.wgrad_defer(1, grp[1], &b.c2.d, A + b.y1, dz2, A + b.p1, 1, T.dw(b.c2.w)));
+    else if (w16) RC(sc.wgrad(cur, &b.c2.d, A + b.a1, dz2, nullptr, 0, T.dw(b.c2.w)));
+    else RC(sc.wgrad(cur, &b.c2.d, A + b.y1, dz2, A + b.p1, 1, T.dw(b.c2.w)));
     BnReduceFuse f1{A + b.y1, A + b.p1, nullptr, 1, fuse_on ? sums.buf[sums.cur] : nullptr, false};
-    RC(conv_dgrad_fused(&b.c2.d, dyv[cur], wt + b.c2.wt, dab, 0, ws, st, &f1));
+    RC(conv_dgrad_fused(&b.c2.d, dz2, wt + b.c2.wt, dab, 0, ws, st, &f1));
     cur ^= 1;
-    RC(sc.acquire(cur));
-    RC(bn_backward(A + b.y1, dab, nullptr, A + b.p1, A + b.p1, T.gamma(b.bn1), sums, dyv[cur], T.dgamma(b.bn1), T.dbeta(b.bn1), M1, planes, st, a16, nullptr, f1.applied));
-    RC(sc.wgrad(cur, &b.c1.d, A + b.x, dyv[cur], nullptr, 0, T.dw(b.c1.w)));
+    RC(g1 ? sc.ring_acquire(2) : sc.acquire(cur));
+    float* const dz1 = g1 ? sc.ring_slot(A, 2) : dyv[cur];
+    RC(bn_backward(A + b.y1, dab, nullptr, A + b.p1, A + b.p1, T.gamma(b.bn1), sums, dz1, T.dgamma(b.bn1), T.dbeta(b.bn1), M1, planes, st, a16, nullptr, f1.applied));
+    if (g1) RC(sc.wgrad_defer(2, grp[2], &b.c1.d, A + b.x, dz1, nullptr, 0, T.dw(b.c1.w)));
+    else RC(sc.wgrad(cur, &b.c1.d, A + b.x, dz1, nullptr, 0, T.dw(b.c1.w)));
     BnReduceFuse fn{nullptr, nullptr, nullptr, 0, nullptr, false};
     if (b.has_ds) {
         RC(sc.acquire(2));
@@ -652,12 +755,12 @@
         RC(dpft_conv2d_nhwc_dgrad_f32(&b.cd.d, dyd, wt + b.cd.wt, dx, 0, ws, st));
         if (nextb && fuse_on)
             fn = BnReduceFuse{A + nextb->y3, A + nextb->p3, (const unsigned char*)(A + nextb->mask), 0, sums.buf[sums.cur], false};
-        RC(conv_dgrad_fused(&b.c1.d, dyv[cur], wt + b.c1.wt, dx, 1, ws, st, nextb ? &fn : nullptr));
+        RC(conv_dgrad_fused(&b.c1.d, dz1, wt + b.c1.wt, dx, 1, ws, st, nextb ? &fn : nullptr));
     } else {
         if (nextb && fuse_on)
             fn = BnReduceFuse{A + nextb->y3, A + nextb->p3, (const unsigned char*)(A + nextb->mask), 0, sums.buf[sums.cur], false};
         static const bool m8_a16 = getenv("DPFT_RES_MASK8_A16") == nullptr || atoi(getenv("DPFT_RES_MASK8_A16")) != 0;
-        RC(conv_dgrad_residual(&b.c1.d, dyv[cur], wt + b.c1.wt, dx, gp, A + b.out, ws, st, nextb ? &fn : nullptr, (a16 && !m8_a16) ? nullptr : m8));
+        RC(conv_dgrad_residual(&b.c1.d, dz1, wt + b.c1.wt, dx, gp, A + b.out, ws, st, nextb ? &fn : nullptr, (a16 && !m8_a16) ? nullptr : m8));
     }
     if (next_reduced) *next_reduced = fn.applied;
     cur ^= 1;
@@ -680,6 +783,7 @@
         p->dyi = done & 1;
         p->g_valid = stage != p->desc.n_layers - 1;
         p->ev_valid[0] = p->ev_valid[1] = p->ev_valid[2] = false;
+        p->ring_valid[0] = p->ring_valid[1] = p->ring_valid[2] = false;
     }
     const size_t out_n = (size_t)p->out_shape[stage][0] * p->out_shape[stage][1] * p->out_shape[stage][2] * p->out_shape[stage][3];
     const float* gp;
@@ -712,6 +816,7 @@
         reduced = next_reduced;
         p->g_cur ^= 1;
         gp = dx;
+        if (!nextb || nextb->has_ds) RC(sc.flush_all());
     }
     p->g_valid = true;
     if (stage == 0) {
diff --git a/dpft_amd/hip/lib.py b/dpft_amd/hip/lib.py
--- a/dpft_amd/hip/lib.py
+++ b/dpft_amd/hip/lib.py
@@ -101,6 +101,7 @@
     "dpft_conv2d_nhwc_dgrad_f32": (_I, [_DESC, _P, _P, _P, _I, _P, _P]),
     "dpft_conv2d_nhwc_dgrad_bn_reduce_f32": (_I, [_DESC, _P, _P, _P, _I, _P, _P, _P, _P, _P, _P, _I, _P, _P, _P, _P]),
     "dpft_conv2d_nhwc_wgrad_f32": (_I, [_DESC, _P, _P, _P, _I, _P, _P, _P]),
+    "dpft_conv2d_nhwc_wgrad_group_f32": (_I, [_DESC, _I, _P, _P, _P, _I, _P, _P, _P]),
     "dpft_conv2d_nhwc_wgrad_bias_f32": (_I, [_P, _P, _P, _P, _P, _P, _P]),
     "dpft_weight_transpose_f32": (_I, [_P, _P, _I, _I, _I, _P]),
     "dpft_weight_transpose_batch_f32": (_I, [_I, _P, _P, _P, _P, _P, _P]),
diff --git a/dpft_amd/hip/ops.py b/dpft_amd/hip/ops.py
--- a/dpft_amd/hip/ops.py
+++ b/dpft_amd/hip/ops.py
@@ -242,6 +242,20 @@
     lib.call("dpft_conv2d_nhwc_wgrad_f32", C.byref(cv.desc), ptr(x), ptr(dy), ptr(pb), prelu, ptr(dw),
              ptr(ws), stream())
     return dw
+
+
+def conv_wgrad_group(cv: Conv, xs, dys, pros=None, relu=True, outs=None):
+    n = len(xs)
+    dws = list(outs) if outs is not None else [
+        torch.empty((cv.K, cv.kh, cv.kw, cv.C), dtype=torch.float32, device=xs[0].device) for _ in range(n)]
+    ws = workspace(cv.ws_bytes, xs[0].device)
+
+    def table(ts):
+        return (C.c_void_p * max(n, 1))(*[None if t is None else t.data_ptr() for t in ts])
+    pt = table(pros) if pros is not None else None
+    lib.call("dpft_conv2d_nhwc_wgrad_group_f32", C.byref(cv.desc), n, table(xs), table(dys), pt, int(bool(relu)) if pros is not None else 0,
+             table(dws), ptr(ws), stream())
+    return dws
 
 
 def conv_wgrad_bias(cv: Conv, x, dy, out=None, bias_out=None):
diff --git a/include/dpft_hip.h b/include/dpft_hip.h
--- a/include/dpft_hip.h
+++ b/include/dpft_hip.h
@@ -57,6 +57,9 @@
 int dpft_conv2d_nhwc_wgrad_f32(const dpft_conv_desc* d, const float* x, const float* dy,
                                const float* pro_bn, int32_t pro_relu, float* dw, void* workspace,
                                dpft_stream_t stream);
+int dpft_conv2d_nhwc_wgrad_group_f32(const dpft_conv_desc* d, int32_t n, const float* const* x, const float* const* dy,
+                                     const float* const* pro_bn, int32_t pro_relu, float* const* dw, void* workspace,
+                                     dpft_stream_t stream);
 int dpft_weight_transpose_f32(const float* w, float* w_t, int32_t K, int32_t taps, int32_t C,
                               dpft_stream_t stream);
 int dpft_weight_transpose_batch_f32(int32_t n, const float* const* w, float* const* w_t, const int32_t* K,
```

New measurement: 164.3. No clear change (-0.5%).
